# ufcg-lsd/custom-k8s-scheduler

Hardware: AMD Instinct MI355X
Metric: pods scheduled/sec (exact sequential stream, 5,000 nodes x 100,000 pods) (higher is better)
Workload: dtype int32+f64; 1 GPU; config2: 5,000 nodes x 100,000 pods, exact sequential, Fit+Balanced+QoS weights, percentageOfNodesToScore=100; engine=lookahead, launch=resident, table_layout=compact, lookahead=32, parallelism=single

## Files before the change

### custom-k8s-scheduler_amd/csrc/qs_ctx.hpp

```cpp
#pragma once
#include <hip/hip_runtime.h>
#include <rccl/rccl.h>

#include <mutex>
#include <string>
#include <vector>

#include "../../include/qsched.h"
#include "qs_device.hpp"
#include "qs_launch.hpp"

namespace qs_host {

constexpr int64_t kLimit = (1LL << 24) - 1;
constexpr int64_t kWideMemLimit = (1LL << 46) - 1;
constexpr int64_t kGrowLimit32 = (1LL << 31) - 1;
constexpr int64_t kGrowLimitF64 = (1LL << 53) - 1;
constexpr uint32_t kSoaMinNodes = 1u << 16;
constexpr uint32_t kAaMaxNodes = 1u << 20;

struct QsError {
    qs_status st;
    std::string msg;
};

#define HIPCHK(x)                                                                          \
    do {                                                                                   \
        hipError_t e_ = (x);                                                               \
        if (e_ != hipSuccess)                                                              \
            throw QsError{QS_EDEVICE, std::string(#x) + ": " + hipGetErrorString(e_)};     \
    } while (0)

[[noreturn]] inline void fail(qs_status st, const std::string &m) { throw QsError{st, m}; }

inline thread_local std::string g_open_err;
inline qs_status open_failed(qs_status st, const std::string &m) {
    g_open_err = m;
    return st;
}

struct DevBuf {
    void *p = nullptr;
    size_t bytes = 0;
    void ensure(size_t b) {
        if (b <= bytes) return;
        if (p) (void)hipFree(p);
        p = nullptr;
        bytes = 0;
        HIPCHK(hipMalloc(&p, b));
        bytes = b;
    }
    ~DevBuf() {
        if (p) (void)hipFree(p);
    }
    template <class T>
    T *as() const { return (T *)p; }
};

struct Mirror {
    uint32_t n = 0;
    std::vector<int64_t> ac, am, mp, rc, rm, zc, zm, np;
    std::vector<int64_t> ae, re;
    std::vector<uint64_t> th, ts, lb;
    std::vector<int32_t> zone;
    std::vector<uint64_t> gen;
    void resize(uint32_t nn) {
        n = nn;
        zone.assign(nn, 0);
        for (auto *v : {&ac, &am, &mp, &rc, &rm, &zc, &zm, &np}) v->assign(nn, 0);
        ae.assign((size_t)nn * QS_MAX_EXT, 0);
        re.assign((size_t)nn * QS_MAX_EXT, 0);
        th.assign(nn, 0);
        ts.assign(nn, 0);
        lb.assign((size_t)nn * 2, 0);
        gen.assign(nn, 0);
    }
};

inline int ctz64(int64_t v) { return v == 0 ? 64 : __builtin_ctzll((uint64_t)v); }

}

struct qs_stream {
    uint32_t p = 0;
    uint32_t feat = 0;
    std::vector<qs_pod> pods;
    std::vector<uint32_t> order;
    qs_host::DevBuf d_pods, d_podx, d_node, d_key, d_stamp;
    bool ran = false;
    int mode_ran = -1;
    uint64_t epoch_after = 0;
    int shift = 0;
    bool wide = false;
    qs_ctx *owner = nullptr;
    hipGraphExec_t gexec = nullptr;
    std::vector<uint8_t> gkey;
    ~qs_stream() {
        if (gexec) (void)hipGraphExecDestroy(gexec);
    }
};

struct qs_ctx {
    std::mutex mu;
    uint64_t table_epoch = 0;
    qs_config cfg{};
    int device = 0;
    hipStream_t stream = nullptr;
    hipStream_t stream2 = nullptr;
    std::string err;
    qs_host::Mirror m;
    int shift = 20;
    bool wide = false;
    bool dev_valid = false;
    uint32_t zero_alloc = 0;
    qs::DevTable dt{};
    qs::DevCfg dc{};
    qs_scoring_strategy strat[3] = {};
    qs_host::DevBuf strat_tab;
    std::vector<qs_stream *> streams;
    qs_host::DevBuf tbl;
    qs_host::DevBuf soa;
    bool soa_valid = false;
    qs_host::DevBuf tbl_saved;
    qs_host::Mirror m_saved;
    bool saved = false;
    bool saved_wide = false;
    int saved_shift = 20;
    bool mirror_stale = false;
    uint64_t device_faults = 0;
    qs_host::DevBuf diag;
    qs_host::DevBuf scratch, lists, clists, dio, npart, normi, nstat, nfall, nrec, bctrl, one_pod, one_podx;
    qs_host::DevBuf vshard;
    void *pin = nullptr;
    size_t pin_bytes = 0;
    uint64_t score_seq = 0;
    qs_host::DevBuf score_gs;
    uint32_t pend = 0xFFFFFFFFu;
    qs_host::DevBuf hand;
    bool handoff_off = false;
    qs_host::DevBuf resctl;
    int res_timeouts = 0;
    bool res_cooldown = false;
    uint32_t inject_used = 0;
    bool last_resident = false;
    int32_t last_res_path = 0;
    int cus = 0;
    uint64_t run_seq = 0;
    bool last_waits = false;
    uint32_t cap = 0;
    int rank = 0, world = 1;
    ncclComm_t comm = nullptr;
    qs_host::DevBuf mbox, mbox_peers;
    std::vector<void *> mbox_opened;
    bool mbox_on = false;
    bool mbox_fine = false;
    bool mbox_broken = false;
    bool mbox_host = false;
    void *mbox_hptr = nullptr;
    std::string mbox_shm;
    std::vector<void *> mbox_hmaps;
};
namespace qs_host {
void mbox_host_release(qs_ctx *c);
}

namespace qs_host {
struct ShardPlan {
    uint32_t W, v0, nv;
};
inline ShardPlan shard_plan(const qs_ctx *c) {
    if (c->world > 1) return {(uint32_t)c->world, (uint32_t)c->rank, 1u};
    if (c->cfg.virtual_shards > 1) return {(uint32_t)c->cfg.virtual_shards, 0u, (uint32_t)c->cfg.virtual_shards};
    return {1u, 0u, 1u};
}
void exchange_lists(qs_ctx *c, uint64_t *lists, size_t per_rank_entries, hipStream_t stream);
void exchange_u32(qs_ctx *c, uint32_t *buf, size_t per_rank_words, hipStream_t stream);
void allreduce_max_u64(qs_ctx *c, uint64_t *buf, size_t count, hipStream_t stream);
void allreduce_max_u32(qs_ctx *c, uint32_t *buf, size_t count, hipStream_t stream);
constexpr size_t kDioWords = 68;
constexpr size_t kMbRanks = 16, kMbSlots = 3, kMbPartPerRank = 4096;
constexpr size_t kMbFlags = 2 * kMbRanks * 8;
constexpr size_t kMbListSlot = kMbRanks * 64 * 64 * 8;
constexpr size_t kMbPartSlot = kMbRanks * kMbPartPerRank * 16;
constexpr size_t kMbResSlots = 4, kMbResPods = 32;
constexpr size_t kMbResHello = kMbFlags + kMbSlots * (kMbListSlot + kMbPartSlot);
constexpr size_t kMbResFlags = kMbResHello + 256;
constexpr size_t kMbResLists = kMbResFlags + kMbResSlots * kMbResPods * kMbRanks * 8;
constexpr size_t kMbResNFlags = kMbResLists + kMbResSlots * kMbResPods * kMbRanks * 64 * 8;
constexpr size_t kMbResNorm = kMbResNFlags + kMbResSlots * kMbResPods * kMbRanks * 8;
constexpr size_t kMbBytes = kMbResNorm + kMbResSlots * kMbResPods * kMbRanks * 16;
inline uint64_t *mbox_lists(qs_ctx *c, uint32_t slot) {
    return reinterpret_cast<uint64_t *>(static_cast<char *>(c->mbox.p) + kMbFlags + slot * kMbListSlot);
}
inline uint4 *mbox_npart(qs_ctx *c, uint32_t slot) {
    return reinterpret_cast<uint4 *>(static_cast<char *>(c->mbox.p) + kMbFlags + kMbSlots * kMbListSlot +
                                     slot * kMbPartSlot);
}
void mbox_exchange(qs_ctx *c, int phase, uint32_t slot, size_t block_bytes, uint32_t pods, uint32_t L,
                   uint64_t seq, uint32_t *werr, hipStream_t stream);
}
```

### custom-k8s-scheduler_amd/csrc/qs_host.cpp

```cpp
#include "../../include/qsched.h"

#include <hip/hip_runtime.h>

#include <algorithm>
#include <atomic>
#include <chrono>
#include <cmath>
#include <cstddef>
#include <cstdio>
#include <cstdlib>
#include <cstring>
#include <exception>
#include <mutex>
#include <new>
#include <string>
#include <vector>
#include <functional>
#include <condition_variable>
#include <thread>

#include "qs_ctx.hpp"

using namespace qs;

using namespace qs_host;

namespace {

uint32_t feat_of(const qs_config &c) {
    uint32_t f = 0;
    if (c.enable_taint) f |= kFeatTaint;
    if (c.enable_affinity) f |= kFeatAffinity;
    return f;
}

void check_cfg(const qs_config &c) {
    if (c.abi_version != QS_ABI_VERSION) fail(QS_EINVAL, "qs_config.abi_version mismatch");
    if (c.fit_weight_cpu < 0 || c.fit_weight_mem < 0 || c.fit_weight_cpu > 65535 ||
        c.fit_weight_mem > 65535)
        fail(QS_EINVAL, "fit weights out of range");
    int64_t wmax = 0;
    for (int q = 0; q < 3; q++) {
        if (c.w_fit[q] < 0 || c.w_bal[q] < 0 || c.w_fit[q] > 65535 || c.w_bal[q] > 65535)
            fail(QS_EINVAL, "plugin weights must be in [0, 65535]");
        wmax = std::max<int64_t>(wmax, (int64_t)c.w_fit[q] + c.w_bal[q]);
    }
    if (c.w_taint < 0 || c.w_affinity < 0 || c.w_taint > 65535 || c.w_affinity > 65535)
        fail(QS_EINVAL, "plugin weights must be in [0, 65535]");
    if (c.n_fit_resources < 0 || c.n_fit_resources > QS_MAX_SCORE_RES)
        fail(QS_EINVAL, "n_fit_resources must be in [0, 4]");
    if (c.n_balanced_resources < 0 || c.n_balanced_resources > QS_MAX_SCORE_RES)
        fail(QS_EINVAL, "n_balanced_resources must be in [0, 4]");
    uint32_t seen = 0;
    for (int i = 0; i < c.n_fit_resources; i++) {
        const int32_t r = c.fit_resources[i].resource;
        if (r < QS_RES_CPU || r > QS_RES_EXT1) fail(QS_EINVAL, "fit_resources: unknown resource");
        if (seen & (1u << r)) fail(QS_EINVAL, "fit_resources: duplicate resource");
        seen |= 1u << r;
        if (c.fit_resources[i].weight < 1 || c.fit_resources[i].weight > 100)
            fail(QS_EINVAL, "fit_resources: weight must be in [1, 100]");
    }
    seen = 0;
    for (int i = 0; i < c.n_balanced_resources; i++) {
        const int32_t r = c.balanced_resources[i];
        if (r < QS_RES_CPU || r > QS_RES_EXT1) fail(QS_EINVAL, "balanced_resources: unknown resource");
        if (seen & (1u << r)) fail(QS_EINVAL, "balanced_resources: duplicate resource");
        seen |= 1u << r;
    }
    const int64_t tmax = 100 * (wmax + (c.enable_taint ? c.w_taint : 0) +
                                (c.enable_affinity ? c.w_affinity : 0));
    if (tmax >= 0x7FFFFFFF) fail(QS_EINVAL, "weighted total would overflow the packed key");
}

void fit_weights(const qs_config &c, int64_t w[5]) {
    for (int r = 0; r < 5; r++) w[r] = 0;
    if (c.n_fit_resources == 0) {
        w[QS_RES_CPU] = c.fit_weight_cpu;
        w[QS_RES_MEMORY] = c.fit_weight_mem;
        return;
    }
    for (int i = 0; i < c.n_fit_resources; i++) w[c.fit_resources[i].resource] = c.fit_resources[i].weight;
}

uint32_t balanced_ids(const qs_config &c) {
    if (c.n_balanced_resources == 0) return QS_RES_CPU | (QS_RES_MEMORY << 4);
    uint32_t b = 0;
    for (int i = 0; i < c.n_balanced_resources; i++) b |= (uint32_t)c.balanced_resources[i] << (4 * i);
    return b;
}

uint32_t res_feat(const qs_config &c, bool has_ext) {
    static const bool force = getenv("QS_FORCE_RES") && getenv("QS_FORCE_RES")[0] == '1';
    if (force) return kFeatRes | kFeatExt;
    int64_t w[5];
    fit_weights(c, w);
    bool generic = has_ext && (w[QS_RES_EXT0] != 0 || w[QS_RES_EXT1] != 0);
    uint32_t set = 0;
    const uint32_t b = balanced_ids(c);
    for (int i = 0; i < QS_MAX_SCORE_RES; i++) {
        const uint32_t id = (b >> (4 * i)) & 15u;
        if (id == QS_RES_CPU || id == QS_RES_MEMORY || (has_ext && id >= QS_RES_EXT0)) set |= 1u << id;
    }
    generic |= set != ((1u << QS_RES_CPU) | (1u << QS_RES_MEMORY));
    return generic ? (kFeatRes | kFeatExt) : 0u;
}
uint32_t strat_feat(const qs_ctx *c, const qs_pod *pods, uint32_t p) {
    if (c->strat[0].type == QS_STRATEGY_LEAST_ALLOCATED && c->strat[1].type == QS_STRATEGY_LEAST_ALLOCATED &&
        c->strat[2].type == QS_STRATEGY_LEAST_ALLOCATED)
        return 0u;
    for (uint32_t j = 0; j < p; j++)
        if (c->strat[pods[j].qos].type != QS_STRATEGY_LEAST_ALLOCATED) return kFeatStrat | kFeatRes | kFeatExt;
    return 0u;
}

DevCfg make_devcfg(const qs_config &c) {
    DevCfg d{};
    int64_t w[5];
    fit_weights(c, w);
    d.wc = (int32_t)w[QS_RES_CPU];
    d.wm = (int32_t)w[QS_RES_MEMORY];
    d.we0 = (int32_t)w[QS_RES_EXT0];
    d.we1 = (int32_t)w[QS_RES_EXT1];
    d.bal = balanced_ids(c);
    auto rcp = [](int64_t v) { return v > 0 ? 1.0 / (double)v : 0.0; };
    d.yd_both = rcp(w[QS_RES_CPU] + w[QS_RES_MEMORY]);
    d.yd_c = rcp(w[QS_RES_CPU]);
    d.yd_m = rcp(w[QS_RES_MEMORY]);
    d.wtt = c.enable_taint ? c.w_taint : 0;
    d.wna = c.enable_affinity ? c.w_affinity : 0;
    d.feat = feat_of(c);
    d.ba_skip_be = c.balanced_skip_besteffort ? 1u : 0u;
    return d;
}

int table_shift(const Mirror &m) {
    int s = 20;
    for (uint32_t i = 0; i < m.n; i++) {
        s = std::min(s, ctz64(m.am[i]));
        s = std::min(s, ctz64(m.rm[i]));
        s = std::min(s, ctz64(m.zm[i]));
    }
    return s;
}

bool zero_alloc_row(const Mirror &m, uint32_t i) { return m.ac[i] <= 0 || m.am[i] <= 0; }
uint32_t count_zero_alloc(const Mirror &m) {
    uint32_t z = 0;
    for (uint32_t i = 0; i < m.n; i++) z += zero_alloc_row(m, i) ? 1u : 0u;
    return z;
}

void check_range(int64_t v, const char *what, uint32_t i, int64_t limit = kLimit) {
    if (v < 0 || v > limit)
        fail(QS_EINVAL, std::string("node ") + std::to_string(i) + ": " + what + " = " + std::to_string(v) +
                            " outside the device range [0, " + std::to_string(limit) + "]");
}

void check_row_values(const Mirror &m, uint32_t i) {
    check_range(m.ac[i], "alloc_cpu", i);
    check_range(m.rc[i], "req_cpu", i);
    check_range(m.zc[i], "nz_cpu", i);
    check_range(m.np[i], "pods", i);
    check_range(m.mp[i], "max_pods", i);
    check_range(m.am[i], "alloc_mem", i, kWideMemLimit);
    check_range(m.rm[i], "req_mem", i, kWideMemLimit);
    check_range(m.zm[i], "nz_mem", i, kWideMemLimit);
    for (int k = 0; k < QS_MAX_EXT; k++) {
        check_range(m.ae[(size_t)i * QS_MAX_EXT + k], "alloc_ext", i);
        check_range(m.re[(size_t)i * QS_MAX_EXT + k], "req_ext", i);
    }
    if (m.zone[i] < 0 || m.zone[i] >= (int32_t)kMaxZones)
        fail(QS_EINVAL, "node " + std::to_string(i) + ": zone outside [0, 64)");
}

bool row_compact_ok(const Mirror &m, uint32_t i, int shift) {
    return (m.am[i] >> shift) <= kLimit && (m.rm[i] >> shift) <= kLimit && (m.zm[i] >> shift) <= kLimit;
}

HostRow compact_row(const Mirror &m, uint32_t i, int shift, bool wide) {
    HostRow r{};
    check_row_values(m, i);
    if (!wide && !row_compact_ok(m, i, shift))
        fail(QS_EINVAL, "node " + std::to_string(i) + ": memory outside the compact layout");
    r.zone = m.zone[i];
    r.ac = (int32_t)m.ac[i];
    r.rc = (int32_t)m.rc[i];
    r.zc = (int32_t)m.zc[i];
    r.np = (int32_t)m.np[i];
    r.mp = (int32_t)m.mp[i];
    r.yc = r.ac ? 1.0 / (double)r.ac : 0.0;
    if (wide) {
        r.wam = (double)m.am[i];
        r.wrm = (double)m.rm[i];
        r.wzm = (double)m.zm[i];
        r.ym = m.am[i] ? 1.0 / r.wam : 0.0;
    } else {
        r.am = (int32_t)(m.am[i] >> shift);
        r.rm = (int32_t)(m.rm[i] >> shift);
        r.zm = (int32_t)(m.zm[i] >> shift);
        r.ym = r.am ? 1.0 / (double)r.am : 0.0;
    }
    r.ae0 = (int32_t)m.ae[(size_t)i * QS_MAX_EXT + 0];
    r.ae1 = (int32_t)m.ae[(size_t)i * QS_MAX_EXT + 1];
    r.re0 = (int32_t)m.re[(size_t)i * QS_MAX_EXT + 0];
    r.re1 = (int32_t)m.re[(size_t)i * QS_MAX_EXT + 1];
    r.th = m.th[i];
    r.ts = m.ts[i];
    r.lb0 = m.lb[(size_t)i * 2];
    r.lb1 = m.lb[(size_t)i * 2 + 1];
    return r;
}

size_t carve(DevTable &t, uint32_t cap, bool wide, char *base) {
    size_t off = 0;
    auto take = [&](size_t bytes) {
        char *p = base ? base + off : nullptr;
        off += (bytes + 255) & ~(size_t)255;
        return p;
    };
    if (wide) {
        t.rows = nullptr;
        t.wrows = (DRowW *)take((size_t)cap * sizeof(DRowW));
    } else {
        t.wrows = nullptr;
        t.rows = (DRow *)take((size_t)cap * sizeof(DRow));
    }
    t.masks = (DMask *)take((size_t)cap * sizeof(DMask));
    t.zone = (int32_t *)take((size_t)cap * 4);
    t.cap = cap;
    if (cap <= kAaMaxNodes) {
        t.apps = (uint32_t *)take((size_t)kAppWords * cap * 4);
        t.zcount = (int32_t *)take((size_t)kMaxApps * kMaxZones * 4);
    } else {
        t.apps = nullptr;
        t.zcount = nullptr;
    }
    return off;
}

DRow to_drow(const HostRow &r) {
    DRow d;
    d.ac = r.ac; d.am = r.am; d.rc = r.rc; d.rm = r.rm; d.zc = r.zc; d.zm = r.zm;
    d.np = r.np; d.mp = r.mp; d.yc = r.yc; d.ym = r.ym;
    d.ae0 = r.ae0; d.re0 = r.re0; d.ae1 = r.ae1; d.re1 = r.re1;
    return d;
}

uint32_t soa_min_nodes(const qs_ctx *c) {
    const int32_t v = c->cfg.scan_soa_min_nodes;
    return v == 0 ? kSoaMinNodes : (v < 0 ? 0xFFFFFFFFu : (uint32_t)v);
}

DRowW to_drow_wide(const HostRow &r) {
    DRowW d;
    d.ac = r.ac; d.rc = r.rc; d.zc = r.zc; d.np = r.np;
    d.am = r.wam; d.rm = r.wrm; d.zm = r.wzm; d.ym = r.ym;
    d.yc = r.yc; d.mp = r.mp; d.pad = 0;
    d.ae0 = r.ae0; d.re0 = r.re0; d.ae1 = r.ae1; d.re1 = r.re1;
    return d;
}

void upload_table(qs_ctx *c) {
    const uint32_t n = c->m.n;
    const uint32_t cap = std::max<uint32_t>(64, (n + 63) & ~63u);
    const bool wide = c->wide;
    const size_t need = carve(c->dt, cap, wide, nullptr);
    if (cap > c->cap || !c->tbl.p || need > c->tbl.bytes) {
        c->tbl.ensure(need);
        c->cap = std::max(cap, c->cap);
    }
    carve(c->dt, c->cap, wide, c->tbl.as<char>());
    c->dt.n = n;
    const bool soa = !wide && n > 0 && n >= soa_min_nodes(c);
    std::memset(&c->dt.soa, 0, sizeof c->dt.soa);
    std::vector<DRow> rows(wide ? 0 : n);
    std::vector<DRowW> wrows(wide ? n : 0);
    std::vector<DMask> masks(n);
    std::vector<int32_t> cols(soa ? (size_t)kSCols * c->cap : 0, 0);
    for (uint32_t i = 0; i < n; i++) {
        const HostRow r = compact_row(c->m, i, c->shift, wide);
        if (wide) wrows[i] = to_drow_wide(r);
        else rows[i] = to_drow(r);
        masks[i] = DMask{r.th, r.ts, r.lb0, r.lb1};
        if (soa) {
            const int32_t f[kSCols] = {r.ac, r.am, r.rc, r.rm, r.zc, r.zm, r.np, r.mp, r.ae0, r.re0, r.ae1, r.re1};
            for (int k = 0; k < kSCols; k++) cols[(size_t)k * c->cap + i] = f[k];
        }
    }
    if (n) {
        if (wide) HIPCHK(hipMemcpyAsync(c->dt.wrows, wrows.data(), n * sizeof(DRowW), hipMemcpyHostToDevice, c->stream));
        else HIPCHK(hipMemcpyAsync(c->dt.rows, rows.data(), n * sizeof(DRow), hipMemcpyHostToDevice, c->stream));
        HIPCHK(hipMemcpyAsync(c->dt.masks, masks.data(), n * sizeof(DMask), hipMemcpyHostToDevice, c->stream));
        HIPCHK(hipMemcpyAsync(c->dt.zone, c->m.zone.data(), n * 4, hipMemcpyHostToDevice, c->stream));
    }
    if (c->dt.apps) {
        HIPCHK(hipMemsetAsync(c->dt.apps, 0, (size_t)kAppWords * c->cap * 4, c->stream));
        HIPCHK(hipMemsetAsync(c->dt.zcount, 0, (size_t)kMaxApps * kMaxZones * 4, c->stream));
    }
    if (soa) {
        c->soa.ensure(cols.size() * 4);
        for (int k = 0; k < kSCols; k++) c->dt.soa.c[k] = c->soa.as<int32_t>() + (size_t)k * c->cap;
        HIPCHK(hipMemcpyAsync(c->soa.p, cols.data(), cols.size() * 4, hipMemcpyHostToDevice, c->stream));
    }
    HIPCHK(hipStreamSynchronize(c->stream));
    c->dev_valid = true;
    c->soa_valid = soa;
    c->mirror_stale = false;
}

void ensure_soa(qs_ctx *c) {
    if (!c->dt.soa.c[0] || c->soa_valid) return;
    HIPCHK(launch_rows_to_soa(c->dt, c->stream));
    c->soa_valid = true;
}

void push_row(qs_ctx *c, uint32_t i, bool sync = true) {
    if (!c->dev_valid) return;
    const HostRow r = compact_row(c->m, i, c->shift, c->wide);
    hipLaunchKernelGGL(k_set_row, dim3(1), dim3(1), 0, c->stream, c->dt, i, r,
                       kFeatExt | kFeatTaint | kFeatAffinity);
    HIPCHK(hipGetLastError());
    if (sync) HIPCHK(hipStreamSynchronize(c->stream));
}

void flush_pending(qs_ctx *c) {
    if (c->pend == 0xFFFFFFFFu) return;
    const uint32_t i = c->pend;
    c->pend = 0xFFFFFFFFu;
    if (c->dev_valid && i < c->m.n) push_row(c, i, false);
}

void sync_mirror(qs_ctx *c) {
    if (!c->mirror_stale || !c->dev_valid) return;
    const uint32_t n = c->m.n;
    Mirror &m = c->m;
    if (c->wide) {
        std::vector<DRowW> rows(n);
        if (n) HIPCHK(hipMemcpyAsync(rows.data(), c->dt.wrows, n * sizeof(DRowW), hipMemcpyDeviceToHost, c->stream));
        HIPCHK(hipStreamSynchronize(c->stream));
        for (uint32_t i = 0; i < n; i++) {
            m.rc[i] = rows[i].rc;
            m.rm[i] = (int64_t)rows[i].rm;
            m.zc[i] = rows[i].zc;
            m.zm[i] = (int64_t)rows[i].zm;
            m.np[i] = rows[i].np;
            m.re[(size_t)i * QS_MAX_EXT] = rows[i].re0;
            m.re[(size_t)i * QS_MAX_EXT + 1] = rows[i].re1;
        }
    } else {
        std::vector<DRow> rows(n);
        if (n) HIPCHK(hipMemcpyAsync(rows.data(), c->dt.rows, n * sizeof(DRow), hipMemcpyDeviceToHost, c->stream));
        HIPCHK(hipStreamSynchronize(c->stream));
        for (uint32_t i = 0; i < n; i++) {
            m.rc[i] = rows[i].rc;
            m.rm[i] = (int64_t)rows[i].rm << c->shift;
            m.zc[i] = rows[i].zc;
            m.zm[i] = (int64_t)rows[i].zm << c->shift;
            m.np[i] = rows[i].np;
            m.re[(size_t)i * QS_MAX_EXT] = rows[i].re0;
            m.re[(size_t)i * QS_MAX_EXT + 1] = rows[i].re1;
        }
    }
    c->mirror_stale = false;
}

int pod_min_shift(const qs_pod &p) { return std::min(ctz64(p.req_mem), ctz64(p.nz_mem)); }

void check_pod(const qs_pod &p, uint32_t j) {
    auto bad = [&](const char *w) {
        fail(QS_EINVAL, std::string("pod ") + std::to_string(j) + ": " + w);
    };
    if (p.qos < 0 || p.qos > 2) bad("qos must be 0..2");
    if (p.req_cpu < 0 || p.req_mem < 0 || p.nz_cpu < 0 || p.nz_mem < 0) bad("negative request");
    for (int k = 0; k < QS_MAX_EXT; k++)
        if (p.req_ext[k] < 0 || p.req_ext[k] > kLimit) bad("req_ext out of range");
    if (p.req_cpu > kLimit || p.nz_cpu > kLimit) bad("cpu request out of range");
    if (p.req_mem > kWideMemLimit || p.nz_mem > kWideMemLimit) bad("memory request above 2^46 bytes");
    if (p.n_req_terms < 0 || p.n_req_terms > QS_MAX_TERMS || p.n_pref_terms < 0 ||
        p.n_pref_terms > QS_MAX_TERMS)
        bad("term count out of range");
    for (int t = 0; t < p.n_pref_terms; t++)
        if (p.pref_weight[t] < 0 || p.pref_weight[t] > 100) bad("preferred term weight must be 0..100");
    if (p.app < 0 || p.app >= QS_MAX_APPS) bad("app outside [0, QS_MAX_APPS)");
    if (p.anti_affinity < QS_AA_NONE || p.anti_affinity > QS_AA_ZONE) bad("anti_affinity must be 0..2");
}

uint32_t pod_flags(const qs_ctx *c, const qs_pod &p) {
    const uint32_t aff = c->cfg.enable_affinity ? 1u : 0u;
    return (uint32_t)p.qos | ((uint32_t)c->strat[p.qos].type << 2) | (aff * (uint32_t)p.n_req_terms << 4) |
           (aff * (uint32_t)p.n_pref_terms << 8) | ((uint32_t)p.anti_affinity << 12) | ((uint32_t)p.app << 16);
}

size_t pod_record_bytes(bool wide) { return wide ? sizeof(DPodW) : sizeof(DPod); }

void compact_pod(const qs_ctx *c, const qs_pod &p, uint32_t j, int shift, bool wide, void *dst) {
    check_pod(p, j);
    if (wide) {
        DPodW d{};
        d.rc = (int32_t)p.req_cpu;
        d.zc = (int32_t)p.nz_cpu;
        d.rm = (double)p.req_mem;
        d.zm = (double)p.nz_mem;
        d.re0 = (int32_t)p.req_ext[0];
        d.re1 = (int32_t)p.req_ext[1];
        d.wfit = (uint16_t)c->cfg.w_fit[p.qos];
        d.wbal = (uint16_t)c->cfg.w_bal[p.qos];
        d.flags = pod_flags(c, p);
        std::memcpy(dst, &d, sizeof d);
        return;
    }
    if ((p.req_mem >> shift) > kLimit || (p.nz_mem >> shift) > kLimit)
        fail(QS_EINVAL, "pod " + std::to_string(j) + ": memory request out of the compact range");
    DPod d{};
    d.rc = (int32_t)p.req_cpu;
    d.rm = (int32_t)(p.req_mem >> shift);
    d.zc = (int32_t)p.nz_cpu;
    d.zm = (int32_t)(p.nz_mem >> shift);
    d.re0 = (int32_t)p.req_ext[0];
    d.re1 = (int32_t)p.req_ext[1];
    d.wfit = (uint16_t)c->cfg.w_fit[p.qos];
    d.wbal = (uint16_t)c->cfg.w_bal[p.qos];
    d.flags = pod_flags(c, p);
    std::memcpy(dst, &d, sizeof d);
}

DPodX compact_podx(const qs_ctx *c, const qs_pod &p) {
    DPodX x{};
    const bool taint = c->cfg.enable_taint != 0, aff = c->cfg.enable_affinity != 0;
    x.tol_hard = taint ? p.tol_hard : ~0ull;
    x.tol_soft = taint ? p.tol_soft : ~0ull;
    x.sel0 = aff ? p.sel[0] : 0ull;
    x.sel1 = aff ? p.sel[1] : 0ull;
    for (int t = 0; t < QS_MAX_TERMS; t++) {
        x.req[t][0] = p.req_terms[t][0];
        x.req[t][1] = p.req_terms[t][1];
        x.pref[t][0] = p.pref_terms[t][0];
        x.pref[t][1] = p.pref_terms[t][1];
        x.pw[t] = p.pref_weight[t];
    }
    return x;
}

std::vector<uint32_t> qos_order(const qs_pod *pods, uint32_t p, bool sort) {
    std::vector<uint32_t> o(p);
    for (uint32_t j = 0; j < p; j++) o[j] = j;
    if (sort)
        std::stable_sort(o.begin(), o.end(), [&](uint32_t a, uint32_t b) {
            if (pods[a].qos != pods[b].qos) return pods[a].qos > pods[b].qos;
            return pods[a].priority > pods[b].priority;
        });
    return o;
}

void mirror_reserve(Mirror &m, uint32_t i, const qs_pod &p, int sign) {
    m.rc[i] += sign * p.req_cpu;
    m.rm[i] += sign * p.req_mem;
    for (int k = 0; k < QS_MAX_EXT; k++) m.re[(size_t)i * QS_MAX_EXT + k] += sign * p.req_ext[k];
    m.zc[i] += sign * p.nz_cpu;
    m.zm[i] += sign * p.nz_mem;
    m.np[i] += sign;
}

void ensure_layout(qs_ctx *c, const qs_pod *pods, uint32_t p, int extra_shift = 64) {
    const Mirror &m = c->m;
    int want = std::min(c->shift, extra_shift);
    int64_t mem_max = 0, nzm = 0, nzc = 0;
    for (uint32_t j = 0; j < p; j++) {
        want = std::min(want, pod_min_shift(pods[j]));
        mem_max = std::max({mem_max, pods[j].req_mem, pods[j].nz_mem});
        nzm = std::max(nzm, pods[j].nz_mem);
        nzc = std::max(nzc, pods[j].nz_cpu);
    }
    want = std::max(0, want);
    bool wide = c->wide;
    for (uint32_t i = 0; i < m.n; i++) {
        const __int128 more = (__int128)std::max<int64_t>(0, m.mp[i] - m.np[i]) + 1;
        if ((__int128)m.zc[i] + more * nzc > kGrowLimit32)
            fail(QS_EINVAL, "node " + std::to_string(i) + ": NonZeroRequested cpu could pass 2^31 m during the stream");
        if (!wide && (!row_compact_ok(m, i, want) ||
                      (__int128)(m.zm[i] >> want) + more * (nzm >> want) > kGrowLimit32))
            wide = true;
        if (wide && (__int128)m.zm[i] + more * nzm > kGrowLimitF64)
            fail(QS_EINVAL, "node " + std::to_string(i) + ": NonZeroRequested memory could pass 2^53 B during the stream");
    }
    if (!wide && (mem_max >> want) > kLimit) wide = true;
    if (wide != c->wide || (!wide && want < c->shift)) {
        sync_mirror(c);
        c->wide = wide;
        if (!wide) c->shift = want;
        c->dev_valid = false;
        c->saved = false;
    }
    if (!c->dev_valid) upload_table(c);
}

bool pod_fits_layout(const qs_ctx *c, const qs_pod &p) {
    if (!c->dev_valid) return false;
    if (c->wide) return true;
    return pod_min_shift(p) >= c->shift && (p.req_mem >> c->shift) <= kLimit && (p.nz_mem >> c->shift) <= kLimit;
}

struct RowSnap {
    int64_t ac, am, mp, rc, rm, zc, zm, np, ae[QS_MAX_EXT], re[QS_MAX_EXT];
    uint64_t th, ts, lb0, lb1, gen;
    int32_t zone;
};
RowSnap snap_row(const Mirror &m, uint32_t i) {
    RowSnap r{m.ac[i], m.am[i], m.mp[i], m.rc[i], m.rm[i], m.zc[i], m.zm[i], m.np[i], {}, {},
              m.th[i], m.ts[i], m.lb[2 * (size_t)i], m.lb[2 * (size_t)i + 1], m.gen[i], m.zone[i]};
    for (int k = 0; k < QS_MAX_EXT; k++) {
        r.ae[k] = m.ae[(size_t)i * QS_MAX_EXT + k];
        r.re[k] = m.re[(size_t)i * QS_MAX_EXT + k];
    }
    return r;
}
void put_row(Mirror &m, uint32_t i, const RowSnap &r) {
    m.ac[i] = r.ac; m.am[i] = r.am; m.mp[i] = r.mp; m.rc[i] = r.rc; m.rm[i] = r.rm;
    m.zc[i] = r.zc; m.zm[i] = r.zm; m.np[i] = r.np;
    for (int k = 0; k < QS_MAX_EXT; k++) {
        m.ae[(size_t)i * QS_MAX_EXT + k] = r.ae[k];
        m.re[(size_t)i * QS_MAX_EXT + k] = r.re[k];
    }
    m.th[i] = r.th; m.ts[i] = r.ts; m.lb[2 * (size_t)i] = r.lb0; m.lb[2 * (size_t)i + 1] = r.lb1;
    m.gen[i] = r.gen; m.zone[i] = r.zone;
}

enum InjectHook : uint32_t { kInjStreamRun = 1u, kInjHandoff = 2u, kInjResidentStall = 4u };
bool inject_once(qs_ctx *c, const char *name, uint32_t bit) {
    const char *e = getenv("QS_INJECT_FAULT");
    if (!e || std::strcmp(e, name) != 0 || (c->inject_used & bit)) return false;
    c->inject_used |= bit;
    return true;
}
void maybe_inject_fault(qs_ctx *c, const char *entry) {
    if (inject_once(c, entry, kInjStreamRun))
        fail(QS_EDEVICE, std::string("injected device fault in ") + entry);
}

void flush_pending(qs_ctx *c);

template <class F>
qs_status guarded(qs_ctx *c, F &&f, bool keep_pending = false) {
    if (!c) return QS_EINVAL;
    std::lock_guard<std::mutex> lk(c->mu);
    try {
        if (!keep_pending) flush_pending(c);
        f();
        c->err.clear();
        return QS_OK;
    } catch (const QsError &e) {
        c->err = e.msg;
        if (e.st == QS_EDEVICE || e.st == QS_ETIMEOUT) {
            c->dev_valid = false;
            c->mirror_stale = false;
            c->saved = false;
            c->device_faults++;
        }
        return e.st;
    } catch (const std::bad_alloc &) {
        c->err = "out of host memory";
        return QS_ENOMEM;
    } catch (const std::exception &e) {
        c->err = e.what();
        return QS_EINVAL;
    } catch (...) {
        c->err = "unknown error";
        return QS_EINVAL;
    }
}

struct KernelTimer {
    bool on;
    hipStream_t stream, stream2;
    std::vector<std::pair<hipEvent_t, hipEvent_t>> ev[4];
    double secs[4] = {0, 0, 0, 0};
    uint64_t count[4] = {0, 0, 0, 0};
    KernelTimer(bool o, hipStream_t s, hipStream_t s2) : on(o), stream(s), stream2(s2) {}
    void begin(int k, hipStream_t s) {
        if (!on) return;
        hipEvent_t a, b;
        HIPCHK(hipEventCreate(&a));
        HIPCHK(hipEventCreate(&b));
        HIPCHK(hipEventRecord(a, s));
        ev[k].push_back({a, b});
    }
    void end(int k, hipStream_t s) {
        if (!on) return;
        HIPCHK(hipEventRecord(ev[k].back().second, s));
    }
    void finish() {
        if (!on) return;
        HIPCHK(hipStreamSynchronize(stream));
        HIPCHK(hipStreamSynchronize(stream2));
        for (int k = 0; k < 4; k++) {
            for (auto &e : ev[k]) {
                float ms = 0.f;
                HIPCHK(hipEventElapsedTime(&ms, e.first, e.second));
                secs[k] += ms * 1e-3;
                count[k]++;
                (void)hipEventDestroy(e.first);
                (void)hipEventDestroy(e.second);
            }
            ev[k].clear();
        }
    }
};

uint32_t la_window(const qs_ctx *c);
bool la_overlap(const qs_ctx *c);

int pick_engine(const qs_ctx *c, uint32_t n) {
    int e = c->cfg.engine;
    const uint32_t feat = c->dc.feat;
    if (e == QS_ENGINE_AUTO) {
        if (n > 0 && la_geometry(n, la_window(c), shard_plan(c).W, 2 * la_window(c)).G > 0)
            e = QS_ENGINE_LOOKAHEAD;
        else if (n <= persistent_max_nodes(feat)) e = QS_ENGINE_PERSISTENT;
        else e = QS_ENGINE_SCAN;
    }
    if (e == QS_ENGINE_BATCHED) fail(QS_EINVAL, "the batched engine runs through QS_MODE_BATCHED");
    if (e == QS_ENGINE_PERSISTENT && n > persistent_max_nodes(feat))
        fail(QS_EINVAL, "PERSISTENT engine supports at most " +
                            std::to_string(persistent_max_nodes(feat)) + " nodes for this profile");
    return e;
}

bool la_overlap(const qs_ctx *c) {
    static const char *env = getenv("QS_LA_OVERLAP");
    if (env && env[0] == '0') return false;
    return !c->cfg.lookahead_serial && la_window(c) <= 32;
}

LaGeom lookahead_geometry(const qs_ctx *c, uint32_t n, bool overlap) {
    const ShardPlan sp = shard_plan(c);
    const uint32_t K = la_window(c);
    LaGeom geo = la_geometry(n, K, sp.W, overlap ? 2 * K : K);
    geo.v0 = sp.v0;
    geo.nv = sp.nv;
    return geo;
}

uint32_t la_window(const qs_ctx *c) {
    int K = c->cfg.lookahead > 0 ? c->cfg.lookahead : 32;
    return (uint32_t)std::min(64, std::max(1, K));
}

void percentile_stats(const std::vector<uint64_t> &st, qs_stats *s) {
    if (st.size() < 2) return;
    std::vector<double> d(st.size() - 1);
    for (size_t i = 1; i < st.size(); i++) d[i - 1] = (double)(st[i] - st[i - 1]) * 0.01;
    std::sort(d.begin(), d.end());
    auto pct = [&](double q) { return d[std::min(d.size() - 1, (size_t)(q * (double)(d.size() - 1) + 0.5))]; };
    s->p50_cycle_us = pct(0.50);
    s->p99_cycle_us = pct(0.99);
    s->max_cycle_us = d.back();
}

}

uint64_t run_batched(qs_ctx *c, qs_stream *s, const void *dp, const DPodX *dx, int32_t *on, uint64_t *ok,
                     KernelTimer &kt) {
    const uint32_t n = c->m.n, P = s->p;
    for (int q = 0; q < 3; q++)
        if (c->strat[q].type != QS_STRATEGY_LEAST_ALLOCATED)
            fail(QS_EINVAL, "QS_MODE_BATCHED scores LeastAllocated only (qs_set_scoring_strategy[_qos]: class " +
                                std::to_string(q) + " has another strategy)");
    if (c->dc.feat & (kFeatTaint | kFeatAffinity))
        fail(QS_EINVAL, "QS_MODE_BATCHED supports the Fit + Balanced (+ extended resources) profile");
    if (!c->dt.apps) fail(QS_EINVAL, "QS_MODE_BATCHED keeps anti-affinity state for tables up to 2^20 nodes");
    if (c->world > 1 || c->cfg.virtual_shards > 1) fail(QS_EINVAL, "QS_MODE_BATCHED runs unsharded");
    if (batch_claim_lds(n) > 160 * 1024)
        fail(QS_EINVAL, "QS_MODE_BATCHED claims batches in LDS: tables up to 712,672 nodes");
    HIPCHK(batch_claim_prepare());
    const uint32_t B = c->cfg.batch_pods > 0 ? (uint32_t)std::min(64, c->cfg.batch_pods) : 64u;
    LaGeom geo = la_geometry(n, B, 1, 64);
    if (geo.G == 0) fail(QS_EINVAL, "no batched geometry for this table size");
    geo.waves = 4;
    geo.k32 = 0;
    const size_t lwords = (size_t)geo.K * 64 * geo.eplr;
    const size_t cwords = std::max<size_t>(1, (size_t)geo.K * geo.G * geo.L);
    c->lists.ensure(8 * lwords);
    c->clists.ensure(8 * cwords);
    c->bctrl.ensure(4 * 192);
    uint32_t *ctrl = c->bctrl.as<uint32_t>(), *bidx = ctrl + 64, *tickets = ctrl + 128;
    LaBufs bf{c->lists.as<uint64_t>(), c->clists.as<uint64_t>(), nullptr, nullptr, nullptr, nullptr,
              nullptr, bidx, ctrl};
    const char *fm = getenv("QS_BATCH_FUSED_MERGE");
    if (!(fm && fm[0] == '0')) bf.tickets = tickets;
    auto batch = [&]() {
        kt.begin(2, c->stream);
        HIPCHK(launch_la_window(c->dt, dp, dx, 0, P, c->dc, geo, bf, on, ok, nullptr, nullptr, c->stream, 1));
        kt.end(2, c->stream);
        kt.begin(3, c->stream);
        HIPCHK(launch_batch_claim(c->dt, dp, bf.lists, ctrl, bidx, P, B, on, ok, c->stream));
        kt.end(3, c->stream);
    };
    const uint32_t nb0 = (P + B - 1) / B;
    auto enqueue = [&]() {
        HIPCHK(hipMemsetAsync(bf.lists, 0, 8 * lwords, c->stream));
        HIPCHK(hipMemsetAsync(tickets, 0, 4 * 64, c->stream));
        HIPCHK(launch_batch_init(ctrl, bidx, P, B, c->stream));
        static const char *se = getenv("QS_SYNC_EVERY");
        const uint32_t every = se ? (uint32_t)atoi(se) : 0u;
        for (uint32_t b = 0; b < nb0; ++b) {
            batch();
            if (every && (b + 1) % every == 0 && !kt.on) HIPCHK(hipStreamSynchronize(c->stream));
        }
    };
    static const char *genv = getenv("QS_GRAPH");
    if (!kt.on && !(genv && genv[0] == '0')) {
        std::vector<uint8_t> key;
        auto put = [&](const void *p, size_t nb) { key.insert(key.end(), (const uint8_t *)p, (const uint8_t *)p + nb); };
        const void *ptrs[] = {c->dt.rows, c->dt.wrows, c->dt.apps, bf.lists, bf.clists, ctrl, dp, on, ok};
        put(ptrs, sizeof ptrs);
        put(&c->dt.n, sizeof c->dt.n);
        put(&c->dc, sizeof c->dc);
        put(&geo, sizeof geo);
        const int tag = 2;
        put(&tag, sizeof tag);
        put(&bf.tickets, sizeof bf.tickets);
        if (!s->gexec || s->gkey != key) {
            if (s->gexec) (void)hipGraphExecDestroy(s->gexec);
            s->gexec = nullptr;
            HIPCHK(hipStreamBeginCapture(c->stream, hipStreamCaptureModeThreadLocal));
            try {
                enqueue();
            } catch (...) {
                hipGraph_t g = nullptr;
                (void)hipStreamEndCapture(c->stream, &g);
                if (g) (void)hipGraphDestroy(g);
                throw;
            }
            hipGraph_t g = nullptr;
            HIPCHK(hipStreamEndCapture(c->stream, &g));
            const hipError_t ie = hipGraphInstantiate(&s->gexec, g, nullptr, nullptr, 0);
            (void)hipGraphDestroy(g);
            HIPCHK(ie);
            s->gkey = key;
        }
        HIPCHK(hipGraphLaunch(s->gexec, c->stream));
    } else {
        enqueue();
    }
    uint64_t batches = nb0;
    for (;;) {
        uint32_t h[2] = {0, 0};
        HIPCHK(hipMemcpyAsync(h, ctrl, 8, hipMemcpyDeviceToHost, c->stream));
        HIPCHK(hipStreamSynchronize(c->stream));
        if (h[0] == 0) break;
        if (batches > 2ull * P + 64) fail(QS_EDEVICE, "batched mode made no progress");
        batch();
        ++batches;
    }
    c->soa_valid = false;
    return batches;
}

extern "C" {

const char *qs_version(void) { return "qsched 0.1 (gfx950)"; }

void qs_config_default(qs_config *cfg) {
    if (!cfg) return;
    std::memset(cfg, 0, sizeof(*cfg));
    cfg->abi_version = QS_ABI_VERSION;
    cfg->engine = QS_ENGINE_AUTO;
    cfg->fit_weight_cpu = 1;
    cfg->fit_weight_mem = 1;
    const int32_t wf[3] = {1, 2, 3}, wb[3] = {1, 1, 1};
    for (int q = 0; q < 3; q++) { cfg->w_fit[q] = wf[q]; cfg->w_bal[q] = wb[q]; }
    cfg->w_taint = 3;
    cfg->w_affinity = 2;
    cfg->qos_sort = 1;
}

qs_status qs_open(const qs_config *cfg, int device, qs_ctx **out) {
    g_open_err.clear();
    if (!cfg || !out) return open_failed(QS_EINVAL, "qs_open: null config or output pointer");
    *out = nullptr;
    qs_ctx *c = new (std::nothrow) qs_ctx();
    if (!c) return QS_ENOMEM;
    try {
        check_cfg(*cfg);
        c->cfg = *cfg;
        c->device = device;
        int ndev = 0;
        HIPCHK(hipGetDeviceCount(&ndev));
        if (device < 0 || device >= ndev) fail(QS_EINVAL, "no such device");
        HIPCHK(hipSetDevice(device));
        HIPCHK(hipStreamCreateWithFlags(&c->stream, hipStreamNonBlocking));
        HIPCHK(hipStreamCreateWithFlags(&c->stream2, hipStreamNonBlocking));
        c->dc = make_devcfg(c->cfg);
        c->scratch.ensure(scan_scratch_bytes());
        HIPCHK(hipMemset(c->scratch.p, 0, scan_scratch_bytes()));
    } catch (const QsError &e) {
        delete c;
        return open_failed(e.st, e.msg);
    } catch (...) {
        delete c;
        return open_failed(QS_EDEVICE, "qs_open: unexpected failure");
    }
    *out = c;
    return QS_OK;
}

qs_status qs_close(qs_ctx *c) {
    if (!c) return QS_EINVAL;
    {
        std::lock_guard<std::mutex> lk(c->mu);
        (void)hipSetDevice(c->device);
        if (c->stream) (void)hipStreamSynchronize(c->stream);
        if (c->comm) (void)ncclCommDestroy(c->comm);
        c->comm = nullptr;
        for (void *p : c->mbox_opened) (void)hipIpcCloseMemHandle(p);
        c->mbox_opened.clear();
        mbox_host_release(c);
        for (qs_stream *ps : c->streams) ps->owner = nullptr;
        c->streams.clear();
    }
    hipStream_t s = c->stream, s2 = c->stream2;
    if (s2) (void)hipStreamSynchronize(s2);
    if (c->pin) (void)hipHostFree(c->pin);
    delete c;
    if (s) (void)hipStreamDestroy(s);
    if (s2) (void)hipStreamDestroy(s2);
    return QS_OK;
}

static void shape_table(const qs_shape_point *sh, uint32_t n, uint8_t table[101]) {
    if (!sh || !table) fail(QS_EINVAL, "shape: null pointer");
    if (n < 1 || n > QS_MAX_SHAPE) fail(QS_EINVAL, "shape: 1 to 16 points");
    for (uint32_t i = 0; i < n; i++) {
        if (sh[i].utilization < 0 || sh[i].utilization > 100) fail(QS_EINVAL, "shape: utilization must be in [0, 100]");
        if (sh[i].score < 0 || sh[i].score > 10) fail(QS_EINVAL, "shape: score must be in [0, 10]");
        if (i && sh[i].utilization <= sh[i - 1].utilization)
            fail(QS_EINVAL, "shape: utilization must be strictly increasing");
    }
    for (int64_t p = 0; p <= 100; p++) {
        int64_t v = (int64_t)sh[n - 1].score * 10;
        for (uint32_t i = 0; i < n; i++) {
            if (p > sh[i].utilization) continue;
            const int64_t s1 = (int64_t)sh[i].score * 10;
            if (i == 0) { v = s1; break; }
            const int64_t s0 = (int64_t)sh[i - 1].score * 10, u0 = sh[i - 1].utilization, u1 = sh[i].utilization;
            v = s0 + (s1 - s0) * (p - u0) / (u1 - u0);
            break;
        }
        table[p] = (uint8_t)v;
    }
}

qs_status qs_shape_table(const qs_shape_point *shape, uint32_t n, uint8_t table[101]) {
    try {
        shape_table(shape, n, table);
    } catch (const QsError &) {
        return QS_EINVAL;
    }
    return QS_OK;
}

static void strategy_table(const qs_scoring_strategy *s, uint8_t tab[128]) {
    if (!s) fail(QS_EINVAL, "null scoring strategy");
    if (s->type != QS_STRATEGY_LEAST_ALLOCATED && s->type != QS_STRATEGY_MOST_ALLOCATED &&
        s->type != QS_STRATEGY_REQUESTED_TO_CAPACITY_RATIO)
        fail(QS_EINVAL, "unknown scoring strategy type");
    if (s->type != QS_STRATEGY_REQUESTED_TO_CAPACITY_RATIO && s->n_shape != 0)
        fail(QS_EINVAL, "a shape is given for a scoring strategy that takes none");
    std::memset(tab, 0, 128);
    if (s->type == QS_STRATEGY_REQUESTED_TO_CAPACITY_RATIO) {
        if (s->n_shape < 1 || s->n_shape > QS_MAX_SHAPE) fail(QS_EINVAL, "shape: 1 to 16 points");
        shape_table(s->shape, (uint32_t)s->n_shape, tab);
    }
}

static void set_strategy(qs_ctx *c, int q0, int q1, const qs_scoring_strategy *s, const uint8_t tab[128]) {
    if (!c->streams.empty()) fail(QS_ESTATE, "the scoring strategy cannot change while prepared streams exist");
    HIPCHK(hipSetDevice(c->device));
    HIPCHK(hipStreamSynchronize(c->stream));
    alignas(16) uint8_t all[3 * 128];
    qs_scoring_strategy next[3] = {c->strat[0], c->strat[1], c->strat[2]};
    for (int q = 0; q < 3; q++) {
        if (q >= q0 && q <= q1) {
            next[q] = qs_scoring_strategy{};
            next[q].type = s->type;
            next[q].n_shape = s->n_shape;
            for (int i = 0; i < s->n_shape; i++) next[q].shape[i] = s->shape[i];
            std::memcpy(all + 128 * q, tab, 128);
        } else {
            uint8_t t[128];
            strategy_table(&c->strat[q], t);
            std::memcpy(all + 128 * q, t, 128);
        }
    }
    c->strat_tab.ensure(sizeof all);
    HIPCHK(hipMemcpy(c->strat_tab.p, all, sizeof all, hipMemcpyHostToDevice));
    bool rtcr = false;
    for (int q = 0; q < 3; q++) {
        c->strat[q] = next[q];
        rtcr |= next[q].type == QS_STRATEGY_REQUESTED_TO_CAPACITY_RATIO;
    }
    const uint64_t tp = rtcr ? (uint64_t)(uintptr_t)c->strat_tab.p : 0;
    c->dc.strat_tab_lo = (uint32_t)tp;
    c->dc.strat_tab_hi = (uint32_t)(tp >> 32);
}

qs_status qs_set_scoring_strategy(qs_ctx *c, const qs_scoring_strategy *s) {
    return guarded(c, [&] {
        uint8_t tab[128];
        strategy_table(s, tab);
        set_strategy(c, 0, 2, s, tab);
    });
}

qs_status qs_set_scoring_strategy_qos(qs_ctx *c, int32_t qos, const qs_scoring_strategy *s) {
    return guarded(c, [&] {
        if (qos < 0 || qos > 2) fail(QS_EINVAL, "qos must be 0 (BestEffort), 1 (Burstable) or 2 (Guaranteed)");
        uint8_t tab[128];
        strategy_table(s, tab);
        set_strategy(c, qos, qos, s, tab);
    });
}

qs_status qs_get_scoring_strategy_qos(qs_ctx *c, int32_t qos, qs_scoring_strategy *out) {
    return guarded(c, [&] {
        if (qos < 0 || qos > 2) fail(QS_EINVAL, "qos must be 0 (BestEffort), 1 (Burstable) or 2 (Guaranteed)");
        if (!out) fail(QS_EINVAL, "null scoring strategy");
        *out = c->strat[qos];
    });
}

const char *qs_last_error(const qs_ctx *c) {
    if (c) return c->err.c_str();
    return g_open_err.empty() ? "null context" : g_open_err.c_str();
}

qs_status qs_nodes_load(qs_ctx *c, const qs_node_soa *nd, uint32_t n) {
    return guarded(c, [&] {
        if (!nd || !nd->alloc_cpu || !nd->alloc_mem) fail(QS_EINVAL, "alloc_cpu/alloc_mem required");
        HIPCHK(hipSetDevice(c->device));
        Mirror &m = c->m;
        m.resize(n);
        auto get = [](const int64_t *a, size_t i, int64_t d) { return a ? a[i] : d; };
        for (uint32_t i = 0; i < n; i++) {
            m.ac[i] = nd->alloc_cpu[i];
            m.am[i] = nd->alloc_mem[i];
            m.mp[i] = get(nd->max_pods, i, 110);
            m.rc[i] = get(nd->req_cpu, i, 0);
            m.rm[i] = get(nd->req_mem, i, 0);
            m.zc[i] = get(nd->nz_cpu, i, 0);
            m.zm[i] = get(nd->nz_mem, i, 0);
            m.np[i] = get(nd->pods, i, 0);
            for (int k = 0; k < QS_MAX_EXT; k++) {
                m.ae[(size_t)i * QS_MAX_EXT + k] = get(nd->alloc_ext, (size_t)i * QS_MAX_EXT + k, 0);
                m.re[(size_t)i * QS_MAX_EXT + k] = get(nd->req_ext, (size_t)i * QS_MAX_EXT + k, 0);
            }
            m.zone[i] = nd->zone ? nd->zone[i] : 0;
            m.th[i] = nd->taint_hard ? nd->taint_hard[i] : 0;
            m.ts[i] = nd->taint_soft ? nd->taint_soft[i] : 0;
            m.lb[2 * (size_t)i] = nd->label_bits ? nd->label_bits[2 * (size_t)i] : 0;
            m.lb[2 * (size_t)i + 1] = nd->label_bits ? nd->label_bits[2 * (size_t)i + 1] : 0;
        }
        for (uint32_t i = 0; i < n; i++) check_row_values(m, i);
        c->shift = table_shift(m);
        c->zero_alloc = count_zero_alloc(m);
        c->wide = false;
        for (uint32_t i = 0; i < n && !c->wide; i++) c->wide = !row_compact_ok(m, i, c->shift);
        c->dev_valid = false;
        c->saved = false;
        c->mirror_stale = false;
        ++c->table_epoch;
        upload_table(c);
    });
}

qs_status qs_nodes_read(qs_ctx *c, const qs_node_soa_out *o, uint32_t n) {
    return guarded(c, [&] {
        if (!o) fail(QS_EINVAL, "null output");
        if (n != c->m.n) fail(QS_EINVAL, "n does not match the loaded table");
        sync_mirror(c);
        const Mirror &m = c->m;
        auto put = [](int64_t *d, const std::vector<int64_t> &s) {
            if (d) std::memcpy(d, s.data(), s.size() * 8);
        };
        put(o->alloc_cpu, m.ac); put(o->alloc_mem, m.am); put(o->max_pods, m.mp);
        put(o->req_cpu, m.rc); put(o->req_mem, m.rm); put(o->nz_cpu, m.zc); put(o->nz_mem, m.zm);
        put(o->pods, m.np); put(o->alloc_ext, m.ae); put(o->req_ext, m.re);
        if (o->taint_hard) std::memcpy(o->taint_hard, m.th.data(), 8 * (size_t)n);
        if (o->taint_soft) std::memcpy(o->taint_soft, m.ts.data(), 8 * (size_t)n);
        if (o->label_bits) std::memcpy(o->label_bits, m.lb.data(), 16 * (size_t)n);
        if (o->zone) std::memcpy(o->zone, m.zone.data(), 4 * (size_t)n);
    });
}

qs_status qs_node_upsert(qs_ctx *c, uint32_t idx, const qs_node_row *r, uint64_t generation) {
    return guarded(c, [&] {
        if (!r) fail(QS_EINVAL, "null row");
        HIPCHK(hipSetDevice(c->device));
        sync_mirror(c);
        Mirror &m = c->m;
        if (idx > m.n) fail(QS_EINVAL, "idx beyond table end (append only at idx == n)");
        if (idx < m.n && generation != 0 && generation <= m.gen[idx]) return;
        Mirror one;
        one.resize(1);
        one.ac[0] = r->alloc_cpu; one.am[0] = r->alloc_mem; one.mp[0] = r->max_pods;
        one.rc[0] = r->req_cpu; one.rm[0] = r->req_mem; one.zc[0] = r->nz_cpu; one.zm[0] = r->nz_mem;
        one.np[0] = r->pods;
        for (int k = 0; k < QS_MAX_EXT; k++) { one.ae[k] = r->alloc_ext[k]; one.re[k] = r->req_ext[k]; }
        one.th[0] = r->taint_hard; one.ts[0] = r->taint_soft;
        one.lb[0] = r->label_bits[0]; one.lb[1] = r->label_bits[1];
        one.zone[0] = r->zone;
        one.gen[0] = generation;
        check_row_values(one, 0);
        const bool was_zero = idx < m.n && zero_alloc_row(m, idx);
        if (idx == m.n) {
            Mirror old = m;
            m.resize(old.n + 1);
            auto cp = [&](std::vector<int64_t> &d, const std::vector<int64_t> &s) { std::copy(s.begin(), s.end(), d.begin()); };
            cp(m.ac, old.ac); cp(m.am, old.am); cp(m.mp, old.mp); cp(m.rc, old.rc); cp(m.rm, old.rm);
            cp(m.zc, old.zc); cp(m.zm, old.zm); cp(m.np, old.np); cp(m.ae, old.ae); cp(m.re, old.re);
            std::copy(old.th.begin(), old.th.end(), m.th.begin());
            std::copy(old.ts.begin(), old.ts.end(), m.ts.begin());
            std::copy(old.lb.begin(), old.lb.end(), m.lb.begin());
            std::copy(old.gen.begin(), old.gen.end(), m.gen.begin());
            std::copy(old.zone.begin(), old.zone.end(), m.zone.begin());
            c->dev_valid = false;
            c->saved = false;
        }
        put_row(m, idx, snap_row(one, 0));
        c->zero_alloc += (zero_alloc_row(m, idx) ? 1u : 0u) - (was_zero ? 1u : 0u);
        ++c->table_epoch;
        const int want = std::min({ctz64(r->alloc_mem), ctz64(r->req_mem), ctz64(r->nz_mem)});
        const bool was_valid = c->dev_valid;
        const int old_shift = c->shift;
        const bool old_wide = c->wide;
        ensure_layout(c, nullptr, 0, want);
        if (was_valid && c->dev_valid && c->shift == old_shift && c->wide == old_wide) push_row(c, idx);
    });
}

static qs_status reserve_impl(qs_ctx *c, uint32_t node, const qs_pod *p, int sign) {
    return guarded(c, [&] {
        if (!p) fail(QS_EINVAL, "null pod");
        if (node >= c->m.n) fail(QS_EINVAL, "node index out of range");
        check_pod(*p, 0);
        HIPCHK(hipSetDevice(c->device));
        sync_mirror(c);
        const RowSnap before = snap_row(c->m, node);
        mirror_reserve(c->m, node, *p, sign);
        ++c->table_epoch;
        try {
            check_row_values(c->m, node);
            if (pod_fits_layout(c, *p) && (c->wide || row_compact_ok(c->m, node, c->shift))) {
                if (c->pend != 0xFFFFFFFFu && c->pend != node) flush_pending(c);
                c->pend = node;
                return;
            }
            flush_pending(c);
            const bool was_valid = c->dev_valid;
            const int old_shift = c->shift;
            const bool old_wide = c->wide;
            ensure_layout(c, p, 1);
            if (was_valid && c->shift == old_shift && c->wide == old_wide) push_row(c, node);
        } catch (...) {
            put_row(c->m, node, before);
            throw;
        }
    }, true);
}
qs_status qs_reserve(qs_ctx *c, uint32_t node, const qs_pod *p) { return reserve_impl(c, node, p, +1); }
qs_status qs_unreserve(qs_ctx *c, uint32_t node, const qs_pod *p) { return reserve_impl(c, node, p, -1); }

__attribute__((always_inline)) static inline void unpack_body(const uint32_t *pk, uint32_t n, const uint32_t w[4],
                                                              uint8_t *feas, int32_t *score, int32_t *total) {
    typedef uint32_t u32x16 __attribute__((ext_vector_type(16)));
    typedef int32_t i32x16 __attribute__((ext_vector_type(16)));
    typedef uint8_t u8x16 __attribute__((ext_vector_type(16)));
    typedef uint8_t u8x64 __attribute__((ext_vector_type(64)));
    typedef int32_t i32x64 __attribute__((ext_vector_type(64)));
    uint32_t i = 0;
    for (; i + 16 <= n; i += 16) {
        u32x16 v;
        std::memcpy(&v, pk + i, sizeof v);
        const i32x16 ok = v != kScoreInfeasible;
        const u32x16 z = v & (u32x16)ok;
        if (feas) {
            const u8x16 f = __builtin_convertvector(ok, u8x16) & (uint8_t)1;
            std::memcpy(feas + i, &f, sizeof f);
        }
        if (total) {
            const u32x16 t = (z & 255u) * w[0] + ((z >> 8) & 255u) * w[1] + ((z >> 16) & 255u) * w[2] + (z >> 24) * w[3];
            const i32x16 r = ((i32x16)t & ok) | ~ok;
            std::memcpy(total + i, &r, sizeof r);
        }
        if (score) {
            u8x64 b;
            std::memcpy(&b, &z, sizeof b);
            const i32x64 wd = __builtin_convertvector(b, i32x64);
            std::memcpy(score + 4 * (size_t)i, &wd, sizeof wd);
        }
    }
    for (; i < n; ++i) {
        const bool f = pk[i] != kScoreInfeasible;
        const uint32_t z = f ? pk[i] : 0u;
        if (feas) feas[i] = f;
        if (score)
            for (uint32_t k = 0; k < 4; ++k) score[4 * (size_t)i + k] = (int32_t)((z >> (8 * k)) & 255u);
        if (total)
            total[i] = f ? (int32_t)((z & 255u) * w[0] + ((z >> 8) & 255u) * w[1] + ((z >> 16) & 255u) * w[2] +
                                     (z >> 24) * w[3])
                         : -1;
    }
}
__attribute__((target("avx512f,avx512bw,avx512vl"))) static void unpack_avx512(const uint32_t *pk, uint32_t n,
                                                                               const uint32_t w[4], uint8_t *feas,
                                                                               int32_t *score, int32_t *total) {
    unpack_body(pk, n, w, feas, score, total);
}
__attribute__((target("avx2"))) static void unpack_avx2(const uint32_t *pk, uint32_t n, const uint32_t w[4],
                                                        uint8_t *feas, int32_t *score, int32_t *total) {
    unpack_body(pk, n, w, feas, score, total);
}
static void unpack_base(const uint32_t *pk, uint32_t n, const uint32_t w[4], uint8_t *feas, int32_t *score,
                        int32_t *total) {
    unpack_body(pk, n, w, feas, score, total);
}
class UnpackPool {
   public:
    static UnpackPool &get() {
        static UnpackPool *p = new UnpackPool;
        return *p;
    }
    int parts() const { return (int)th_.size() + 1; }
    void run(const std::function<void(int)> &fn) {
        std::lock_guard<std::mutex> one(run_mu_);
        {
            std::lock_guard<std::mutex> g(mu_);
            fn_ = &fn;
            left_.store((int)th_.size(), std::memory_order_relaxed);
            gen_.fetch_add(1, std::memory_order_release);
        }
        cv_.notify_all();
        fn(0);
        while (left_.load(std::memory_order_acquire) != 0) std::this_thread::yield();
    }

   private:
    UnpackPool() {
        const unsigned hw = std::max(1u, std::thread::hardware_concurrency());
        const char *e = getenv("QS_UNPACK_THREADS");
        const unsigned want = e ? (unsigned)std::max(0, atoi(e)) : 7u;
        const int helpers = (int)std::min(want, hw > 1 ? hw - 1 : 0u);
        for (int k = 0; k < helpers; ++k) th_.emplace_back([this, k] { loop(k + 1); });
        for (auto &t : th_) t.detach();
    }
    void loop(int part) {
        uint64_t seen = 0;
        for (;;) {
            const auto t0 = std::chrono::steady_clock::now();
            while (gen_.load(std::memory_order_acquire) == seen &&
                   std::chrono::steady_clock::now() - t0 < std::chrono::microseconds(50))
                std::this_thread::yield();
            if (gen_.load(std::memory_order_acquire) == seen) {
                std::unique_lock<std::mutex> lk(mu_);
                cv_.wait(lk, [&] { return gen_.load(std::memory_order_acquire) != seen; });
            }
            seen = gen_.load(std::memory_order_acquire);
            (*fn_)(part);
            left_.fetch_sub(1, std::memory_order_acq_rel);
        }
    }
    std::vector<std::thread> th_;
    std::mutex mu_, run_mu_;
    std::condition_variable cv_;
    std::atomic<uint64_t> gen_{0};
    std::atomic<int> left_{0};
    const std::function<void(int)> *fn_ = nullptr;
};

static void unpack_scores(const uint32_t *pk, uint32_t n, const uint32_t w[4], uint8_t *feas, int32_t *score,
                          int32_t *total) {
    using Fn = void (*)(const uint32_t *, uint32_t, const uint32_t *, uint8_t *, int32_t *, int32_t *);
    static const Fn fn = [] {
#if !defined(__HIP_DEVICE_COMPILE__)
        __builtin_cpu_init();
        if (getenv("QS_UNPACK_BASE")) return (Fn)unpack_base;
        if (__builtin_cpu_supports("avx512bw") && __builtin_cpu_supports("avx512vl")) return (Fn)unpack_avx512;
        if (__builtin_cpu_supports("avx2")) return (Fn)unpack_avx2;
#endif
        return (Fn)unpack_base;
    }();
    static const uint32_t par_min = [] {
        const char *e = getenv("QS_UNPACK_PAR_MIN");
        return e ? (uint32_t)std::max(0, atoi(e)) : 16384u;
    }();
    if (n < par_min || (!score && !total) || UnpackPool::get().parts() < 2) {
        fn(pk, n, w, feas, score, total);
        return;
    }
    UnpackPool &pool = UnpackPool::get();
    const uint32_t parts = (uint32_t)pool.parts();
    const uint32_t per = ((n + parts - 1) / parts + 15) & ~15u;
    pool.run([&](int part) {
        const uint32_t b = std::min(n, (uint32_t)part * per), e = std::min(n, b + per);
        if (b < e)
            fn(pk + b, e - b, w, feas ? feas + b : nullptr, score ? score + 4 * (size_t)b : nullptr,
               total ? total + b : nullptr);
    });
}

static const bool g_sdiag = getenv("QS_SCORE_DIAG") && getenv("QS_SCORE_DIAG")[0] == '1';
struct ScoreSplit { std::chrono::steady_clock::time_point ts, tl, t0, te; };
static thread_local ScoreSplit g_split;
static void score_diag_report(uint64_t seq, std::chrono::steady_clock::time_point tu) {
    auto us = [](auto a, auto b) { return std::chrono::duration<double, std::micro>(b - a).count(); };
    const ScoreSplit &s = g_split;
    if (us(s.ts, tu) > 500.0)
        std::fprintf(stderr, "QS_SCORE_DIAG call %llu: prep %.1f us, launch %.1f us, wait %.1f us, unpack %.1f us\n",
                     (unsigned long long)seq, us(s.ts, s.tl), us(s.tl, s.t0), us(s.t0, s.te), us(s.te, tu));
}

static const uint32_t *score_pod_launch(qs_ctx *c, const qs_pod *pod, uint32_t wts[4], int32_t *best) {
    if (g_sdiag) g_split.ts = std::chrono::steady_clock::now();
    if (!pod) fail(QS_EINVAL, "null pod");
    HIPCHK(hipSetDevice(c->device));
    check_pod(*pod, 0);
    if (!pod_fits_layout(c, *pod)) {
        flush_pending(c);
        ensure_layout(c, pod, 1);
    }
    const uint32_t n = c->m.n;
    alignas(16) uint8_t dp[sizeof(DPodW)];
    compact_pod(c, *pod, 0, c->shift, c->wide, dp);
    if (c->wide) {
        const DPodW *q = reinterpret_cast<const DPodW *>(dp);
        wts[0] = q->wfit; wts[1] = q->wbal;
    } else {
        const DPod *q = reinterpret_cast<const DPod *>(dp);
        wts[0] = q->wfit; wts[1] = q->wbal;
    }
    DevCfg dc = c->dc;
    const bool pod_ext = pod->req_ext[0] || pod->req_ext[1];
    dc.feat = feat_of(c->cfg) | (pod_ext ? kFeatExt : 0u) | (c->wide ? kFeatWide | kFeatExt : 0u) |
              res_feat(c->cfg, pod_ext) | strat_feat(c, pod, 1);
    wts[2] = (dc.feat & kFeatTaint) ? (uint32_t)dc.wtt : 0u;
    wts[3] = (dc.feat & kFeatAffinity) ? (uint32_t)dc.wna : 0u;
    if (n == 0 || !c->dev_valid) {
        if (best) *best = -1;
        return nullptr;
    }
    const DPodX dx = compact_podx(c, *pod);
    const size_t pb = score_pod1_pack_bytes(n);
    if (c->pin_bytes < pb) {
        if (c->pin) (void)hipHostFree(c->pin);
        c->pin = nullptr;
        c->pin_bytes = 0;
        HIPCHK(hipHostMalloc(&c->pin, pb, hipHostMallocDefault));
        c->pin_bytes = pb;
        std::memset(c->pin, 0, pb);
    }
    if (!c->score_gs.p) {
        c->score_gs.ensure(32);
        HIPCHK(hipMemsetAsync(c->score_gs.p, 0, 32, c->stream));
    }
    const uint32_t pidx = c->pend < n ? c->pend : 0xFFFFFFFFu;
    const HostRow prow = pidx < n ? compact_row(c->m, pidx, c->shift, c->wide) : HostRow{};
    const uint64_t seq = ++c->score_seq;
    const auto tl = std::chrono::steady_clock::now();
    HIPCHK(launch_score_pod1(c->dt, dp, &dx, dc, static_cast<uint8_t *>(c->pin), c->score_gs.as<uint64_t>(), seq,
                             pidx, prow, c->stream));
    c->pend = 0xFFFFFFFFu;
    volatile uint64_t *done = reinterpret_cast<volatile uint64_t *>(static_cast<uint8_t *>(c->pin) + 8);
    const auto t0 = std::chrono::steady_clock::now();
    while (*done != seq) {
        if (std::chrono::steady_clock::now() - t0 > std::chrono::milliseconds(200)) {
            HIPCHK(hipStreamSynchronize(c->stream));
            if (*done != seq) fail(QS_EDEVICE, "qs_score_pod: the scoring kernel did not complete");
            break;
        }
    }
    if (g_sdiag) {
        g_split.tl = tl;
        g_split.t0 = t0;
        g_split.te = std::chrono::steady_clock::now();
    }
    std::atomic_thread_fence(std::memory_order_acquire);
    const uint8_t *h = static_cast<const uint8_t *>(c->pin);
    uint64_t kbest = 0;
    std::memcpy(&kbest, h, 8);
    if (best) *best = kbest ? (int32_t)(0xFFFFFFFFu - (uint32_t)kbest) : -1;
    return reinterpret_cast<const uint32_t *>(h + 16);
}

qs_status qs_score_pod(qs_ctx *c, const qs_pod *pod, uint8_t *feas, int32_t *score, int32_t *total,
                       int32_t *best) {
    return guarded(c, [&] {
        uint32_t w[4];
        const uint32_t *pk = score_pod_launch(c, pod, w, best);
        if (pk) unpack_scores(pk, c->m.n, w, feas, score, total);
        if (g_sdiag && pk) score_diag_report(c->score_seq, std::chrono::steady_clock::now());
    }, true);
}

qs_status qs_score_pod_packed(qs_ctx *c, const qs_pod *pod, const uint32_t **packed, int32_t *best) {
    return guarded(c, [&] {
        uint32_t w[4];
        const uint32_t *pk = score_pod_launch(c, pod, w, best);
        if (packed) *packed = pk;
        if (g_sdiag && pk) score_diag_report(c->score_seq, std::chrono::steady_clock::now());
    }, true);
}

qs_status qs_stream_prepare(qs_ctx *c, const qs_pod *pods, uint32_t p, qs_stream **out) {
    if (!out) return QS_EINVAL;
    *out = nullptr;
    qs_stream *s = nullptr;
    qs_status st = guarded(c, [&] {
        if (p && !pods) fail(QS_EINVAL, "null pods");
        HIPCHK(hipSetDevice(c->device));
        s = new qs_stream();
        s->p = p;
        s->pods.assign(pods, pods + p);
        for (uint32_t j = 0; j < p; j++) check_pod(pods[j], j);
        ensure_layout(c, pods, p);
        s->shift = c->shift;
        s->wide = c->wide;
        s->feat = feat_of(c->cfg) | (c->wide ? kFeatWide | kFeatExt : 0u);
        bool has_ext = false;
        for (uint32_t j = 0; j < p && !has_ext; j++) has_ext = pods[j].req_ext[0] || pods[j].req_ext[1];
        if (has_ext) s->feat |= kFeatExt;
        s->feat |= res_feat(c->cfg, has_ext) | strat_feat(c, pods, p);
        s->order = qos_order(pods, p, c->cfg.qos_sort != 0);
        const size_t rb = pod_record_bytes(c->wide);
        std::vector<uint8_t> dp(rb * std::max<uint32_t>(p, 1));
        const bool needx = feat_of(c->cfg) & (kFeatTaint | kFeatAffinity);
        std::vector<DPodX> dx(needx ? std::max<uint32_t>(p, 1) : 1);
        for (uint32_t k = 0; k < p; k++) {
            const uint32_t j = s->order[k];
            compact_pod(c, pods[j], j, c->shift, c->wide, dp.data() + rb * k);
            if (needx) dx[k] = compact_podx(c, pods[j]);
        }
        const size_t P1 = std::max<uint32_t>(p, 1);
        s->d_pods.ensure(rb * P1);
        s->d_podx.ensure(sizeof(DPodX) * dx.size());
        s->d_node.ensure(4 * P1);
        s->d_key.ensure(8 * P1);
        if (c->cfg.record_timestamps) s->d_stamp.ensure(8 * P1);
        HIPCHK(hipMemcpyAsync(s->d_pods.p, dp.data(), rb * p, hipMemcpyHostToDevice, c->stream));
        HIPCHK(hipMemcpyAsync(s->d_podx.p, dx.data(), sizeof(DPodX) * dx.size(), hipMemcpyHostToDevice, c->stream));
        HIPCHK(hipStreamSynchronize(c->stream));
        c->streams.push_back(s);
        s->owner = c;
    });
    if (st != QS_OK) {
        delete s;
        return st;
    }
    *out = s;
    return QS_OK;
}

qs_status qs_stream_run(qs_ctx *c, qs_stream *s, qs_mode mode, qs_stats *stats) {
    return guarded(c, [&] {
        if (!s) fail(QS_EINVAL, "null stream");
        if (mode != QS_MODE_EXACT && mode != QS_MODE_BATCHED) fail(QS_EINVAL, "unknown qs_mode");
        if (s->shift != c->shift || s->wide != c->wide) fail(QS_ESTATE, "node table re-laid out after prepare");
        HIPCHK(hipSetDevice(c->device));
        s->ran = false;
        s->mode_ran = -1;
        ++c->table_epoch;
        if (!c->dev_valid) upload_table(c);
        const uint32_t n = c->m.n, P = s->p;
        c->dc.feat = s->feat;
        const int eng = mode == QS_MODE_BATCHED ? QS_ENGINE_BATCHED : pick_engine(c, n);
        int32_t *on = s->d_node.as<int32_t>();
        uint64_t *ok = s->d_key.as<uint64_t>();
        uint64_t *st = c->cfg.record_timestamps ? s->d_stamp.as<uint64_t>() : nullptr;
        uint64_t batches = 0;
        hipEvent_t e0, e1;
        HIPCHK(hipEventCreate(&e0));
        HIPCHK(hipEventCreate(&e1));
        KernelTimer kt(c->cfg.profile_kernels != 0, c->stream, c->stream2);
        HIPCHK(hipEventRecord(e0, c->stream));
        if (P > 0 && n == 0) {
            HIPCHK(hipMemsetAsync(on, 0xFF, 4 * (size_t)P, c->stream));
            HIPCHK(hipMemsetAsync(ok, 0, 8 * (size_t)P, c->stream));
        } else if (P > 0) {
            const void *dp = s->d_pods.p;
            const DPodX *dx = s->d_podx.as<DPodX>();
            if (eng == QS_ENGINE_BATCHED) {
                batches = run_batched(c, s, dp, dx, on, ok, kt);
            } else if (eng == QS_ENGINE_PERSISTENT) {
                kt.begin(0, c->stream);
                HIPCHK(launch_persistent(c->dt, dp, dx, P, c->dc, on, ok, st, c->stream));
                kt.end(0, c->stream);
                batches = 1;
            } else if (eng == QS_ENGINE_SCAN) {
                HIPCHK(hipMemsetAsync(c->scratch.p, 0, scan_scratch_bytes(), c->stream));
                ensure_soa(c);
                for (uint32_t k = 0; k < P; k++) {
                    kt.begin(1, c->stream);
                    HIPCHK(launch_scan_pod(c->dt, dp, dx, k, c->dc, c->scratch.p, on, ok, st,
                                           nullptr, nullptr, nullptr, 1, c->stream));
                    kt.end(1, c->stream);
                    HIPCHK(launch_scan_pod(c->dt, dp, dx, k, c->dc, c->scratch.p, on, ok, st,
                                           nullptr, nullptr, nullptr, 2, c->stream));
                }
                batches = P;
            } else if (eng == QS_ENGINE_ALLREDUCE) {
                if (!c->comm)
                    fail(QS_ESTATE, "the all-reduce engine needs an RCCL communicator (qs_open_shard with an id)");
                const uint32_t V = c->world == 1 && c->cfg.virtual_shards > 1 ? (uint32_t)c->cfg.virtual_shards : 1u;
                const uint32_t R = V > 1 ? V : (uint32_t)c->world;
                DevTable dt = c->dt;
                std::memset(&dt.soa, 0, sizeof dt.soa);
                std::vector<uint32_t> sh(2 * (size_t)R);
                for (uint32_t r = 0; r < R; ++r) {
                    sh[2 * r] = (uint32_t)((uint64_t)n * r / R);
                    sh[2 * r + 1] = (uint32_t)((uint64_t)n * (r + 1) / R);
                }
                const uint32_t r0 = V > 1 ? 0u : (uint32_t)c->rank;
                c->vshard.ensure(8 * (size_t)R);
                HIPCHK(hipMemcpy(c->vshard.p, sh.data(), 8 * (size_t)R, hipMemcpyHostToDevice));
                HIPCHK(hipMemsetAsync(c->scratch.p, 0, scan_scratch_bytes(), c->stream));
                char *lohi = static_cast<char *>(c->scratch.p) + offsetof(ScanHead, lo);
                auto range = [&](uint32_t r) {
                    return hipMemcpyAsync(lohi, c->vshard.as<uint32_t>() + 2 * r, 8, hipMemcpyDeviceToDevice, c->stream);
                };
                if (V == 1) HIPCHK(range(r0));
                ScanHead *sc = c->scratch.as<ScanHead>();
                const bool norm = (c->dc.feat & (kFeatTaint | kFeatAffinity)) != 0;
                for (uint32_t k = 0; k < P; k++) {
                    kt.begin(1, c->stream);
                    if (norm) {
                        for (uint32_t v = 0; v < V; ++v) {
                            if (V > 1) HIPCHK(range(v));
                            HIPCHK(launch_scan_pod(dt, dp, dx, k, c->dc, c->scratch.p, on, ok, st, nullptr, nullptr,
                                                   nullptr, 8, c->stream));
                        }
                        allreduce_max_u32(c, &sc->mt, 2, c->stream);
                    }
                    for (uint32_t v = 0; v < V; ++v) {
                        if (V > 1) HIPCHK(range(v));
                        HIPCHK(launch_scan_pod(dt, dp, dx, k, c->dc, c->scratch.p, on, ok, st, nullptr, nullptr,
                                               nullptr, 16 | 32, c->stream));
                    }
                    allreduce_max_u64(c, reinterpret_cast<uint64_t *>(&sc->best), 1, c->stream);
                    HIPCHK(launch_scan_pod(dt, dp, dx, k, c->dc, c->scratch.p, on, ok, st, nullptr, nullptr,
                                           nullptr, 64, c->stream));
                    kt.end(1, c->stream);
                }
                batches = P;
            } else {
                const bool overlap = la_overlap(c);
                LaGeom geo = lookahead_geometry(c, n, overlap);
                static const char *rw = getenv("QS_RESOLVER_WAVES");
                const bool norm = (c->dc.feat & (kFeatTaint | kFeatAffinity)) != 0;
                const bool mbox = c->mbox_on && !c->comm;
                if (c->world > 1 && !c->comm && !mbox)
                    fail(QS_ESTATE, "sharded context without a transport: pass an RCCL id to qs_open_shard "
                                    "or connect the mailbox (qs_dist_mailbox_connect)");
                if (mbox && c->mbox_broken)
                    fail(QS_ESTATE, "mailbox ranks out of step after a timeout: every rank must call "
                                    "qs_dist_mailbox_connect again (between two barriers) before the next run");
                geo.waves = norm || (rw && rw[0] == '1' && !overlap) ? 1u : 4u;
                const char *nw = getenv("QS_NORM_WAVES");
                if (norm && overlap && geo.epl == 1 && !(nw && nw[0] == '1')) geo.waves = 4;
                int64_t wmax = 0;
                for (int q = 0; q < 3; q++) wmax = std::max<int64_t>(wmax, (int64_t)c->cfg.w_fit[q] + c->cfg.w_bal[q]);
                if (c->dc.feat & kFeatTaint) wmax += c->cfg.w_taint;
                if (c->dc.feat & kFeatAffinity) wmax += c->cfg.w_affinity;
                geo.k32 = (100 * wmax + 1 < 1024 && n <= (1u << 22)) ? 1u : 0u;
                if (geo.G == 0) fail(QS_EINVAL, "no lookahead geometry for this table size");
                const size_t rank_entries = (size_t)geo.K * 64 * geo.eplr;
                const size_t lwords = geo.W * rank_entries;
                const size_t cwords = std::max<size_t>(1, (size_t)geo.nv * geo.K * geo.G * geo.L);
                const int nbuf = overlap ? 2 : 1;
                c->lists.ensure(8 * lwords * nbuf);
                c->clists.ensure(8 * cwords * nbuf);
                c->dio.ensure(2 * kDioWords * 4);
                const size_t nparts = norm ? (size_t)geo.W * geo.K * geo.G : 1;
                c->npart.ensure(16 * nparts * nbuf);
                c->normi.ensure(16 * (size_t)geo.K * nbuf);
                c->nfall.ensure(16);
                c->nrec.ensure(4 * kDioWords);
                static const bool diag_on = getenv("QS_DIAG") && getenv("QS_DIAG")[0] == '1';
                uint64_t *diag = nullptr;
                if (diag_on) {
                    c->diag.ensure(128);
                    HIPCHK(hipMemsetAsync(c->diag.p, 0, 128, c->stream));
                    diag = c->diag.as<uint64_t>();
                }
                static const char *ho = getenv("QS_HANDOFF");
                static const char *genv0 = getenv("QS_GRAPH");
                const bool handoff_ok = overlap && !c->comm && !c->handoff_off && !kt.on && !(ho && ho[0] == '0');
                const bool graph_forced = genv0 && genv0[0] == '1';
                const bool handoff = handoff_ok && !graph_forced;
                if (!c->hand.p) {
                    c->hand.ensure(32);
                    HIPCHK(hipMemset(c->hand.p, 0, 32));
                }
                uint64_t *hw = c->hand.as<uint64_t>();
                c->dc.ready = handoff ? hw + 1 : nullptr;
                const uint64_t seq_run = (handoff || mbox) ? ++c->run_seq : 0;
                c->dc.epoch = handoff ? seq_run : 0;
                c->last_waits = handoff || mbox;
                if (mbox && (uint64_t)geo.K * geo.G > kMbPartPerRank)
                    fail(QS_EINVAL, "mailbox transport: K*G exceeds the mailbox partials capacity");
                c->dc.werr = handoff ? reinterpret_cast<uint32_t *>(hw + 2) : nullptr;
                uint64_t *L0 = c->lists.as<uint64_t>(), *C0 = c->clists.as<uint64_t>();
                uint32_t *dio = c->dio.as<uint32_t>();
                const uint32_t nwin = (P + geo.K - 1) / geo.K;
                const auto th0 = std::chrono::steady_clock::now();
                static const char *se = getenv("QS_SYNC_EVERY");
                const uint32_t sync_every = se ? (uint32_t)std::max(0, atoi(se)) : 0u;
                bool capturing = false;
                auto enqueue = [&]() {
                if (handoff || mbox) HIPCHK(hipMemsetAsync(hw + 2, 0, 8, c->stream));
                HIPCHK(hipMemsetAsync(c->lists.p, 0, 8 * lwords * nbuf, c->stream));
                HIPCHK(hipMemsetAsync(c->dio.p, 0, 2 * kDioWords * 4, c->stream));
                HIPCHK(hipMemsetAsync(c->nfall.p, 0, 16, c->stream));
                auto bufs = [&](uint32_t w) {
                    const int b = overlap ? (int)(w & 1) : 0;
                    LaBufs bf{L0 + b * lwords, C0 + b * cwords, c->npart.as<uint4>() + b * nparts,
                              c->normi.as<NormInfo>() + (size_t)b * geo.K, nullptr, nullptr,
                              c->nfall.as<unsigned long long>()};
                    bf.rec = c->nrec.as<uint32_t>();
                    if (mbox) {
                        bf.lists = mbox_lists(c, w % 3);
                        bf.npart = mbox_npart(c, w % 3);
                    }
                    if (overlap) {
                        bf.dprev = dio + ((w + 1) & 1) * kDioWords;
                        bf.dcur = dio + (w & 1) * kDioWords;
                    }
                    return bf;
                };
                auto select = [&](uint32_t w, hipStream_t ss) {
                    const LaBufs bf = bufs(w);
                    kt.begin(2, ss);
                    uint32_t *werr = reinterpret_cast<uint32_t *>(hw + 2);
                    if (norm) {
                        HIPCHK(launch_la_window(c->dt, dp, dx, w * geo.K, P, c->dc, geo, bf, on, ok, st, diag, ss, 4));
                        if (c->comm) exchange_u32(c, (uint32_t *)bf.npart, 4 * (size_t)geo.K * geo.G, ss);
                        else if (mbox) mbox_exchange(c, 0, w % 3, 16 * (size_t)geo.K * geo.G, 0, 0, (seq_run << 32) | (w + 1), werr, ss);
                    }
                    HIPCHK(launch_la_window(c->dt, dp, dx, w * geo.K, P, c->dc, geo, bf, on, ok, st, diag, ss, 1));
                    kt.end(2, ss);
                    if (c->comm) exchange_lists(c, bf.lists, rank_entries, ss);
                    else if (mbox) mbox_exchange(c, 1, w % 3, 8 * rank_entries, geo.K, geo.L, (seq_run << 32) | (w + 1), werr, ss);
                    if (handoff) HIPCHK(launch_ready_set(hw + 1, (c->dc.epoch << 32) | (w + 1), ss));
                };
                auto resolve = [&](uint32_t w) {
                    kt.begin(3, c->stream);
                    HIPCHK(launch_la_window(c->dt, dp, dx, w * geo.K, P, c->dc, geo, bufs(w), on, ok, st,
                                            diag, c->stream, 2));
                    kt.end(3, c->stream);
                };
                if (!overlap) {
                    for (uint32_t w = 0; w < nwin; ++w) {
                        select(w, c->stream);
                        resolve(w);
                        if (sync_every && !capturing && (w + 1) % sync_every == 0)
                            HIPCHK(hipStreamSynchronize(c->stream));
                    }
                } else {
                    constexpr int R = 4;
                    hipEvent_t esel[R], eres[R], est;
                    for (int r = 0; r < R; ++r) {
                        HIPCHK(hipEventCreateWithFlags(&esel[r], hipEventDisableTiming));
                        HIPCHK(hipEventCreateWithFlags(&eres[r], hipEventDisableTiming));
                    }
                    HIPCHK(hipEventCreateWithFlags(&est, hipEventDisableTiming));
                    HIPCHK(hipEventRecord(est, c->stream));
                    HIPCHK(hipStreamWaitEvent(c->stream2, est, 0));
                    select(0, c->stream2);
                    HIPCHK(hipEventRecord(esel[0], c->stream2));
                    for (uint32_t w = 0; w < nwin; ++w) {
                        if (w + 1 < nwin) {
                            if (w >= 1) HIPCHK(hipStreamWaitEvent(c->stream2, eres[(w - 1) % R], 0));
                            select(w + 1, c->stream2);
                            HIPCHK(hipEventRecord(esel[(w + 1) % R], c->stream2));
                        }
                        if (!handoff) HIPCHK(hipStreamWaitEvent(c->stream, esel[w % R], 0));
                        resolve(w);
                        HIPCHK(hipEventRecord(eres[w % R], c->stream));
                        if (sync_every && !capturing && (w + 1) % sync_every == 0) {
                            HIPCHK(hipStreamSynchronize(c->stream2));
                            HIPCHK(hipStreamSynchronize(c->stream));
                        }
                    }
                    hipEvent_t eend = nullptr;
                    if (handoff) {
                        HIPCHK(hipEventCreateWithFlags(&eend, hipEventDisableTiming));
                        HIPCHK(hipEventRecord(eend, c->stream2));
                        HIPCHK(hipStreamWaitEvent(c->stream, eend, 0));
                    }
                    for (int r = 0; r < R; ++r) {
                        (void)hipEventDestroy(esel[r]);
                        (void)hipEventDestroy(eres[r]);
                    }
                    (void)hipEventDestroy(est);
                    if (eend) (void)hipEventDestroy(eend);
                }
                };
                static const char *genv = getenv("QS_GRAPH");
                const bool graph_ok = !c->comm || (genv && genv[0] == '1');
                const bool use_graph = graph_ok && !handoff && !mbox && !kt.on && !diag_on && !(genv && genv[0] == '0');
                const char *renv = getenv("QS_RESIDENT");
                if (!c->cus) {
                    int cu = 0;
                    HIPCHK(hipDeviceGetAttribute(&cu, hipDeviceAttributeMultiprocessorCount, c->device));
                    c->cus = cu;
                }
                LaGeom pgeo = geo;
                if (norm && overlap && !(nw && nw[0] == '1')) pgeo.waves = 4;
                const char *rk = getenv("QS_RES_K32");
                if (rk && rk[0] == '0') pgeo.k32 = 0;
                LaGeom rgeo = la_stream_res_plan(pgeo, c->dc.feat, n, (uint32_t)c->cus, 2);
                if (rgeo.G > 0 && rgeo.K * rgeo.G + 1 > la_stream_res_max_blocks(rgeo, c->dc.feat, n, (uint32_t)c->cus))
                    rgeo = la_stream_res_plan(pgeo, c->dc.feat, n, (uint32_t)c->cus, 1);
                static const char *senv = getenv("QS_RES_SEL");
                uint32_t sel = rgeo.K * rgeo.G;
                if (senv && atoi(senv) > 0) sel = (uint32_t)atoi(senv);
                if (norm) sel = std::max(sel, rgeo.K * rgeo.G);
                const bool coresident =
                    rgeo.G > 0 && 1 + sel <= la_stream_res_max_blocks(rgeo, c->dc.feat, n, (uint32_t)c->cus);
                const bool res_transport = c->world == 1 ? !mbox && !c->comm : mbox;
                const bool res_allowed = c->res_timeouts < 2 && !c->res_cooldown;
                const bool resident = overlap && res_transport && res_allowed && !diag_on &&
                                      !(renv && renv[0] == '0') && rgeo.G > 0 && coresident;
                c->last_resident = resident;
                if (!resident) c->res_cooldown = false;
                if (resident) {
                    c->resctl.ensure(la_stream_res_ctl_bytes());
                    c->dc.ready = nullptr;
                    c->dc.epoch = 0;
                    c->dc.werr = reinterpret_cast<uint32_t *>(hw + 2);
                    c->last_waits = true;
                    HIPCHK(hipMemsetAsync(c->lists.p, 0, 8 * lwords * nbuf, c->stream));
                    HIPCHK(hipMemsetAsync(c->dio.p, 0, 2 * kDioWords * 4, c->stream));
                    HIPCHK(hipMemsetAsync(c->resctl.p, 0, la_stream_res_ctl_bytes(), c->stream));
                    HIPCHK(hipMemsetAsync(hw + 2, 0, 8, c->stream));
                    c->npart.ensure(16 * 2 * (size_t)rgeo.K * rgeo.G);
                    c->normi.ensure(16 * 2 * 64);
                    c->nstat.ensure(4 * 2 * 128 * (size_t)rgeo.K);
                    HIPCHK(hipMemsetAsync(c->nfall.p, 0, 16, c->stream));
                    const size_t rcw = std::max<size_t>(1, (size_t)rgeo.K * rgeo.G * rgeo.L);
                    c->clists.ensure(8 * rcw * 2);
                    ResShard rsh{1u, 0u, 0ull, nullptr, 0ull, 0ull, 0ull, 0ull, 0ull};
                    if (c->world > 1)
                        rsh = ResShard{(uint32_t)c->world, (uint32_t)c->rank, seq_run, c->mbox_peers.as<char *>(),
                                       kMbResHello, kMbResFlags, kMbResLists, kMbResNFlags, kMbResNorm};
                    DevCfg dcr = c->dc;
                    const char *inj = getenv("QS_INJECT_FAULT");
                    dcr.inject = (inject_once(c, "resident_stall", kInjResidentStall) ||
                                  (inj && std::strcmp(inj, "resident_stall_always") == 0)) ? 1u : 0u;
                    if (inj && std::strcmp(inj, "resident_skew") == 0) dcr.inject = 2u;
                    dcr.first_ticks = c->world > 1 ? 500000000ull : 0ull;
                    const char *fa = getenv("QS_FAST_ALLOC");
                    dcr.all_alloc = c->zero_alloc == 0 && !(fa && fa[0] == '0') ? 1u : 0u;
                    c->last_res_path = (!norm && rgeo.k32 ? 1 : 0) |
                                       (!norm && !(c->dc.feat & kFeatRes) && dcr.all_alloc ? 2 : 0);
                    static const bool rdiag_on = getenv("QS_RES_DIAG") && (getenv("QS_RES_DIAG")[0] == '1' ||
                                                                             getenv("QS_RES_DIAG")[0] == '2');
                    dcr.sel_diag = getenv("QS_RES_DIAG") && getenv("QS_RES_DIAG")[0] == '1' ? 1u : 0u;
                    uint64_t *rdiag = nullptr;
                    if (rdiag_on) {
                        c->diag.ensure(1024);
                        rdiag = c->diag.as<uint64_t>();
                        HIPCHK(hipMemsetAsync(rdiag, 0, 1024, c->stream));
                    }
                    kt.begin(3, c->stream);
                    HIPCHK(launch_la_stream_res(c->dt, dp, dx, dcr, P, rgeo, L0, c->clists.as<uint64_t>(),
                                                (uint32_t)lwords, (uint32_t)rcw, c->npart.as<uint4>(),
                                                c->normi.as<NormInfo>(), c->nstat.as<uint32_t>(),
                                                c->nfall.as<unsigned long long>(), on, ok,
                                                st, c->resctl.p, sel, rdiag, rsh, c->stream));
                    kt.end(3, c->stream);
                    if (rdiag) {
                        uint64_t h[128] = {0};
                        HIPCHK(hipMemcpyAsync(h, rdiag, 1024, hipMemcpyDeviceToHost, c->stream));
                        HIPCHK(hipStreamSynchronize(c->stream));
                        const double nw = h[3] ? (double)h[3] : 1.0;
                        fprintf(stderr, "QS_RES_DIAG resolver %.3f us per window; windows whose lists were not prefetched %llu of %llu (selectors %u)\n",
                                h[1] * 0.01 / nw, (unsigned long long)h[4], (unsigned long long)h[3], sel);
                        if (h[2])
                            fprintf(stderr, "QS_RES_DIAG selector 0: done seen %.2f us, its task finished %.2f us after "
                                            "the resolver's start of the window it overlaps (%llu windows)\n",
                                    h[13] * 0.01 / (double)h[2], h[14] * 0.01 / (double)h[2], (unsigned long long)h[2]);
                        {
                            std::vector<double> fin;
                            for (uint32_t k = 0; k < std::min(sel, 64u); ++k)
                                if (h[64 + k]) fin.push_back(h[64 + k] * 0.01);
                            std::sort(fin.begin(), fin.end());
                            if (!fin.empty()) {
                                fprintf(stderr, "QS_RES_DIAG selectors' mean finish (us after window start), sorted:");
                                for (double v : fin) fprintf(stderr, " %.1f", v);
                                fprintf(stderr, "\n");
                            }
                        }
                        if (h[36] + h[37] + h[38])
                            fprintf(stderr, "QS_RES_DIAG B3 -> B1 busy (ns per window, without the B1 wait): D %.0f, A %.0f, "
                                            "C %.0f\n", h[38] * 10.0 / nw, h[37] * 10.0 / nw, h[36] * 10.0 / nw);
                        if (h[33])
                            fprintf(stderr, "QS_RES_DIAG last list of a window published %.2f us after the start of "
                                            "the window before it (%llu windows; after 13 us %llu, after 15 us %llu)\n",
                                    h[32] * 0.01 / (double)h[33], (unsigned long long)h[33],
                                    (unsigned long long)h[34], (unsigned long long)h[35]);
                        if (h[6])
                            fprintf(stderr, "QS_RES_DIAG prefetch check: %llu windows short of lists, %.2f lists missing "
                                            "on average\n", (unsigned long long)h[6], (double)h[5] / (double)h[6]);
                        if (h[27] + h[28] + h[29] + h[30] + h[31])
                            fprintf(stderr, "QS_RES_DIAG window boundary (ns per window, wave D): bookkeeping %.0f "
                                            "-> B2 %.0f -> B3 %.0f -> B1 %.0f -> pod 0 decided %.0f\n",
                                    h[27] * 10.0 / nw, h[28] * 10.0 / nw, h[29] * 10.0 / nw, h[30] * 10.0 / nw,
                                    h[31] * 10.0 / nw);
                        if (h[19])
                            fprintf(stderr, "QS_RES_DIAG selector task (us): scoring %.2f chunk top-L %.2f publish/merge %.2f (tasks %llu, merges %llu)\n",
                                    h[16] * 0.01 / (double)h[19], h[17] * 0.01 / (double)h[19], h[18] * 0.01 / (double)h[19],
                                    (unsigned long long)h[19], (unsigned long long)h[20]);
                        if (h[12])
                            fprintf(stderr, "QS_RES_DIAG busy cycles/step: D %.0f A %.0f B %.0f C %.0f (steps %llu)\n",
                                    h[8] / (double)h[12], h[9] / (double)h[12], h[10] / (double)h[12],
                                    h[11] / (double)h[12], (unsigned long long)h[12]);
                        if (h[12])
                            fprintf(stderr, "QS_RES_DIAG step marks: D argmax %.0f | A pub+reads %.0f applied %.0f | C reads %.0f keyC %.0f loads %.0f\n",
                                    h[26] / (double)h[12], h[21] / (double)h[12], h[22] / (double)h[12],
                                    h[23] / (double)h[12], h[24] / (double)h[12], h[25] / (double)h[12]);
                    }
                } else if (use_graph) {
                    std::vector<uint8_t> key;
                    auto put = [&](const void *p, size_t nb) {
                        key.insert(key.end(), (const uint8_t *)p, (const uint8_t *)p + nb);
                    };
                    const void *ptrs[] = {c->dt.rows, c->dt.wrows, c->dt.masks, L0, C0, dio, st, (void *)c->comm, dp, dx,
                                          c->npart.p, c->normi.p, c->nfall.p};
                    put(ptrs, sizeof ptrs);
                    put(&c->dt.n, sizeof c->dt.n);
                    put(&c->dc, sizeof c->dc);
                    put(&geo, sizeof geo);
                    put(&overlap, sizeof overlap);
                    if (!s->gexec || s->gkey != key) {
                        if (s->gexec) (void)hipGraphExecDestroy(s->gexec);
                        s->gexec = nullptr;
                        HIPCHK(hipStreamBeginCapture(c->stream, hipStreamCaptureModeThreadLocal));
                        capturing = true;
                        try {
                            enqueue();
                        } catch (...) {
                            hipGraph_t g = nullptr;
                            (void)hipStreamEndCapture(c->stream, &g);
                            if (g) (void)hipGraphDestroy(g);
                            throw;
                        }
                        hipGraph_t g = nullptr;
                        HIPCHK(hipStreamEndCapture(c->stream, &g));
                        const hipError_t ie = hipGraphInstantiate(&s->gexec, g, nullptr, nullptr, 0);
                        (void)hipGraphDestroy(g);
                        HIPCHK(ie);
                        s->gkey = key;
                    }
                    HIPCHK(hipGraphLaunch(s->gexec, c->stream));
                } else {
                    enqueue();
                }
                batches = nwin;
                if (getenv("QS_HOSTTIME"))
                    fprintf(stderr, "QS_HOSTTIME enqueue %.3f ms for %u windows (overlap %d)\n",
                            std::chrono::duration<double>(std::chrono::steady_clock::now() - th0).count() * 1e3,
                            nwin, (int)overlap);
                if (diag_on) {
                    uint64_t h[16] = {0};
                    HIPCHK(hipMemcpyAsync(h, diag, 128, hipMemcpyDeviceToHost, c->stream));
                    HIPCHK(hipStreamSynchronize(c->stream));
                    const double np = h[5] ? (double)h[5] : 1.0;
                    fprintf(stderr, geo.waves == 1 ? "QS_DIAG resolve cycles/pod: cand %.0f issue %.0f fresh %.0f wmax %.0f commit %.0f (pods %llu, G=%u E=%u epl=%u)\n"
                                                   : "QS_DIAG resolve4 busy cycles/pod: D %.0f A %.0f B %.0f C %.0f (C row wait %.0f) (pods %llu, G=%u E=%u epl=%u)\n",
                            h[0] / np, h[1] / np, h[2] / np, h[3] / np, h[4] / np,
                            (unsigned long long)h[5], geo.G, geo.E, geo.epl);
                    if (geo.waves == 4)
                        fprintf(stderr, "QS_DIAG resolve4 pre-score cycles/pod: A %.0f C %.0f; per window: prologue %.0f epilogue %.0f\n",
                                h[6] / np, h[7] / np, h[8] / (double)nwin, h[9] / (double)nwin);
                }
            }
        }
        HIPCHK(hipEventRecord(e1, c->stream));
        HIPCHK(hipEventSynchronize(e1));
        float ms = 0.f;
        HIPCHK(hipEventElapsedTime(&ms, e0, e1));
        (void)hipEventDestroy(e0);
        (void)hipEventDestroy(e1);
        uint64_t rescans = 0, resumed = 0;
        if (eng == QS_ENGINE_LOOKAHEAD && c->last_waits) {
            uint64_t w = 0;
            HIPCHK(hipMemcpy(&w, c->hand.as<uint64_t>() + 2, 8, hipMemcpyDeviceToHost));
            if (inject_once(c, "handoff", kInjHandoff)) w = 1;
            if (w) {
                if (c->last_resident) {
                    ++c->res_timeouts;
                    c->res_cooldown = true;
                } else if (!c->mbox_on) {
                    c->handoff_off = true;
                }
                if (c->mbox_on && !c->comm) c->mbox_broken = true;
                fail(QS_ETIMEOUT, c->mbox_on ? "mailbox exchange timed out (a peer never posted its window)"
                                             : c->last_resident
                                                   ? "resident lookahead stream timed out (a hand-off never arrived); "
                                                     "the next run uses per-window launches"
                                                   : "lookahead window hand-off timed out (lists never published); "
                                                     "the context falls back to stream events");
            }
        }
        if (eng == QS_ENGINE_LOOKAHEAD && c->last_resident) c->res_timeouts = 0;
        if (eng == QS_ENGINE_LOOKAHEAD && c->nfall.p) {
            uint64_t h[2] = {0, 0};
            HIPCHK(hipMemcpy(h, c->nfall.p, 16, hipMemcpyDeviceToHost));
            rescans = h[0];
            resumed = h[1];
            if (getenv("QS_NORM_DIAG"))
                fprintf(stderr, "QS_NORM_DIAG rescans %llu resumed windows %llu\n", (unsigned long long)h[0],
                        (unsigned long long)h[1]);
        }
        c->mirror_stale = true;
        if (eng != QS_ENGINE_SCAN) c->soa_valid = false;
        kt.finish();
        maybe_inject_fault(c, "stream_run");
        sync_mirror(c);
        s->ran = true;
        s->mode_ran = (int)mode;
        s->epoch_after = ++c->table_epoch;
        if (stats) {
            std::memset(stats, 0, sizeof(*stats));
            for (int k = 0; k < 4; k++) {
                stats->kernel_s[k] = kt.secs[k];
                stats->kernel_launches[k] = kt.count[k];
            }
            stats->pods = P;
            stats->evals = (uint64_t)P * n;
            stats->wall_s = ms * 1e-3;
            stats->batches = batches;
            stats->truncations = rescans;
            stats->engine_used = eng;
            stats->table_layout = c->wide ? 1 : 0;
            stats->resumed_windows = resumed;
            stats->resident = (eng == QS_ENGINE_LOOKAHEAD && c->last_resident) ? 1 : 0;
            stats->resident_path = stats->resident ? c->last_res_path : 0;
            stats->device_faults = c->device_faults;
        }
    });
}

qs_status qs_stream_results(qs_ctx *c, qs_stream *s, int32_t *placement, uint64_t *best_key) {
    return guarded(c, [&] {
        if (!s || !s->ran) fail(QS_ESTATE, "stream has not run");
        HIPCHK(hipSetDevice(c->device));
        const uint32_t P = s->p;
        std::vector<int32_t> node(P);
        std::vector<uint64_t> key(P);
        if (P) {
            HIPCHK(hipMemcpyAsync(node.data(), s->d_node.p, 4 * (size_t)P, hipMemcpyDeviceToHost, c->stream));
            HIPCHK(hipMemcpyAsync(key.data(), s->d_key.p, 8 * (size_t)P, hipMemcpyDeviceToHost, c->stream));
            HIPCHK(hipStreamSynchronize(c->stream));
        }
        for (uint32_t k = 0; k < P; k++) {
            const uint32_t j = s->order[k];
            if (placement) placement[j] = node[k];
            if (best_key) best_key[j] = key[k];
        }
    });
}

qs_status qs_stream_free(qs_ctx *c, qs_stream *s) {
    (void)c;
    if (s && s->owner) {
        std::lock_guard<std::mutex> lk(s->owner->mu);
        auto &v = s->owner->streams;
        v.erase(std::remove(v.begin(), v.end(), s), v.end());
    }
    delete s;
    return QS_OK;
}

qs_status qs_table_save(qs_ctx *c) {
    return guarded(c, [&] {
        if (!c->dev_valid) fail(QS_ESTATE, "no node table loaded");
        HIPCHK(hipSetDevice(c->device));
        sync_mirror(c);
        c->tbl_saved.ensure(c->tbl.bytes);
        HIPCHK(hipMemcpyAsync(c->tbl_saved.p, c->tbl.p, c->tbl.bytes, hipMemcpyDeviceToDevice, c->stream));
        HIPCHK(hipStreamSynchronize(c->stream));
        c->m_saved = c->m;
        c->saved_wide = c->wide;
        c->saved_shift = c->shift;
        c->saved = true;
    });
}

qs_status qs_table_restore(qs_ctx *c) {
    return guarded(c, [&] {
        if (!c->saved || !c->dev_valid || c->tbl_saved.bytes != c->tbl.bytes || c->saved_wide != c->wide ||
            c->saved_shift != c->shift)
            fail(QS_ESTATE, "no matching qs_table_save snapshot");
        HIPCHK(hipSetDevice(c->device));
        HIPCHK(hipMemcpyAsync(c->tbl.p, c->tbl_saved.p, c->tbl.bytes, hipMemcpyDeviceToDevice, c->stream));
        c->m = c->m_saved;
        c->zero_alloc = count_zero_alloc(c->m);
        c->mirror_stale = false;
        ++c->table_epoch;
        c->soa_valid = false;
    });
}

qs_status qs_schedule_stream(qs_ctx *c, const qs_pod *pods, uint32_t p, qs_mode mode,
                             int32_t *placement, qs_stats *stats) {
    using clk = std::chrono::steady_clock;
    auto t0 = clk::now();
    qs_stream *s = nullptr;
    qs_status st = qs_stream_prepare(c, pods, p, &s);
    if (st != QS_OK) return st;
    auto t1 = clk::now();
    qs_stats local{};
    st = qs_stream_run(c, s, mode, &local);
    if (st != QS_OK) { qs_stream_free(nullptr, s); return st; }
    auto t2 = clk::now();
    st = qs_stream_results(c, s, placement, nullptr);
    if (st == QS_OK && c->cfg.record_timestamps && p > 1) {
        std::vector<uint64_t> stamps(p);
        if (hipMemcpy(stamps.data(), s->d_stamp.p, 8 * (size_t)p, hipMemcpyDeviceToHost) == hipSuccess)
            percentile_stats(stamps, &local);
    }
    auto t3 = clk::now();
    for (uint32_t j = 0; j < p && st == QS_OK; j++) {
        if (placement[j] >= 0) local.placed++;
        else local.unschedulable++;
    }
    qs_status st2 = qs_stream_free(c, s);
    if (st == QS_OK) st = st2;
    local.h2d_s = std::chrono::duration<double>(t1 - t0).count();
    local.d2h_s = std::chrono::duration<double>(t3 - t2).count();
    if (stats) *stats = local;
    return st;
}

size_t qs_struct_size(int which) {
    switch (which) {
        case 0: return sizeof(qs_config);
        case 1: return sizeof(qs_node_soa);
        case 2: return sizeof(qs_node_row);
        case 3: return sizeof(qs_pod);
        case 4: return sizeof(qs_container);
        case 5: return sizeof(qs_stats);
        case 6: return sizeof(qs_scoring_strategy);
        default: return 0;
    }
}

static qs_status fit_errors(qs_ctx *c, qs_stream *s, const uint32_t *pods, uint32_t mreq, uint32_t *counts,
                            uint32_t *tcounts) {
    return guarded(c, [&] {
        if (!s || !s->ran) fail(QS_ESTATE, "stream has not run");
        if (s->mode_ran != QS_MODE_EXACT) fail(QS_EINVAL, "FitError diagnosis covers exact streams");
        if (s->epoch_after != c->table_epoch) fail(QS_ESTATE, "the node table changed after the stream's run");
        if (mreq && (!pods || !counts)) fail(QS_EINVAL, "null pods / counts");
        const uint32_t P = s->p;
        for (uint32_t q = 0; q < mreq; q++)
            if (pods[q] >= P) fail(QS_EINVAL, "pod index out of range");
        std::memset(counts, 0, sizeof(uint32_t) * QS_FIT_REASONS * (size_t)mreq);
        if (tcounts) std::memset(tcounts, 0, sizeof(uint32_t) * 64 * (size_t)mreq);
        if (!mreq) return;
        HIPCHK(hipSetDevice(c->device));
        sync_mirror(c);
        std::vector<int32_t> node(P);
        if (P) HIPCHK(hipMemcpy(node.data(), s->d_node.p, 4 * (size_t)P, hipMemcpyDeviceToHost));
        std::vector<std::vector<uint32_t>> want(P);
        std::vector<uint32_t> pos_of(P);
        for (uint32_t k = 0; k < P; k++) pos_of[s->order[k]] = k;
        for (uint32_t q = 0; q < mreq; q++) want[pos_of[pods[q]]].push_back(q);
        Mirror m = c->m;
        for (uint32_t k = 0; k < P; k++)
            if (node[k] >= 0) mirror_reserve(m, (uint32_t)node[k], s->pods[s->order[k]], -1);
        const bool taint = c->cfg.enable_taint != 0, aff = c->cfg.enable_affinity != 0;
        auto subset = [](const uint64_t *mask, const uint64_t *bits) {
            return (mask[0] & ~bits[0]) == 0 && (mask[1] & ~bits[1]) == 0;
        };
        for (uint32_t k = 0; k < P; k++) {
            const qs_pod &p = s->pods[s->order[k]];
            if (node[k] < 0 && !want[k].empty()) {
                uint32_t cnt[QS_FIT_REASONS] = {0};
                uint32_t tcnt[64] = {0};
                const bool any_req = p.req_cpu || p.req_mem || p.req_ext[0] || p.req_ext[1];
                for (uint32_t i = 0; i < m.n; i++) {
                    if (taint && (m.th[i] & ~p.tol_hard) != 0) {
                        ++cnt[QS_FIT_TAINT];
                        ++tcnt[__builtin_ctzll(m.th[i] & ~p.tol_hard)];
                        continue;
                    }
                    if (aff) {
                        const uint64_t *lb = &m.lb[2 * (size_t)i];
                        bool ok = subset(p.sel, lb);
                        if (ok && p.n_req_terms > 0) {
                            bool one = false;
                            for (int t = 0; t < p.n_req_terms; t++) one = one || subset(p.req_terms[t], lb);
                            ok = one;
                        }
                        if (!ok) { ++cnt[QS_FIT_AFFINITY]; continue; }
                    }
                    if (m.np[i] + 1 > m.mp[i]) ++cnt[QS_FIT_TOO_MANY_PODS];
                    if (!any_req) continue;
                    if (p.req_cpu > 0 && p.req_cpu > m.ac[i] - m.rc[i]) ++cnt[QS_FIT_CPU];
                    if (p.req_mem > 0 && p.req_mem > m.am[i] - m.rm[i]) ++cnt[QS_FIT_MEMORY];
                    for (int e = 0; e < QS_MAX_EXT; e++) {
                        const int64_t q = p.req_ext[e];
                        if (q != 0 && q > m.ae[(size_t)i * QS_MAX_EXT + e] - m.re[(size_t)i * QS_MAX_EXT + e])
                            ++cnt[QS_FIT_EXT0 + e];
                    }
                }
                for (uint32_t q : want[k]) {
                    std::memcpy(counts + (size_t)q * QS_FIT_REASONS, cnt, sizeof cnt);
                    if (tcounts) std::memcpy(tcounts + (size_t)q * 64, tcnt, sizeof tcnt);
                }
            }
            if (node[k] >= 0) mirror_reserve(m, (uint32_t)node[k], p, +1);
        }
    });
}

qs_status qs_stream_fit_errors(qs_ctx *c, qs_stream *s, const uint32_t *pods, uint32_t mreq, uint32_t *counts) {
    return fit_errors(c, s, pods, mreq, counts, nullptr);
}

qs_status qs_stream_fit_taints(qs_ctx *c, qs_stream *s, const uint32_t *pods, uint32_t mreq, uint32_t *counts,
                               uint32_t *taint_counts) {
    if (!taint_counts && mreq) return QS_EINVAL;
    return fit_errors(c, s, pods, mreq, counts, taint_counts);
}

qs_status qs_stream_stamps(qs_ctx *c, qs_stream *s, uint64_t *stamps) {
    return guarded(c, [&] {
        if (!s || !s->ran || !s->d_stamp.p) fail(QS_ESTATE, "no timestamps recorded");
        HIPCHK(hipMemcpy(stamps, s->d_stamp.p, 8 * (size_t)s->p, hipMemcpyDeviceToHost));
    });
}

}
```

### custom-k8s-scheduler_amd/csrc/qs_kernels.hip

```cpp
#include "qs_kernels.hpp"

namespace qs {

__global__ __launch_bounds__(256) void k_rows_to_soa(DevTable t) {
    const uint32_t i = blockIdx.x * 256 + threadIdx.x;
    if (i >= t.n) return;
    const DRow r = t.rows[i];
    t.soa.c[kSAc][i] = r.ac; t.soa.c[kSAm][i] = r.am; t.soa.c[kSRc][i] = r.rc; t.soa.c[kSRm][i] = r.rm;
    t.soa.c[kSZc][i] = r.zc; t.soa.c[kSZm][i] = r.zm; t.soa.c[kSNp][i] = r.np; t.soa.c[kSMp][i] = r.mp;
    t.soa.c[kSAe0][i] = r.ae0; t.soa.c[kSRe0][i] = r.re0; t.soa.c[kSAe1][i] = r.ae1; t.soa.c[kSRe1][i] = r.re1;
}

__global__ void k_batch_init(uint32_t *ctrl, uint32_t *bidx, uint32_t P, uint32_t B) {
    const uint32_t nb = min(P, B);
    if (threadIdx.x < nb) bidx[threadIdx.x] = threadIdx.x;
    if (threadIdx.x == 0) { ctrl[0] = nb; ctrl[1] = nb; }
}

hipError_t launch_batch_init(uint32_t *ctrl, uint32_t *bidx, uint32_t P, uint32_t B, hipStream_t stream) {
    hipLaunchKernelGGL(k_batch_init, dim3(1), dim3(64), 0, stream, ctrl, bidx, P, B);
    return hipGetLastError();
}

hipError_t batch_claim_prepare() {
    QS_RET(batch_claim_prepare_f<kFeatExt>());
    return wide_batch_claim_prepare();
}

size_t batch_claim_lds(uint32_t n) {
    return batch_claim_lds_bytes(n);
}

hipError_t launch_batch_claim(const DevTable &t, const void *pods, const uint64_t *lists, uint32_t *ctrl,
                              uint32_t *bidx, uint32_t P, uint32_t B, int32_t *on, uint64_t *ok,
                              hipStream_t stream) {
    const size_t lds = batch_claim_lds(t.n);
    if (lds > 160 * 1024) return hipErrorInvalidValue;
    if (t.wrows) return wide_batch_claim(t, pods, lists, ctrl, bidx, P, B, on, ok, lds, stream);
    return batch_claim_f<kFeatExt>(t, pods, lists, ctrl, bidx, P, B, on, ok, lds, stream);
}

__global__ void k_set_row(DevTable t, uint32_t i, HostRow v, uint32_t feat) {
    (void)feat;
    set_row(t, i, v);
}

static uint32_t feat_class(uint32_t feat) {
    return feat == 0 ? 0u : (feat == kFeatExt ? kFeatExt : (kFeatExt | kFeatTaint | kFeatAffinity));
}

hipError_t launch_persistent(const DevTable &t, const void *pods, const DPodX *podx, uint32_t P,
                             const DevCfg &c, int32_t *on, uint64_t *ok, uint64_t *st,
                             hipStream_t stream) {
    if (c.feat & kFeatStrat)
        return t.wrows ? strat_wide_persistent(t, pods, podx, P, c, on, ok, st, stream)
                       : strat_compact_persistent(t, pods, podx, P, c, on, ok, st, stream);
    if (c.feat & kFeatRes)
        return t.wrows ? res_wide_persistent(t, pods, podx, P, c, on, ok, st, stream)
                       : res_compact_persistent(t, pods, podx, P, c, on, ok, st, stream);
    if (t.wrows) return wide_persistent(t, pods, podx, P, c, on, ok, st, stream);
    switch (feat_class(c.feat)) {
        case 0: return persistent_f<0>(t, pods, podx, P, c, on, ok, st, stream);
        case kFeatExt: return persistent_f<kFeatExt>(t, pods, podx, P, c, on, ok, st, stream);
        default:
            return persistent_f<kFeatExt | kFeatTaint | kFeatAffinity>(t, pods, podx, P, c, on, ok,
                                                                         st, stream);
    }
}

uint32_t persistent_max_nodes(uint32_t feat) {
    if (feat & kFeatStrat)
        return (feat & kFeatWide) ? strat_wide_persistent_max_nodes(feat) : strat_compact_persistent_max_nodes(feat);
    if (feat & kFeatRes)
        return (feat & kFeatWide) ? res_wide_persistent_max_nodes(feat) : res_compact_persistent_max_nodes(feat);
    if (feat & kFeatWide) return wide_persistent_max_nodes(feat);
    switch (feat_class(feat)) {
        case 0: return persistent_cap<0>();
        case kFeatExt: return persistent_cap<kFeatExt>();
        default: return persistent_cap<kFeatExt | kFeatTaint | kFeatAffinity>();
    }
}

hipError_t launch_rows_to_soa(const DevTable &t, hipStream_t stream) {
    if (!t.soa.c[0] || t.n == 0 || !t.rows) return hipSuccess;
    hipLaunchKernelGGL(k_rows_to_soa, dim3((t.n + 255) / 256), dim3(256), 0, stream, t);
    return hipGetLastError();
}

hipError_t launch_scan_pod(const DevTable &t, const void *pods, const DPodX *podx, uint32_t s,
                           const DevCfg &c, void *scratch, int32_t *on, uint64_t *ok, uint64_t *st,
                           uint8_t *feas, int32_t *score, int32_t *total, int part,
                           hipStream_t stream) {
    if (c.feat & kFeatStrat)
        return t.wrows ? strat_wide_scan_pod(t, pods, podx, s, c, scratch, on, ok, st, feas, score, total, part, stream)
                       : strat_compact_scan_pod(t, pods, podx, s, c, scratch, on, ok, st, feas, score, total, part, stream);
    if (c.feat & kFeatRes)
        return t.wrows ? res_wide_scan_pod(t, pods, podx, s, c, scratch, on, ok, st, feas, score, total, part, stream)
                       : res_compact_scan_pod(t, pods, podx, s, c, scratch, on, ok, st, feas, score, total, part, stream);
    if (t.wrows) return wide_scan_pod(t, pods, podx, s, c, scratch, on, ok, st, feas, score, total, part, stream);
    switch (feat_class(c.feat)) {
        case 0: return scan_pod_f<0>(t, pods, podx, s, c, scratch, on, ok, st, feas, score, total, part, stream);
        case kFeatExt: return scan_pod_f<kFeatExt>(t, pods, podx, s, c, scratch, on, ok, st, feas, score, total, part, stream);
        default:
            return scan_pod_f<kFeatExt | kFeatTaint | kFeatAffinity>(t, pods, podx, s, c, scratch, on, ok, st, feas, score, total, part, stream);
    }
}

size_t scan_scratch_bytes() { return sizeof(ScanScratch); }

uint32_t score_pod1_max_nodes() { return kScorePod1Max; }
size_t score_pod1_pack_bytes(uint32_t n) { return score_pack_bytes(n); }
hipError_t launch_score_pod1(const DevTable &t, const void *pod, const DPodX *podx, const DevCfg &c, uint8_t *hout,
                             uint64_t *gs, uint64_t seq, uint32_t pidx, const HostRow &prow, hipStream_t stream) {
    if (c.feat & kFeatStrat)
        return t.wrows ? strat_wide_score_pod1(t, pod, podx, c, hout, gs, seq, pidx, prow, stream)
                       : strat_compact_score_pod1(t, pod, podx, c, hout, gs, seq, pidx, prow, stream);
    if (c.feat & kFeatRes)
        return t.wrows ? res_wide_score_pod1(t, pod, podx, c, hout, gs, seq, pidx, prow, stream)
                       : res_compact_score_pod1(t, pod, podx, c, hout, gs, seq, pidx, prow, stream);
    if (t.wrows) return wide_score_pod1(t, pod, podx, c, hout, gs, seq, pidx, prow, stream);
    switch (feat_class(c.feat)) {
        case 0: return score_pod1_f<0>(t, pod, podx, c, hout, gs, seq, pidx, prow, stream);
        case kFeatExt: return score_pod1_f<kFeatExt>(t, pod, podx, c, hout, gs, seq, pidx, prow, stream);
        default:
            return score_pod1_f<kFeatExt | kFeatTaint | kFeatAffinity>(t, pod, podx, c, hout, gs, seq, pidx, prow, stream);
    }
}

__global__ void k_ready_set(uint64_t *ready, uint64_t value) {
    if (threadIdx.x == 0) __hip_atomic_store(ready, value, __ATOMIC_RELEASE, __HIP_MEMORY_SCOPE_AGENT);
}
hipError_t launch_ready_set(uint64_t *ready, uint64_t value, hipStream_t stream) {
    hipLaunchKernelGGL(k_ready_set, dim3(1), dim3(64), 0, stream, ready, value);
    return hipGetLastError();
}

hipError_t launch_la_window(const DevTable &t, const void *pods, const DPodX *podx, uint32_t s0,
                            uint32_t P, const DevCfg &c, const LaGeom &geo, const LaBufs &bf,
                            int32_t *on, uint64_t *ok, uint64_t *st, uint64_t *diag,
                            hipStream_t stream, int part) {
    if (bf.dprev && geo.waves == 1 && !(c.feat & kFeatNorm)) return hipErrorInvalidValue;
    if ((c.feat & kFeatNorm) && diag && geo.waves != 4) return hipErrorInvalidValue;
    if (c.feat & kFeatStrat)
        return t.wrows ? strat_wide_la_window(t, pods, podx, s0, P, c, geo, bf, on, ok, st, diag, stream, part)
                       : strat_compact_la_window(t, pods, podx, s0, P, c, geo, bf, on, ok, st, diag, stream, part);
    if (c.feat & kFeatRes)
        return t.wrows ? res_wide_la_window(t, pods, podx, s0, P, c, geo, bf, on, ok, st, diag, stream, part)
                       : res_compact_la_window(t, pods, podx, s0, P, c, geo, bf, on, ok, st, diag, stream, part);
    if (t.wrows) return wide_la_window(t, pods, podx, s0, P, c, geo, bf, on, ok, st, diag, stream, part);
    if (c.feat & kFeatNorm)
        return la_window_f<kFeatExt | kFeatTaint | kFeatAffinity>(t, pods, podx, s0, P, c, geo, bf, on, ok, st, diag, stream, part);
    if (c.feat & kFeatExt) return la_window_f<kFeatExt>(t, pods, podx, s0, P, c, geo, bf, on, ok, st, diag, stream, part);
    return la_window_f<0>(t, pods, podx, s0, P, c, geo, bf, on, ok, st, diag, stream, part);
}

LaGeom la_stream_res_plan(const LaGeom &geo, uint32_t feat, uint32_t n, uint32_t cus, uint32_t per_cu) {
    LaGeom r = geo;
    r.G = 0;
    const uint32_t fl = feat & ~(kFeatWide | kFeatRes | kFeatStrat);
    const bool fit = fl == 0 || fl == kFeatExt;
    const bool norm = (feat & kFeatNorm) != 0 && geo.K <= kResNormK;
    const bool shard_ok = geo.W == 1 ? geo.nv == 1 && geo.epl == 1
                                     : geo.nv == 1 && geo.K <= 32 && geo.W * geo.L <= (uint32_t)kResBS;
    if (!((fit || norm) && shard_ok && geo.waves == 4 && geo.L <= 64 && n > 0 && cus > geo.K)) return r;
    n = (n + geo.W - 1) / geo.W;
    const bool two = per_cu >= 2 && fit;
    const uint32_t gmax = std::min(two ? 16u : 8u, ((two ? 2u : 1u) * cus - 1) / geo.K);
    if (gmax == 0) return r;
    constexpr uint32_t bs = kResBS;
    static const uint32_t gwant = getenv("QS_RES_G") ? (uint32_t)std::max(0, atoi(getenv("QS_RES_G"))) : 0u;
    const uint32_t gsmall = std::min((cus - 1) / geo.K, (n + 3 * bs - 1) / (3 * bs));
    const uint32_t G0 = std::min(gmax, std::max({gwant, gsmall, (n + 5 * bs - 1) / (5 * bs)}));
    const uint32_t e_need = ((n + G0 - 1) / G0 + bs - 1) / bs;
    uint32_t E = 0;
    for (uint32_t e : {3u, 5u, 7u, 8u, 16u})
        if (e >= e_need) { E = e; break; }
    if (E == 0) return r;
    const uint32_t G = (n + E * bs - 1) / (E * bs);
    const uint32_t e2 = G * geo.L <= bs ? 1u : 2u;
    if (G * geo.L > e2 * bs || (e2 == 2 && (!two || E == 3))) return r;
    r.e2 = e2;
    r.E = E;
    r.chunk = E * bs;
    r.G = G;
    return r;
}
size_t la_stream_res_ctl_bytes() { return kResCtlBytes; }

uint32_t la_stream_res_max_blocks(const LaGeom &geo, uint32_t feat, uint32_t n, uint32_t cus) {
    const int per = (feat & kFeatStrat) ? ((feat & kFeatWide) ? strat_wide_la_stream_res_per_cu(geo, feat, n)
                                                              : strat_compact_la_stream_res_per_cu(geo, feat, n))
                    : (feat & kFeatRes)   ? ((feat & kFeatWide) ? res_wide_la_stream_res_per_cu(geo, feat, n)
                                                              : res_compact_la_stream_res_per_cu(geo, feat, n))
                    : (feat & kFeatWide)  ? wide_la_stream_res_per_cu(geo, feat, n)
                    : (feat & kFeatNorm)  ? la_stream_res_per_cu<kFeatExt | kFeatTaint | kFeatAffinity>(geo, n)
                    : (feat & kFeatExt) ? la_stream_res_per_cu<kFeatExt>(geo, n)
                                        : la_stream_res_per_cu<0>(geo, n);
    const int sgpr_waves = 800 / (((int)kResSgprMax + 15) / 16 * 16 + 16);
    const int safe = std::min(per, sgpr_waves / (kResBS / 64 / 4));
    return (uint32_t)std::max(0, safe) * cus;
}

hipError_t launch_la_stream_res(const DevTable &t, const void *pods, const DPodX *podx, const DevCfg &c, uint32_t P,
                                const LaGeom &geo, uint64_t *lists0, uint64_t *clists0, uint32_t lwords,
                                uint32_t cwords, uint4 *npart, NormInfo *norm, uint32_t *stat, unsigned long long *nfall,
                                int32_t *on, uint64_t *ok, uint64_t *st, void *ctl, uint32_t sel_blocks, uint64_t *rdiag,
                                const ResShard &rsh, hipStream_t stream) {
    if (geo.G == 0 || (uint64_t)t.n * (t.wrows ? sizeof(DRowW) : sizeof(DRow)) >= (1ull << 31))
        return hipErrorInvalidValue;
    if (c.feat & kFeatStrat)
        return (t.wrows ? strat_wide_la_stream_res : strat_compact_la_stream_res)(
            t, pods, podx, c, P, geo, lists0, clists0, lwords, cwords, npart, norm, stat, nfall, on, ok, st, ctl,
            sel_blocks, rdiag, rsh, stream);
    if (c.feat & kFeatRes)
        return (t.wrows ? res_wide_la_stream_res : res_compact_la_stream_res)(
            t, pods, podx, c, P, geo, lists0, clists0, lwords, cwords, npart, norm, stat, nfall, on, ok, st, ctl,
            sel_blocks, rdiag, rsh, stream);
    if (t.wrows)
        return wide_la_stream_res(t, pods, podx, c, P, geo, lists0, clists0, lwords, cwords, npart, norm, stat, nfall, on,
                                  ok, st, ctl, sel_blocks, rdiag, rsh, stream);
    if (c.feat & kFeatNorm)
        return la_stream_res_f<kFeatExt | kFeatTaint | kFeatAffinity>(t, pods, podx, c, P, geo, lists0, clists0, lwords,
                                                                      cwords, npart, norm, stat, nfall, on, ok, st, ctl,
                                                                      sel_blocks, rdiag, rsh, stream);
    if (c.feat & kFeatExt)
        return la_stream_res_f<kFeatExt>(t, pods, podx, c, P, geo, lists0, clists0, lwords, cwords, npart, norm, stat,
                                         nfall, on, ok, st, ctl, sel_blocks, rdiag, rsh, stream);
    return la_stream_res_f<0>(t, pods, podx, c, P, geo, lists0, clists0, lwords, cwords, npart, norm, stat, nfall, on,
                              ok, st, ctl, sel_blocks, rdiag, rsh, stream);
}

LaGeom la_geometry(uint32_t n, uint32_t K, uint32_t W, uint32_t L) {
    static const uint32_t Es[] = {1, 2, 3, 4, 5, 6, 8, 10, 12, 16};
    static const char *env_e = getenv("QS_LA_E");
    const uint32_t e_target = env_e ? (uint32_t)std::max(1, atoi(env_e)) : 5u;
    LaGeom g{};
    g.K = K;
    g.L = std::max(K, L);
    g.W = std::max(1u, W);
    g.v0 = 0;
    g.nv = g.W;
    if (g.W > 16 || g.L > 64) return g;
    const uint32_t ns = (n + g.W - 1) / g.W;
    const uint32_t gmax = 2048u / g.L;
    const uint32_t target = e_target * 256u;
    uint32_t G = std::max(1u, std::min(gmax, (ns + target - 1) / target));
    const uint32_t per = (ns + G - 1) / G;
    const uint32_t e_need = std::max(1u, (per + 255) / 256);
    uint32_t E = 0;
    for (uint32_t e : Es)
        if (e >= e_need) { E = e; break; }
    if (E == 0) return g;
    g.E = E;
    g.chunk = E * 256;
    G = std::max(1u, (ns + g.chunk - 1) / g.chunk);
    g.eplr = 1;
    g.lr = 0;
    g.epl = 1;
    while (g.epl < g.W) g.epl *= 2;
    g.G = G;
    return g;
}

}
```

### custom-k8s-scheduler_amd/csrc/qs_kernels.hpp

```cpp
#pragma once
#include <algorithm>
#include <cstring>

#include "qs_device.hpp"
#include "qs_launch.hpp"

#ifndef QS_EXP_HOOKS
#define QS_EXP_NORM_AB(norm) (norm)
#define QS_EXP_SLOT_KEY(act, r, q)
#define QS_EXP_CAND_KEY(f, tot, cr, p)
#define QS_EXP_PARK_RETURN()
#endif

#include "qs_key32.hpp"

namespace qs {

constexpr uint32_t kFeatNorm = kFeatTaint | kFeatAffinity;

template <int NPT, int BS, uint32_t F>
__global__ __launch_bounds__(BS) void k_persistent(DevTable t, const PodT<F> *__restrict__ pods,
                                                   const DPodX *__restrict__ podx, uint32_t P,
                                                   DevCfg c, int32_t *__restrict__ out_node,
                                                   uint64_t *__restrict__ out_key,
                                                   uint64_t *__restrict__ stamps) {
    constexpr int NW = BS / kWave;
    __shared__ uint64_t red[2][NW];
    __shared__ uint32_t redn[2][2][NW];
    const int tid = threadIdx.x, lane = tid & 63, w = tid >> 6;
    const uint32_t n = t.n;
    RowT<F> r[NPT];
    RowX x[NPT];
#pragma unroll
    for (int k = 0; k < NPT; ++k) {
        const uint32_t idx = tid + k * BS;
        if (idx < n) { r[k] = load_row<F>(t, idx); x[k] = load_rowx<F>(t, idx); }
        else { r[k] = empty_row<F>(); x[k] = RowX{0, 0, 0, 0, 0, 0, 0, 0}; }
    }
    PodT<F> pn = pods[0];
    for (uint32_t s = 0; s < P; ++s) {
        const PodT<F> p = pn;
        pn = pods[s + 1 < P ? s + 1 : s];
        DPodX px;
        if (F & kFeatNorm) px = podx[s];
        uint32_t mt = 0, ma = 0;
        double ymt = 0.0, yma = 0.0;
        if (F & kFeatNorm) {
            uint32_t lt = 0, la = 0;
#pragma unroll
            for (int k = 0; k < NPT; ++k) {
                const bool f = feasible<F>(r[k], x[k], p, px);
                const uint32_t a = f ? taint_raw(x[k], px) : 0u;
                const uint32_t b = f ? affinity_raw(x[k], p, px) : 0u;
                lt = a > lt ? a : lt;
                la = b > la ? b : la;
            }
            lt = wave_max_u32(lt);
            la = wave_max_u32(la);
            if (lane == 0) { redn[s & 1][0][w] = lt; redn[s & 1][1][w] = la; }
            __syncthreads();
#pragma unroll
            for (int i = 0; i < NW; ++i) {
                const uint32_t a = redn[s & 1][0][i], b = redn[s & 1][1][i];
                mt = a > mt ? a : mt;
                ma = b > ma ? b : ma;
            }
            ymt = rcp_exact(mt);
            yma = rcp_exact(ma);
        }
        uint64_t best = 0;
#pragma unroll
        for (int k = 0; k < NPT; ++k) {
            const bool f = feasible<F>(r[k], x[k], p, px);
            const uint32_t tot = node_total<F>(r[k], x[k], p, px, c, mt, ymt, ma, yma, nullptr);
            const uint64_t key = f ? pack_key(tot + 1, tid + k * BS) : 0ull;
            best = key > best ? key : best;
        }
        best = wave_max_u64(best);
        if (lane == 0) red[s & 1][w] = best;
        __syncthreads();
        uint64_t ks = 0;
#pragma unroll
        for (int i = 0; i < NW; ++i) {
            const uint64_t v = red[s & 1][i];
            ks = v > ks ? v : ks;
        }
        const uint32_t win = key_node(ks);
        if (ks != 0) {
#pragma unroll
            for (int k = 0; k < NPT; ++k)
                if (tid + k * BS == win) reserve(r[k], x[k], p, +1);
        }
        if (tid == 0) {
            out_node[s] = ks ? (int32_t)win : -1;
            if (out_key) out_key[s] = ks;
            if (stamps) stamps[s] = __builtin_amdgcn_s_memrealtime();
        }
    }
#pragma unroll
    for (int k = 0; k < NPT; ++k) {
        const uint32_t idx = tid + k * BS;
        if (idx < n) { store_dyn<F>(t, idx, r[k]); store_dynx<F>(t, idx, x[k]); }
    }
}

constexpr uint32_t kScanBlocksMax = 2048;
struct ScanScratch {
    unsigned long long best;
    uint32_t mt, ma;
    uint32_t lo, hi;
    uint64_t partial[kScanBlocksMax];
};
static_assert(offsetof(ScanScratch, lo) == offsetof(ScanHead, lo) && offsetof(ScanScratch, mt) == offsetof(ScanHead, mt),
              "ScanHead mirrors ScanScratch");

template <int BS>
__device__ __forceinline__ uint64_t block_max_u64(uint64_t v) {
    __shared__ uint64_t red[BS / kWave];
    v = wave_max_u64(v);
    if ((threadIdx.x & 63) == 0) red[threadIdx.x >> 6] = v;
    __syncthreads();
    uint64_t m = 0;
#pragma unroll
    for (int i = 0; i < BS / kWave; ++i) m = red[i] > m ? red[i] : m;
    return m;
}

template <uint32_t F>
__global__ __launch_bounds__(256) void k_scan_norm(DevTable t, const PodT<F> *__restrict__ pods,
                                                   const DPodX *__restrict__ podx, uint32_t s,
                                                   ScanScratch *sc) {
    const PodT<F> p = pods[s];
    const DPodX px = podx[s];
    uint32_t lt = 0, la = 0;
    const uint32_t lo = sc->lo, hi = sc->hi ? sc->hi : t.n;
    for (uint32_t i = lo + blockIdx.x * 256 + threadIdx.x; i < hi; i += gridDim.x * 256) {
        const RowT<F> r = load_row<F>(t, i);
        const RowX x = load_rowx<F>(t, i);
        if (feasible<F>(r, x, p, px)) {
            const uint32_t a = taint_raw(x, px), b = affinity_raw(x, p, px);
            lt = a > lt ? a : lt;
            la = b > la ? b : la;
        }
    }
    lt = wave_max_u32(lt);
    la = wave_max_u32(la);
    if ((threadIdx.x & 63) == 0) {
        if (lt) atomicMax(&sc->mt, lt);
        if (la) atomicMax(&sc->ma, la);
    }
}

template <uint32_t F>
__global__ __launch_bounds__(256) void k_scan_key(DevTable t, const PodT<F> *__restrict__ pods,
                                                  const DPodX *__restrict__ podx, uint32_t s,
                                                  DevCfg c, ScanScratch *sc, uint8_t *feas_out,
                                                  int32_t *score_out, int32_t *total_out) {
    const PodT<F> p = pods[s];
    DPodX px;
    uint32_t mt = 0, ma = 0;
    if (F & kFeatNorm) { px = podx[s]; mt = sc->mt; ma = sc->ma; }
    const double ymt = rcp_exact(mt), yma = rcp_exact(ma);
    uint64_t best = 0;
    const uint32_t lo = sc->lo, hi = sc->hi ? sc->hi : t.n;
    for (uint32_t i = lo + blockIdx.x * 256 + threadIdx.x; i < hi; i += gridDim.x * 256) {
        const RowT<F> r = load_row<F>(t, i);
        const RowX x = load_rowx<F>(t, i);
        const bool f = feasible<F>(r, x, p, px);
        uint32_t sco[4];
        const uint32_t tot = node_total<F>(r, x, p, px, c, mt, ymt, ma, yma, score_out ? sco : nullptr);
        const uint64_t key = f ? pack_key(tot + 1, i) : 0ull;
        best = key > best ? key : best;
        if (feas_out) feas_out[i] = f;
        if (total_out) total_out[i] = f ? (int32_t)tot : -1;
        if (score_out) {
#pragma unroll
            for (int q = 0; q < 4; ++q) score_out[4 * (size_t)i + q] = f ? (int32_t)sco[q] : 0;
        }
    }
    best = block_max_u64<256>(best);
    if (threadIdx.x == 0) sc->partial[blockIdx.x] = best;
}

__device__ __forceinline__ int4 soa_quad(const int32_t *col, uint32_t q) {
    return __builtin_bit_cast(int4, __builtin_nontemporal_load(reinterpret_cast<const u32x4 *>(col) + q));
}

template <uint32_t F>
__global__ __launch_bounds__(256) void k_scan_soa(DevTable t, const PodT<F> *__restrict__ pods,
                                                  uint32_t s, DevCfg c, ScanScratch *sc,
                                                  uint8_t *feas_out, int32_t *score_out,
                                                  int32_t *total_out) {
    const PodT<F> p = pods[s];
    const DPodX px{};
    const uint32_t nq = (t.n + 3) / 4;
    uint64_t best = 0;
    const uint32_t stride = gridDim.x * 256;
    for (uint32_t q0 = blockIdx.x * 256 + threadIdx.x; q0 < nq; q0 += 2 * stride) {
        int4 cols[2][kSCols];
#pragma unroll
        for (int h = 0; h < 2; ++h) {
            const uint32_t qh = min(q0 + h * stride, nq - 1);
#pragma unroll
            for (int k = 0; k < 8; ++k) cols[h][k] = soa_quad(t.soa.c[k], qh);
            if (F & kFeatExt) {
#pragma unroll
                for (int k = 8; k < kSCols; ++k) cols[h][k] = soa_quad(t.soa.c[k], qh);
            }
        }
#pragma unroll
        for (int h = 0; h < 2; ++h) {
        const uint32_t q = q0 + h * stride;
        if (q >= nq) break;
        const int4 *col = cols[h];
#pragma unroll
        for (int e = 0; e < 4; ++e) {
            auto el = [&](int k) { return e == 0 ? col[k].x : e == 1 ? col[k].y : e == 2 ? col[k].z : col[k].w; };
            RowT<F> r;
            r.ac = el(kSAc); r.am = el(kSAm); r.rc = el(kSRc); r.rm = el(kSRm);
            r.zc = el(kSZc); r.zm = el(kSZm); r.np = el(kSNp); r.mp = el(kSMp);
            r.yc = r.ac ? rcp_int(r.ac) : 0.0;
            r.ym = r.am ? rcp_int(r.am) : 0.0;
            RowX x{};
            if (F & kFeatExt) { x.ae0 = el(kSAe0); x.re0 = el(kSRe0); x.ae1 = el(kSAe1); x.re1 = el(kSRe1); }
            const uint32_t idx = 4 * q + e;
            const bool f = feasible<F>(r, x, p, px);
            uint32_t sco[4];
            const uint32_t tot = node_total<F>(r, x, p, px, c, 0, 0.0, 0, 0.0, score_out ? sco : nullptr);
            const uint64_t key = f ? pack_key(tot + 1, idx) : 0ull;
            best = key > best ? key : best;
            if (idx < t.n) {
                if (feas_out) feas_out[idx] = f;
                if (total_out) total_out[idx] = f ? (int32_t)tot : -1;
                if (score_out) {
#pragma unroll
                    for (int k = 0; k < 4; ++k) score_out[4 * (size_t)idx + k] = f ? (int32_t)sco[k] : 0;
                }
            }
        }
        }
    }
    best = block_max_u64<256>(best);
    if (threadIdx.x == 0) sc->partial[blockIdx.x] = best;
}

template <uint32_t F>
__global__ __launch_bounds__(256) void k_scan_commit(DevTable t, const PodT<F> *__restrict__ pods,
                                                     uint32_t s, uint32_t nblk, ScanScratch *sc,
                                                     int32_t *out_node, uint64_t *out_key,
                                                     uint64_t *stamps) {
    uint64_t v = 0;
    for (uint32_t i = threadIdx.x; i < nblk; i += 256) v = sc->partial[i] > v ? sc->partial[i] : v;
    const uint64_t ks = nblk ? block_max_u64<256>(v) : sc->best;
    if (threadIdx.x != 0) return;
    if (nblk && !out_node) {
        sc->best = ks > sc->best ? ks : sc->best;
        return;
    }
    sc->best = nblk ? ks : 0ull;
    sc->mt = 0;
    sc->ma = 0;
    if (!out_node) return;
    const PodT<F> p = pods[s];
    if (ks) {
        const uint32_t w = key_node(ks);
        RowT<F> r = load_row<F>(t, w);
        RowX x = load_rowx<F>(t, w);
        reserve(r, x, p, +1);
        store_dyn<F>(t, w, r);
        store_dynx<F>(t, w, x);
        if (t.soa.c[0]) {
            t.soa.c[kSRc][w] = r.rc; t.soa.c[kSRm][w] = r.rm;
            t.soa.c[kSZc][w] = r.zc; t.soa.c[kSZm][w] = r.zm;
            t.soa.c[kSNp][w] = r.np;
            if (F & kFeatExt) { t.soa.c[kSRe0][w] = x.re0; t.soa.c[kSRe1][w] = x.re1; }
        }
    }
    out_node[s] = ks ? (int32_t)key_node(ks) : -1;
    if (out_key) out_key[s] = ks;
    if (stamps) stamps[s] = __builtin_amdgcn_s_memrealtime();
}

__device__ __forceinline__ void set_row(const DevTable &t, uint32_t i, const HostRow &v) {
    t.masks[i] = DMask{v.th, v.ts, v.lb0, v.lb1};
    if (t.zone) t.zone[i] = v.zone;
    if (t.wrows) {
        DRowW w;
        w.ac = v.ac; w.rc = v.rc; w.zc = v.zc; w.np = v.np;
        w.am = v.wam; w.rm = v.wrm; w.zm = v.wzm; w.ym = v.ym;
        w.yc = v.yc; w.mp = v.mp; w.pad = 0;
        w.ae0 = v.ae0; w.re0 = v.re0; w.ae1 = v.ae1; w.re1 = v.re1;
        t.wrows[i] = w;
        return;
    }
    DRow r;
    r.ac = v.ac; r.am = v.am; r.rc = v.rc; r.rm = v.rm; r.zc = v.zc; r.zm = v.zm;
    r.np = v.np; r.mp = v.mp; r.yc = v.yc; r.ym = v.ym;
    r.ae0 = v.ae0; r.re0 = v.re0; r.ae1 = v.ae1; r.re1 = v.re1;
    t.rows[i] = r;
    if (t.soa.c[0]) {
        const int32_t f[kSCols] = {v.ac, v.am, v.rc, v.rm, v.zc, v.zm, v.np, v.mp, v.ae0, v.re0, v.ae1, v.re1};
#pragma unroll
        for (int k = 0; k < kSCols; ++k) t.soa.c[k][i] = f[k];
    }
}
// ... 2705 lines not shown
            const uint32_t nidx = e ? knode(e) : 0u;
            return (dirty[nidx >> 5] >> (nidx & 31)) & 1u;
        };
        for (uint32_t w = 0; w < nwin; ++w) {
            const uint32_t s0 = w * K, kend = min(K, P - s0);
            const PodT<F> *wp = wpods2[w & 1];
            if (*late) {
                ++nfallback;
                const uint64_t *lists = lists0 + (size_t)(w & 1) * lwords;
                if (lane == 0) (void)res_wait_ge(&ctl->rdy[w & 1][0], (w >> 1) * K + kend, c.werr, res_bound(c, w));
                __builtin_amdgcn_fence(__ATOMIC_ACQUIRE, "wavefront");
                uint64_t e[3];
#pragma unroll
                for (uint32_t j = 0; j < 3; ++j)
                    e[j] = j < kend ? load_coh_u64(lists + (size_t)j * 64 + lane) : 0ull;
#pragma unroll
                for (uint32_t j = 0; j < 3; ++j) ringE[(s0 + j) % kResRing][lane] = kconv(e[j]);
                const uint32_t n0 = e[0] ? key_node(e[0]) : 0u;
                ringR[s0 % kResRing][lane] = load_row<F>(t, n0);
                if (F & kFeatExt) {
                    const RowX x = load_rowx<F>(t, n0);
                    ringX[s0 % kResRing][lane] = make_int4(x.ae0, x.re0, x.ae1, x.re1);
                }
            }
            const KT e0 = ringE[s0 % kResRing][lane];
            c1 = (e0 != 0 && !dirty_bit(e0)) ? e0 : (KT)0;
            C1[1][lane] = c1;
            if (w > 0) bmark(0);
            __syncthreads();
            PodT<F> pcur = wp[0];
            for (uint32_t i = 0; i < kend; ++i) {
                QS_RSTAMP_BEGIN()
                const uint32_t g = s0 + i;
                const int par = i & 1;
                const KT en = ringE[(g + 1) % kResRing][lane];
                const RowT<F> r1 = ringR[g % kResRing][lane];
                RowX x1{};
                if (F & kFeatExt) {
                    const int4 e = ringX[g % kResRing][lane];
                    x1.ae0 = e.x; x1.re0 = e.y; x1.ae1 = e.z; x1.re1 = e.w;
                }
                const PodT<F> pn1 = wp[i + 1];
                const uint32_t en_node = en ? knode(en) : 0u;
                const uint32_t dword = dirty[en_node >> 5];
                QS_RSTAMP_MARK(0)
                RowT<F> cr = r1;
                RowX crx = x1;
                reserve(cr, crx, pcur, +1);
                const bool f = feasible<F>(cr, crx, pn1, px);
                const uint32_t tot = fit_bal_total<F, FA>(cr, crx, pn1, cv);
                QS_EXP_CAND_KEY(f, tot, cr, pn1)
                QS_RSTAMP_MARK(1)
                if (i + 1 < kend) {
                    if constexpr (R32) keyC[par][lane] = (c1 != 0 && f) ? (k32_score(tot + 1) | (c1 & kK32NodeMask)) : 0u;
                    else keyC[par][lane] = (c1 != 0 && f) ? pack_key(tot + 1, key_node(c1)) : 0ull;
                    const bool dirt = ((dword >> (en_node & 31)) & 1u) != 0;
                    c1 = (en != 0 && !dirt) ? en : (KT)0;
                    C1[par][lane] = c1;
                }
                QS_RSTAMP_MARK(2)
                pcur = pn1;
                QS_RSTAMP_END()
                __syncthreads();
            }
            __syncthreads();
            __syncthreads();
            bmark(-1);
        }
        if (rdiag && lane == 0) { rdiag[4] = nfallback; rdiag[5] = 0; rdiag[6] = 0; }
        };
        if constexpr (kFastAllocClass) {
            if (fast_alloc) role_c(std::integral_constant<bool, true>{});
            else role_c(std::integral_constant<bool, false>{});
        } else {
            role_c(std::integral_constant<bool, false>{});
        }
    } else if (!NORM && wv == 4) {
        uint64_t ein = 0;
        bool skip = true;
        for (uint32_t w = 0; w < nwin; ++w) {
            const uint32_t s0 = w * K, kend = min(K, P - s0);
            const bool hasnext = w + 1 < nwin;
            const uint32_t knext = hasnext ? min(K, P - s0 - K) : 0u;
            const uint64_t *lists = lists0 + (size_t)(w & 1) * lwords;
            const uint64_t *listsn = lists0 + (size_t)((w + 1) & 1) * lwords;
            const uint32_t tnext = ((w + 1) >> 1) * K + knext;
            const bool pfw = hasnext && kend >= 6;
            const uint32_t ic = pfw ? kend - 3 : kend - 1;
            bool lt = hasnext;
            uint32_t rdyv = 0;
            __syncthreads();
            for (uint32_t i = 0; i < kend; ++i) {
                const uint32_t g = s0 + i;
                if (!(skip && i == 0)) ringE[(g + 2) % kResRing][lane] = kconv(ein);
                if (i == ic) {
                    if (pfw) lt = !((uint32_t)__builtin_amdgcn_readfirstlane(rdyv) >= tnext);
                    if (lane == 0) *late = lt ? 1u : 0u;
                }
                uint64_t v = 0;
                if (i + 3 < kend) {
                    v = load_coh_u64(lists + (size_t)(i + 3) * 64 + lane);
                } else if (i >= ic && !lt && hasnext) {
                    const uint32_t j = i + 3 - kend;
                    v = load_coh_u64(listsn + (size_t)min(j, knext - 1) * 64 + lane);
                    v = j < knext ? v : 0ull;
                }
                ein = v;
                if (pfw && i + 4 == kend) rdyv = load_coh_u32(&ctl->rdy[(w + 1) & 1][0]);
                __syncthreads();
            }
            skip = lt;
            __syncthreads();
            __syncthreads();
        }
    } else if (!NORM && wv == 5) {
        for (uint32_t w = 0; w < nwin; ++w) {
            const uint32_t s0 = w * K, kend = min(K, P - s0);
            const bool hasnext = w + 1 < nwin;
            const bool pfw = hasnext && kend >= 6;
            __syncthreads();
            for (uint32_t i = 0; i < kend; ++i) {
                const uint32_t g = s0 + i;
                const bool go = i + 1 < kend || (pfw ? *late == 0u : !hasnext);
                if (go) {
                    const KT e = ringE[(g + 1) % kResRing][lane];
                    const uint32_t nd = e ? knode(e) : 0u;
                    const RowT<F> r = load_row<F>(t, nd);
                    ringR[(g + 1) % kResRing][lane] = r;
                    if (F & kFeatExt) {
                        const RowX x = load_rowx<F>(t, nd);
                        ringX[(g + 1) % kResRing][lane] = make_int4(x.ae0, x.re0, x.ae1, x.re1);
                    }
                }
                __syncthreads();
            }
            __syncthreads();
            __syncthreads();
        }
    } else if constexpr (NORM) {
        constexpr uint32_t q = sizeof(DPodX) / 16;
        const uint32_t pw = (uint32_t)(wv - 4);
        uint32_t ndi = 0;
        for (uint32_t w = 0; w < nwin; ++w) {
            const uint32_t s0 = w * K, kend = min(K, P - s0);
            const uint32_t knext = w + 1 < nwin ? min(K, P - s0 - K) : 0u;
            const uint32_t wb = w & 1, nb = (w + 1) & 1;
            const PodT<F> *wp = wpods2[wb];
            const uint32_t id0 = pw * 64 + lane, id1 = id0 + 256;
            const bool h0 = id0 < knext * q, h1 = id1 < knext * q;
            const int4 *src = reinterpret_cast<const int4 *>(podx + (size_t)s0 + K);
            int4 q0 = make_int4(0, 0, 0, 0), q1 = make_int4(0, 0, 0, 0);
            if (h0) q0 = src[id0];
            if (h1) q1 = src[id1];
            uint32_t nfl = 0;
            if (pw == 0 && (uint32_t)lane < knext) nfl = pods[s0 + K + lane].flags;
            const uint32_t qq = (uint32_t)lane & 31u;
            const bool mycur = wv == 4 && lane < 32;
            DPodX myx{};
            uint32_t myf = 0;
            auto load_mine = [&]() {
                myx = mycur ? wpodx2[wb][qq] : wpodx2[nb][qq];
                myf = mycur ? wp[qq].flags : nflag2[nb][qq];
            };
            auto new_slot = [&](uint32_t j, bool cur) {
                QS_EXP_PARK_RETURN()
                const ResPub pv = read_pub(&pub[j & 1]);
                if (pv.ks == 0 || pv.slot >= 0) return;
                const RowX sx = stagexN[j & 1][pv.src];
                const uint32_t l = pv.nd_old;
                if (lane == 0) smask[l] = DMask{sx.th, sx.ts, sx.lb0, sx.lb1};
                const uint32_t st = static_raw(sx.th, sx.ts, sx.lb0, sx.lb1, myf, myx);
                if (lane < 32) {
                    if (cur && qq >= j + 3 && qq < kend) Tcur[qq * kResTStride + l] = st;
                } else if (qq < knext) {
                    Tnext[qq * kResTStride + l] = st;
                }
            };
            auto inherited = [&](uint32_t j) {
                QS_EXP_PARK_RETURN()
                const uint32_t l = 2 * j + (lane < 32 ? 0u : 1u);
                if (l < ndi && qq < knext) {
                    const RowX sx = carryxN[l];
                    Tnext[qq * kResTStride + l] = static_raw(sx.th, sx.ts, sx.lb0, sx.lb1, myf, myx);
                }
            };
            auto rescan_tail = [&](uint32_t j, uint64_t ks) {
                const uint32_t W = ks ? key_node(ks) : 0u;
                const bool slot = __ballot((uint32_t)lane < *snd && sidx[lane] == W) != 0;
                if (!ks || slot) return;
                const int pj = j & 1;
                const RowT<F> rw = load_row<F>(t, W);
                const RowX xw = load_rowx<F>(t, W);
                uint32_t st2 = 0;
                if (j + 2 < kend) st2 = static_raw(xw.th, xw.ts, xw.lb0, xw.lb1, wp[j + 2].flags, wpodx2[wb][j + 2]);
                if (lane == 0) {
                    stage[pj][0] = rw;
                    stagexN[pj][0] = xw;
                    stS[pj][0] = st2;
                }
                if (j + 1 < kend) {
                    RowT<F> cr = rw;
                    RowX crx = xw;
                    reserve(cr, crx, wp[j], +1);
                    const PodT<F> q1 = wp[j + 1];
                    const DPodX qx = wpodx2[wb][j + 1];
                    const NormInfo nf = wnorm2[wb][j + 1];
                    const double2 yr = wrcp2[wb][j + 1];
                    const bool f = feasible<F>(cr, crx, q1, qx);
                    const uint32_t tot = node_total<F>(cr, crx, q1, qx, cv, nf.mt, yr.x, nf.ma, yr.y, nullptr);
                    uint32_t fl = 0;
                    if (!f) {
                        if (F & kFeatTaint) fl |= taint_raw(crx, qx) == nf.mt ? 1u : 0u;
                        if (F & kFeatAffinity) fl |= affinity_raw(crx, q1, qx) == nf.ma ? 2u : 0u;
                    }
                    if (lane == 0) {
                        keyC[pj][0] = f ? pack_key(tot + 1, W) : 0ull;
                        flagC[pj][0] = fl;
                    }
                }
            };
            __syncthreads();
            __syncthreads();
            for (uint32_t i = 0; i < kend; ++i) {
                if (i == 0) {
                    int4 *dst = reinterpret_cast<int4 *>(&wpodx2[nb][0]);
                    if (h0) dst[id0] = q0;
                    if (h1) dst[id1] = q1;
                    if (pw == 0 && (uint32_t)lane < knext) nflag2[nb][lane] = nfl;
                } else if (wv == 4 || wv == 7) {
                    if (i == 1) load_mine();
                    if (wv == 4) new_slot(i - 1, true);
                    else inherited(i - 1);
                }
                __syncthreads();
                if (pub[i & 1].slot == -2) {
                    const uint64_t ks = rescan_pass(i, wb);
                    if (wv == 4) rescan_tail(i, ks);
                    __syncthreads();
                }
            }
            if ((wv == 4 || wv == 7) && kend == 1) load_mine();
            if (wv == 4) new_slot(kend - 1, false);
            if (wv == 7)
                for (uint32_t j = kend - 1; 2 * j < ndi; ++j) inherited(j);
            __syncthreads();
            for (uint32_t idx = id0; idx < knext * 64; idx += 256) {
                const uint32_t qq = idx >> 6, l = idx & 63u, r = xrank[l];
                if (r != 0xFFFFFFFFu) Tcur[qq * kResTStride + r] = Tnext[qq * kResTStride + l];
            }
            ndi = (uint32_t)__popcll(__ballot(xrank[lane] != 0xFFFFFFFFu));
            __syncthreads();
        }
    }
    if (kResDiag && rdiag && lane == 0 && wv < 4) {
        rdiag[8 + wv] = busy_;
        if (wv == 1) { rdiag[21] = sub_[0]; rdiag[22] = sub_[1]; }
        if (wv == 3) { rdiag[23] = sub_[0]; rdiag[24] = sub_[1]; rdiag[25] = sub_[2]; }
        if (wv == 0) rdiag[26] = sub_[0];
        if (wv == 0) rdiag[12] = steps_;
    }
    if (rdiag && lane == 0 && wv == 0)
        for (int k = 0; k < 5; ++k) rdiag[27 + k] = bseg_[k];
    if (rdiag && lane == 0 && wv == 0) rdiag[38] = bseg_[5];
    if (rdiag && lane == 0 && (wv == 1 || wv == 3)) rdiag[wv == 1 ? 37 : 36] = bseg_[0];
}
#undef QS_RSTAMP_BEGIN
#undef QS_RSTAMP_END

template <uint32_t F, int E, int E2, bool K32>
__global__ __launch_bounds__(kResBS) void k_la_stream_res(DevTable t, const PodT<F> *__restrict__ pods, DevCfg c,
                                                       uint32_t P, uint32_t K, uint32_t G, uint32_t L,
                                                       uint32_t chunk, uint32_t nwin, uint64_t *lists0,
                                                       uint64_t *clists0, uint32_t lwords, uint32_t cwords,
                                                       int32_t *__restrict__ out_node,
                                                       uint64_t *__restrict__ out_key,
                                                       uint64_t *__restrict__ stamps, ResCtl *ctl,
                                                       uint64_t *__restrict__ rdiag, const DPodX *__restrict__ podx,
                                                       uint4 *npart0, NormInfo *norm0, uint32_t *stat0,
                                                       unsigned long long *nfall, ResShard rsh) {
    if (blockIdx.x != 0) {
        res_selector<E, E2, F>(t, pods, c, P, K, G, L, chunk, nwin, lists0, clists0, lwords, cwords, ctl,
                               blockIdx.x - 1, gridDim.x - 1, rdiag, podx, npart0, norm0, stat0, rsh);
        return;
    }
    if (rsh.W > 1 && threadIdx.x == 0)
        for (uint32_t r = 0; r < rsh.W; ++r)
            __hip_atomic_store(reinterpret_cast<uint64_t *>(rsh.peers[r] + rsh.hello) + rsh.rank, rsh.seq,
                               __ATOMIC_RELEASE, __HIP_MEMORY_SCOPE_SYSTEM);
    extern __shared__ __attribute__((aligned(16))) uint32_t lds[];
    if ((F & kFeatNorm) == 0 && threadIdx.x >= 384) {
        __syncthreads();
        for (uint32_t w = 0; w < nwin; ++w)
            for (uint32_t j = 0, nb = min(K, P - w * K) + 3; j < nb; ++j) __syncthreads();
        return;
    }
    const uint64_t t0 = rdiag ? __builtin_amdgcn_s_memrealtime() : 0ull;
    la_resolve4_stream<F, K32>(lds, t, pods, c, P, K, nwin, lists0, lwords, out_node, out_key, stamps, ctl, rdiag,
                               podx, norm0, stat0, nfall);
    if (rdiag && threadIdx.x == 0) { rdiag[1] = __builtin_amdgcn_s_memrealtime() - t0; rdiag[3] = nwin; }
}

static hipError_t res_lds_attr(const void *fn, size_t lds4) {
    if (lds4 <= 64 * 1024) return hipSuccess;
    return hipFuncSetAttribute(fn, hipFuncAttributeMaxDynamicSharedMemorySize, (int)lds4);
}
template <uint32_t F>
static hipError_t la_stream_res_f(const DevTable &t, const void *pods, const DPodX *podx, const DevCfg &c, uint32_t P,
                                  const LaGeom &geo, uint64_t *lists0, uint64_t *clists0, uint32_t lwords,
                                  uint32_t cwords, uint4 *npart0, NormInfo *norm0, uint32_t *stat0,
                                  unsigned long long *nfall, int32_t *on, uint64_t *ok, uint64_t *st, void *ctl,
                                  uint32_t sel_blocks, uint64_t *rdiag, const ResShard &rsh, hipStream_t stream) {
    const uint32_t K = geo.K, G = geo.G, L = geo.L, nwin = (P + K - 1) / K;
    if (rsh.W > 1 && (rsh.W * L > (uint32_t)kResBS || K > 32 || rsh.W > 16 || !rsh.peers))
        return hipErrorInvalidValue;
    const uint32_t E2 = geo.e2;
    if (G * L > E2 * (uint32_t)kResBS || (E2 == 2 && (F & kFeatNorm))) return hipErrorInvalidValue;
    const size_t lds4 = res_stream_lds_bytes<F>(t.n, geo.k32 != 0);
    if (lds4 > kResLdsMax) return hipErrorInvalidValue;
    if ((F & kFeatNorm) && (K > kResNormK || sel_blocks < K * G || !podx || !npart0 || !norm0 || !stat0))
        return hipErrorInvalidValue;
    const dim3 grid(1 + sel_blocks);
    const PodT<F> *pp = (const PodT<F> *)pods;
    ResCtl *rc = (ResCtl *)ctl;
#define QS_RESK(EE, EE2, KK)                                                                                          \
    do {                                                                                                              \
    if (hipError_t ea = res_lds_attr((const void *)k_la_stream_res<F, EE, EE2, KK>, lds4); ea != hipSuccess) return ea; \
    hipLaunchKernelGGL((k_la_stream_res<F, EE, EE2, KK>), grid, dim3(kResBS), lds4, stream, t, pp, c, P, K, G, L,       \
                       geo.chunk, nwin, lists0, clists0, lwords, cwords, on, ok, st, rc, rdiag, podx, npart0, norm0,   \
                       stat0, nfall, rsh);                                                                       \
    } while (0)
#define QS_RESE(EE, EE2) \
    else if (geo.E == EE && E2 == EE2) { if (geo.k32) QS_RESK(EE, EE2, true); else QS_RESK(EE, EE2, false); }
#define QS_RESE2(EE) \
    else if (geo.E == EE && E2 == 2 && (F & kFeatNorm) == 0) { \
        if constexpr ((F & kFeatNorm) == 0) { if (geo.k32) QS_RESK(EE, 2, true); else QS_RESK(EE, 2, false); } }
    if (false) {
    }
    QS_RESE(3, 1) QS_RESE(5, 1) QS_RESE(7, 1) QS_RESE(8, 1) QS_RESE(16, 1)
    QS_RESE2(5) QS_RESE2(7) QS_RESE2(8) QS_RESE2(16)
    else return hipErrorInvalidValue;
#undef QS_RESE
#undef QS_RESE2
#undef QS_RESK
    return hipGetLastError();
}
constexpr size_t kResCtlBytes = sizeof(ResCtl);

template <uint32_t F>
static int la_stream_res_per_cu(const LaGeom &geo, uint32_t n) {
    const size_t lds4 = res_stream_lds_bytes<F>(n, geo.k32 != 0);
    const void *fn = nullptr;
#define QS_RESP(EE, KK) \
    if (geo.E == EE && geo.e2 == 1 && (geo.k32 != 0) == KK) fn = (const void *)k_la_stream_res<F, EE, 1, KK>;
    QS_RESP(3, true) QS_RESP(3, false) QS_RESP(5, true) QS_RESP(5, false) QS_RESP(7, true) QS_RESP(7, false)
    QS_RESP(8, true) QS_RESP(8, false) QS_RESP(16, true) QS_RESP(16, false)
#undef QS_RESP
    if constexpr ((F & kFeatNorm) == 0) {
#define QS_RESP2(EE, KK) \
        if (geo.E == EE && geo.e2 == 2 && (geo.k32 != 0) == KK) fn = (const void *)k_la_stream_res<F, EE, 2, KK>;
        QS_RESP2(5, true) QS_RESP2(5, false) QS_RESP2(7, true) QS_RESP2(7, false) QS_RESP2(8, true) QS_RESP2(8, false) QS_RESP2(16, true) QS_RESP2(16, false)
#undef QS_RESP2
    }
    int per = 0;
    if (!fn || res_lds_attr(fn, lds4) != hipSuccess ||
        hipOccupancyMaxActiveBlocksPerMultiprocessor(&per, fn, kResBS, lds4) != hipSuccess) {
        (void)hipGetLastError();
        return 0;
    }
    return per;
}

#ifdef QS_CLAIM_DIAG
static __device__ uint64_t g_claim_diag[5];
#define CLAIM_STAMP0() uint64_t cds[4] = {0, 0, 0, 0}; uint64_t ctp = diag_stamp();
#define CLAIM_STAMP(q) { const uint64_t t_ = diag_stamp(); cds[q] += t_ - ctp; ctp = t_; }
#else
#define CLAIM_STAMP0()
#define CLAIM_STAMP(q)
#endif
constexpr int kClaimWaves = 16;
constexpr uint32_t kClaimNonEmpty = 1u << 31;
constexpr uint32_t kClaimCarried = 64, kClaimNone = 65;
constexpr uint32_t kClLkey = 0, kClLnode = kClLkey + 64 * 64 * 8, kClLazb = kClLnode + 64 * 64 * 4,
                   kClAz = kClLazb + 64 * 64 * 4, kClPend = kClAz + kMaxApps * kMaxZones / 8, kClSrc = kClPend + 256,
                   kClPod = kClSrc + 256, kClNodes = kClPod + 512;
__host__ __device__ constexpr size_t batch_claim_lds_bytes(uint32_t n) {
    return kClNodes + (((size_t)n + 31) / 32 + 1 + 3) / 4 * 16;
}

template <uint32_t F>
__global__ __launch_bounds__(64 * kClaimWaves) void k_batch_claim(
    DevTable t, const PodT<F> *__restrict__ pods, const uint64_t *__restrict__ lists, uint32_t GLp,
    uint32_t *ctrl, uint32_t *bidx, uint32_t P, uint32_t B, int32_t *__restrict__ out_node,
    uint64_t *__restrict__ out_key) {
    extern __shared__ __attribute__((aligned(16))) uint32_t lds[];
    const int tid = threadIdx.x, lane = tid & 63, wv = tid >> 6;
    CLAIM_STAMP0();
    const uint32_t nwords = (t.n + 31) / 32, sent = nwords * 32;
    uint8_t *lb = reinterpret_cast<uint8_t *>(lds);
    uint64_t *lkey = reinterpret_cast<uint64_t *>(lb + kClLkey);
    uint32_t *lnode = reinterpret_cast<uint32_t *>(lb + kClLnode);
    uint32_t *lazb = reinterpret_cast<uint32_t *>(lb + kClLazb);
    uint32_t *claimed_az = reinterpret_cast<uint32_t *>(lb + kClAz);
    uint32_t *pend = reinterpret_cast<uint32_t *>(lb + kClPend);
    uint32_t *rsrc = reinterpret_cast<uint32_t *>(lb + kClSrc);
    uint32_t *lpod = reinterpret_cast<uint32_t *>(lb + kClPod);
    uint32_t *claimed = reinterpret_cast<uint32_t *>(lb + kClNodes);
    const uint32_t nb = ctrl[0], cursor = ctrl[1];
    for (uint32_t i = tid; i < nwords; i += 64 * kClaimWaves) claimed[i] = 0;
    if (tid == 0) claimed[nwords] = 0xFFFFFFFFu;
    for (uint32_t i = tid; i < kMaxApps * kMaxZones / 32; i += 64 * kClaimWaves) claimed_az[i] = 0;
    {
        constexpr int Q = 64 / kClaimWaves;
        uint64_t ev[Q];
        uint32_t fv[Q];
#pragma unroll
        for (int q = 0; q < Q; ++q) {
            const uint32_t i = (uint32_t)wv + kClaimWaves * q;
            ev[q] = i < nb ? lists[(size_t)i * GLp + lane] : 0ull;
            fv[q] = i < nb ? bidx[i] : 0u;
        }
        uint32_t sv[Q];
#pragma unroll
        for (int q = 0; q < Q; ++q) {
            sv[q] = fv[q];
            fv[q] = (uint32_t)wv + kClaimWaves * q < nb ? pods[sv[q]].flags : 0u;
        }
        uint32_t zv[Q];
#pragma unroll
        for (int q = 0; q < Q; ++q)
            zv[q] = (ev[q] && pod_aa(fv[q]) == 2u) ? (uint32_t)t.zone[key_node(ev[q])] : 0u;
#pragma unroll
        for (int q = 0; q < Q; ++q) {
            const uint32_t i = (uint32_t)wv + kClaimWaves * q;
            const bool ok = ev[q] != 0ull;
            lkey[i * 64 + lane] = ev[q];
            lnode[i * 64 + lane] = ok ? key_node(ev[q]) : sent;
            lazb[i * 64 + lane] = pod_app(fv[q]) * kMaxZones + (zv[q] & (kMaxZones - 1));
            const uint32_t ne = __ballot(ok) ? kClaimNonEmpty : 0u;
            if (lane == 0) { lpod[i] = sv[q]; lpod[64 + i] = fv[q] | ne; }
        }
    }
    __syncthreads();
    if (wv != 0) return;
    CLAIM_STAMP(0);
    uint32_t npend = 0;
    const uint32_t my_s = (uint32_t)lane < nb ? lpod[lane] : 0u;
    const uint32_t my_flags = lpod[64 + lane];
    CLAIM_STAMP(1);
    struct Ents {
        uint32_t node, azb;
    };
    auto ents = [&](uint32_t j) -> Ents {
        const uint32_t o = min(j, 63u) * 64 + (uint32_t)lane;
        return Ents{lnode[o], lazb[o]};
    };
    Ents sa = ents(0), sb = ents(1), sc{sent, 0u};
    uint32_t fl = (uint32_t)__builtin_amdgcn_readlane((int)my_flags, 0);
    uint64_t am;
    {
        uint32_t tk = (claimed[sa.node >> 5] >> (sa.node & 31)) & 1u;
        am = __ballot(tk == 0u);
    }
    auto step = [&](uint32_t i, const Ents &cur, const Ents &nxt, Ents &n2) {
        const uint32_t fl1 = (uint32_t)__builtin_amdgcn_readlane((int)my_flags, (int)min(i + 1, 63u));
        const bool aa = pod_aa(fl) == 2u, aa1 = pod_aa(fl1) == 2u;
        const uint32_t cw1 = claimed[nxt.node >> 5];
        const uint32_t aw1 = aa1 ? claimed_az[nxt.azb >> 5] : 0u;
        n2 = ents(i + 2);
        uint32_t w = 0xFFFFFFFFu, bw = 0xFFFFFFFFu;
        if (am) {
            const int src = __builtin_ctzll(am);
            w = (uint32_t)__builtin_amdgcn_readlane((int)cur.node, src);
            if (aa) bw = (uint32_t)__builtin_amdgcn_readlane((int)cur.azb, src);
            if (lane == 0) {
                __hip_atomic_fetch_or(&claimed[w >> 5], 1u << (w & 31), __ATOMIC_RELAXED,
                                      __HIP_MEMORY_SCOPE_WORKGROUP);
                if (aa)
                    __hip_atomic_fetch_or(&claimed_az[bw >> 5], 1u << (bw & 31), __ATOMIC_RELAXED,
                                          __HIP_MEMORY_SCOPE_WORKGROUP);
                rsrc[i] = (uint32_t)src;
            }
        } else if (fl & kClaimNonEmpty) {
            if (lane == 0) {
                pend[npend] = (uint32_t)__builtin_amdgcn_readlane((int)my_s, (int)i);
                rsrc[i] = kClaimCarried;
            }
            ++npend;
        } else if (lane == 0) {
            rsrc[i] = kClaimNone;
        }
        uint32_t tk = (cw1 >> (nxt.node & 31)) & 1u;
        if (aa1) tk |= ((aw1 >> (nxt.azb & 31)) & 1u) | ((aa && nxt.azb == bw) ? 1u : 0u);
        am = __ballot(tk == 0u && nxt.node != w);
        fl = fl1;
    };
    uint32_t i = 0;
    for (; i + 2 < nb; i += 3) {
        step(i, sa, sb, sc);
        step(i + 1, sb, sc, sa);
        step(i + 2, sc, sa, sb);
    }
    if (i < nb) step(i, sa, sb, sc);
    if (i + 1 < nb) step(i + 1, sb, sc, sa);
    CLAIM_STAMP(2);
    int32_t my_node = -2;
    uint64_t my_key = 0;
    if ((uint32_t)lane < nb) {
        const uint32_t r = rsrc[lane];
        if (r < 64u) {
            my_key = lkey[(uint32_t)lane * 64 + r];
            my_node = (int32_t)key_node(my_key);
        } else {
            my_node = r == kClaimCarried ? -2 : -1;
        }
    }
    if ((uint32_t)lane < nb && my_node != -2) {
        const uint32_t s = my_s;
        if (my_node >= 0) {
            const PodT<F> p = pods[s];
            const uint32_t w = (uint32_t)my_node;
            RowT<F> r = load_row<F>(t, w);
            RowX x = load_rowx<F>(t, w);
            reserve(r, x, p, +1);
            store_dyn<F>(t, w, r);
            store_dynx<F>(t, w, x);
            if (t.apps) {
                const uint32_t app = pod_app(p.flags);
                atomicOr(&t.apps[(size_t)(app >> 5) * t.cap + w], 1u << (app & 31));
                atomicAdd(&t.zcount[app * kMaxZones + (uint32_t)t.zone[w]], 1);
            }
        }
        out_node[s] = my_node;
        if (out_key) out_key[s] = my_key;
    }
    const uint32_t take = min(B - npend, P - cursor);
    if ((uint32_t)lane < npend) bidx[lane] = pend[lane];
    else if ((uint32_t)lane < npend + take) bidx[lane] = cursor + (uint32_t)lane - npend;
    if (lane == 0) { ctrl[0] = npend + take; ctrl[1] = cursor + take; }
    CLAIM_STAMP(3);
#ifdef QS_CLAIM_DIAG
    if (lane == 0) {
        for (int q = 0; q < 4; ++q) atomicAdd((unsigned long long *)&g_claim_diag[q], (unsigned long long)cds[q]);
        const unsigned long long nbt = atomicAdd((unsigned long long *)&g_claim_diag[4], 1ull);
        if (npend + take == 0)
            printf("claim diag: batches %llu  stage %llu  setup %llu  walk %llu  apply %llu (clocks, totals)\n",
                   nbt + 1, (unsigned long long)g_claim_diag[0], (unsigned long long)g_claim_diag[1],
                   (unsigned long long)g_claim_diag[2], (unsigned long long)g_claim_diag[3]);
    }
#endif
}


#define QS_RET(x) do { hipError_t e_ = (x); if (e_ != hipSuccess) return e_; } while (0)

template <int NPT, int BS, uint32_t F>
static hipError_t persistent_t(const DevTable &t, const void *pods, const DPodX *podx, uint32_t P,
                               const DevCfg &c, int32_t *on, uint64_t *ok, uint64_t *st,
                               hipStream_t stream) {
    hipLaunchKernelGGL((k_persistent<NPT, BS, F>), dim3(1), dim3(BS), 0, stream, t,
                       (const PodT<F> *)pods, podx, P, c, on, ok, st);
    return hipGetLastError();
}

template <uint32_t F>
static constexpr uint32_t persistent_cap() {
    if (F & kFeatWide) return (F & kFeatNorm) ? 2048u : 5120u;
    return F == 0 ? 6144u : (F == kFeatExt ? 5120u : 2048u);
}

template <uint32_t F>
static hipError_t persistent_f(const DevTable &t, const void *pods, const DPodX *podx, uint32_t P,
                               const DevCfg &c, int32_t *on, uint64_t *ok, uint64_t *st,
                               hipStream_t stream) {
    const uint32_t n = t.n;
    if (n > persistent_cap<F>()) return hipErrorInvalidValue;
    if (n <= 64) return persistent_t<1, 64, F>(t, pods, podx, P, c, on, ok, st, stream);
    if (n <= 128) return persistent_t<1, 128, F>(t, pods, podx, P, c, on, ok, st, stream);
    if (n <= 256) return persistent_t<1, 256, F>(t, pods, podx, P, c, on, ok, st, stream);
    if (n <= 512) return persistent_t<1, 512, F>(t, pods, podx, P, c, on, ok, st, stream);
    if (n <= 1024) return persistent_t<1, 1024, F>(t, pods, podx, P, c, on, ok, st, stream);
    if (n <= 2048) return persistent_t<2, 1024, F>(t, pods, podx, P, c, on, ok, st, stream);
    if constexpr (persistent_cap<F>() > 2048) {
        if (n <= 3072) return persistent_t<3, 1024, F>(t, pods, podx, P, c, on, ok, st, stream);
        if (n <= 4096) return persistent_t<4, 1024, F>(t, pods, podx, P, c, on, ok, st, stream);
    }
    if constexpr (persistent_cap<F>() > 4096) {
        if (n <= 5120) return persistent_t<5, 1024, F>(t, pods, podx, P, c, on, ok, st, stream);
    }
    if constexpr (persistent_cap<F>() > 5120) {
        if (n <= 6144) return persistent_t<6, 1024, F>(t, pods, podx, P, c, on, ok, st, stream);
    }
    return hipErrorInvalidValue;
}

template <uint32_t F>
static hipError_t scan_pod_f(const DevTable &t, const void *pods_, const DPodX *podx, uint32_t s,
                             const DevCfg &c, void *scratch, int32_t *on, uint64_t *ok,
                             uint64_t *st, uint8_t *feas, int32_t *score, int32_t *total,
                             int part, hipStream_t stream) {
    const PodT<F> *pods = (const PodT<F> *)pods_;
    ScanScratch *sc = (ScanScratch *)scratch;
    constexpr bool kSoaOk = (F & (kFeatNorm | kFeatWide)) == 0;
    const bool soa = kSoaOk && t.soa.c[0];
    const uint32_t units = soa ? (t.n + 3) / 4 : t.n;
    uint32_t blocks = min(kScanBlocksMax, max(1u, (units + 255) / 256));
    if (part & 1) {
// ... 223 lines not shown
```

### custom-k8s-scheduler_amd/csrc/qs_launch.hpp

```cpp
#pragma once
#include <hip/hip_runtime.h>
#include <stddef.h>
#include <stdint.h>

namespace qs {

struct DevTable;
struct DevCfg;
struct DPodX;

struct HostRow {
    int32_t ac, am, rc, rm, zc, zm, np, mp;
    double yc, ym;
    int32_t ae0, re0, ae1, re1;
    uint64_t th, ts, lb0, lb1;
    int32_t zone, pad;
    double wam, wrm, wzm;
};

struct LaGeom {
    uint32_t K, L, G, E, chunk, epl, waves, k32;
    uint32_t W, v0, nv, eplr, lr;
    uint32_t e2 = 1;
};
struct LaShard {
    uint32_t W, v0, kw, pad;
    uint64_t RS;
};

hipError_t launch_persistent(const DevTable &t, const void *pods, const DPodX *podx, uint32_t P,
                             const DevCfg &c, int32_t *out_node, uint64_t *out_key,
                             uint64_t *stamps, hipStream_t stream);
uint32_t persistent_max_nodes(uint32_t feat);

hipError_t launch_scan_pod(const DevTable &t, const void *pods, const DPodX *podx, uint32_t s,
                           const DevCfg &c, void *scratch, int32_t *out_node, uint64_t *out_key,
                           uint64_t *stamps, uint8_t *feas, int32_t *score, int32_t *total,
                           int part, hipStream_t stream);
hipError_t launch_rows_to_soa(const DevTable &t, hipStream_t stream);
uint32_t score_pod1_max_nodes();
constexpr uint32_t kScoreInfeasible = 0xFFFFFFFFu;
size_t score_pod1_pack_bytes(uint32_t n);
hipError_t launch_score_pod1(const DevTable &t, const void *pod, const DPodX *podx, const DevCfg &c, uint8_t *hout,
                             uint64_t *gs, uint64_t seq, uint32_t pidx, const HostRow &prow, hipStream_t stream);
size_t scan_scratch_bytes();
struct ScanHead {
    unsigned long long best;
    uint32_t mt, ma, lo, hi;
};

LaGeom la_geometry(uint32_t n, uint32_t K, uint32_t W = 1, uint32_t L = 0);
struct NormInfo;
struct LaBufs {
    uint64_t *lists, *clists;
    uint4 *npart;
    NormInfo *norm;
    const uint32_t *dprev;
    uint32_t *dcur;
    unsigned long long *nfall;
    const uint32_t *pidx = nullptr, *pcount = nullptr;
    uint32_t *rec = nullptr;
    uint32_t *tickets = nullptr;
};
hipError_t launch_ready_set(uint64_t *ready, uint64_t value, hipStream_t stream);

LaGeom la_stream_res_plan(const LaGeom &geo, uint32_t feat, uint32_t n, uint32_t cus, uint32_t per_cu = 1);
size_t la_stream_res_ctl_bytes();
uint32_t la_stream_res_max_blocks(const LaGeom &geo, uint32_t feat, uint32_t n, uint32_t cus);
struct ResShard {
    uint32_t W, rank;
    uint64_t seq;
    char *const *peers;
    uint64_t hello, flags, lists;
    uint64_t nflags, norm;
};
hipError_t launch_la_stream_res(const DevTable &t, const void *pods, const DPodX *podx, const DevCfg &c, uint32_t P,
                                const LaGeom &geo, uint64_t *lists0, uint64_t *clists0, uint32_t lwords,
                                uint32_t cwords, uint4 *npart, NormInfo *norm, uint32_t *stat, unsigned long long *nfall, int32_t *on,
                                uint64_t *ok, uint64_t *st, void *ctl, uint32_t sel_blocks, uint64_t *rdiag,
                                const ResShard &rsh, hipStream_t stream);

hipError_t launch_la_window(const DevTable &t, const void *pods, const DPodX *podx, uint32_t s0,
                            uint32_t P, const DevCfg &c, const LaGeom &geo, const LaBufs &bufs,
                            int32_t *out_node, uint64_t *out_key, uint64_t *stamps, uint64_t *diag,
                            hipStream_t stream, int part);

hipError_t launch_batch_init(uint32_t *ctrl, uint32_t *bidx, uint32_t P, uint32_t B, hipStream_t stream);
size_t batch_claim_lds(uint32_t n);
hipError_t batch_claim_prepare();
hipError_t launch_batch_claim(const DevTable &t, const void *pods, const uint64_t *lists, uint32_t *ctrl,
                              uint32_t *bidx, uint32_t P, uint32_t B, int32_t *out_node,
                              uint64_t *out_key, hipStream_t stream);

__global__ void k_set_row(DevTable t, uint32_t i, HostRow v, uint32_t feat);

}
```

Baseline: 2.205 million pods/s.

## Make host mirror lazy via device snapshot tail kernel and reuse run resources

After each stream run, a small tail kernel writes the status words (handoff flag, rescan counters) and the dynamic node-table columns into a double-buffered pinned host snapshot. This replaces the blocking device-to-host memcpys and the per-run host loop that rebuilt the mirror from rows. The host mirror is now materialised lazily, only when a later API call needs it, and table restore becomes a pointer switch to the saved copy instead of a full copy. Timing events, a single zero-filled arena for resident-path memsets, and memoised LDS attribute and per-CU occupancy queries are reused across runs to cut per-call host overhead. The cost is extra state-tracking complexity, with a risk of the mirror going stale if the lazy bookkeeping is wrong.

```diff
diff --git a/custom-k8s-scheduler_amd/csrc/qs_ctx.hpp b/custom-k8s-scheduler_amd/csrc/qs_ctx.hpp
--- a/custom-k8s-scheduler_amd/csrc/qs_ctx.hpp
+++ b/custom-k8s-scheduler_amd/csrc/qs_ctx.hpp
@@ -9,6 +9,7 @@
 #include "../../include/qsched.h"
 #include "qs_device.hpp"
 #include "qs_launch.hpp"
+#include "qs_mirror_state.hpp"
 
 namespace qs_host {
 
@@ -55,26 +56,6 @@
     }
     template <class T>
     T *as() const { return (T *)p; }
-};
-
-struct Mirror {
-    uint32_t n = 0;
-    std::vector<int64_t> ac, am, mp, rc, rm, zc, zm, np;
-    std::vector<int64_t> ae, re;
-    std::vector<uint64_t> th, ts, lb;
-    std::vector<int32_t> zone;
-    std::vector<uint64_t> gen;
-    void resize(uint32_t nn) {
-        n = nn;
-        zone.assign(nn, 0);
-        for (auto *v : {&ac, &am, &mp, &rc, &rm, &zc, &zm, &np}) v->assign(nn, 0);
-        ae.assign((size_t)nn * QS_MAX_EXT, 0);
-        re.assign((size_t)nn * QS_MAX_EXT, 0);
-        th.assign(nn, 0);
-        ts.assign(nn, 0);
-        lb.assign((size_t)nn * 2, 0);
-        gen.assign(nn, 0);
-    }
 };
 
 inline int ctz64(int64_t v) { return v == 0 ? 64 : __builtin_ctzll((uint64_t)v); }
@@ -126,7 +107,10 @@
     bool saved = false;
     bool saved_wide = false;
     int saved_shift = 20;
-    bool mirror_stale = false;
+    qs_host::MirrorLazy lz;
+    hipEvent_t ev_run[2] = {nullptr, nullptr};
+    uint64_t tail_seq = 0;
+    qs_host::DevBuf res_arena;
     uint64_t device_faults = 0;
     qs_host::DevBuf diag;
     qs_host::DevBuf scratch, lists, clists, dio, npart, normi, nstat, nfall, nrec, bctrl, one_pod, one_podx;
@@ -138,7 +122,6 @@
     uint32_t pend = 0xFFFFFFFFu;
     qs_host::DevBuf hand;
     bool handoff_off = false;
-    qs_host::DevBuf resctl;
     int res_timeouts = 0;
     bool res_cooldown = false;
     uint32_t inject_used = 0;
diff --git a/custom-k8s-scheduler_amd/csrc/qs_host.cpp b/custom-k8s-scheduler_amd/csrc/qs_host.cpp
--- a/custom-k8s-scheduler_amd/csrc/qs_host.cpp
+++ b/custom-k8s-scheduler_amd/csrc/qs_host.cpp
@@ -260,7 +260,30 @@
     return d;
 }
 
+void materialise_mirror(qs_ctx *c) { mirror_materialise(c->lz, c->m, c->m_saved); }
+
+void ensure_snap(qs_ctx *c, uint32_t n) {
+    if (c->lz.snap[0] && c->lz.snap[1] && c->lz.snap_cap >= std::max<uint32_t>(n, 1)) return;
+    materialise_mirror(c);
+    c->lz.pending = false;
+    for (int b = 0; b < 2; ++b) {
+        if (c->lz.snap[b]) (void)hipHostFree(c->lz.snap[b]);
+        c->lz.snap[b] = nullptr;
+    }
+    c->lz.snap_cap = 0;
+    const uint32_t cap = std::max<uint32_t>(64, (n + 63) & ~63u);
+    for (int b = 0; b < 2; ++b) {
+        void *p = nullptr;
+        HIPCHK(hipHostMalloc(&p, snap_words(cap) * 8, hipHostMallocDefault));
+        std::memset(p, 0, snap_words(cap) * 8);
+        c->lz.snap[b] = static_cast<int64_t *>(p);
+    }
+    c->lz.snap_cap = cap;
+}
+
 void upload_table(qs_ctx *c) {
+    materialise_mirror(c);
+    ensure_snap(c, c->m.n);
     const uint32_t n = c->m.n;
     const uint32_t cap = std::max<uint32_t>(64, (n + 63) & ~63u);
     const bool wide = c->wide;
@@ -305,7 +328,6 @@
     HIPCHK(hipStreamSynchronize(c->stream));
     c->dev_valid = true;
     c->soa_valid = soa;
-    c->mirror_stale = false;
 }
 
 void ensure_soa(qs_ctx *c) {
@@ -327,42 +349,13 @@
     if (c->pend == 0xFFFFFFFFu) return;
     const uint32_t i = c->pend;
     c->pend = 0xFFFFFFFFu;
-    if (c->dev_valid && i < c->m.n) push_row(c, i, false);
-}
-
-void sync_mirror(qs_ctx *c) {
-    if (!c->mirror_stale || !c->dev_valid) return;
-    const uint32_t n = c->m.n;
-    Mirror &m = c->m;
-    if (c->wide) {
-        std::vector<DRowW> rows(n);
-        if (n) HIPCHK(hipMemcpyAsync(rows.data(), c->dt.wrows, n * sizeof(DRowW), hipMemcpyDeviceToHost, c->stream));
-        HIPCHK(hipStreamSynchronize(c->stream));
-        for (uint32_t i = 0; i < n; i++) {
-            m.rc[i] = rows[i].rc;
-            m.rm[i] = (int64_t)rows[i].rm;
-            m.zc[i] = rows[i].zc;
-            m.zm[i] = (int64_t)rows[i].zm;
-            m.np[i] = rows[i].np;
-            m.re[(size_t)i * QS_MAX_EXT] = rows[i].re0;
-            m.re[(size_t)i * QS_MAX_EXT + 1] = rows[i].re1;
-        }
-    } else {
-        std::vector<DRow> rows(n);
-        if (n) HIPCHK(hipMemcpyAsync(rows.data(), c->dt.rows, n * sizeof(DRow), hipMemcpyDeviceToHost, c->stream));
-        HIPCHK(hipStreamSynchronize(c->stream));
-        for (uint32_t i = 0; i < n; i++) {
-            m.rc[i] = rows[i].rc;
-            m.rm[i] = (int64_t)rows[i].rm << c->shift;
-            m.zc[i] = rows[i].zc;
-            m.zm[i] = (int64_t)rows[i].zm << c->shift;
-            m.np[i] = rows[i].np;
-            m.re[(size_t)i * QS_MAX_EXT] = rows[i].re0;
-            m.re[(size_t)i * QS_MAX_EXT + 1] = rows[i].re1;
-        }
-    }
-    c->mirror_stale = false;
-}
+    if (c->dev_valid && i < c->m.n) {
+        materialise_mirror(c);
+        push_row(c, i, false);
+    }
+}
+
+void sync_mirror(qs_ctx *c) { materialise_mirror(c); }
 
 int pod_min_shift(const qs_pod &p) { return std::min(ctz64(p.req_mem), ctz64(p.nz_mem)); }
 
@@ -540,10 +533,11 @@
 void flush_pending(qs_ctx *c);
 
 template <class F>
-qs_status guarded(qs_ctx *c, F &&f, bool keep_pending = false) {
+qs_status guarded(qs_ctx *c, F &&f, bool keep_pending = false, bool lazy_mirror = false) {
     if (!c) return QS_EINVAL;
     std::lock_guard<std::mutex> lk(c->mu);
     try {
+        if (!lazy_mirror) materialise_mirror(c);
         if (!keep_pending) flush_pending(c);
         f();
         c->err.clear();
@@ -551,8 +545,8 @@
     } catch (const QsError &e) {
         c->err = e.msg;
         if (e.st == QS_EDEVICE || e.st == QS_ETIMEOUT) {
+            mirror_run_discard(c->lz);
             c->dev_valid = false;
-            c->mirror_stale = false;
             c->saved = false;
             c->device_faults++;
         }
@@ -821,6 +815,10 @@
     hipStream_t s = c->stream, s2 = c->stream2;
     if (s2) (void)hipStreamSynchronize(s2);
     if (c->pin) (void)hipHostFree(c->pin);
+    for (int b = 0; b < 2; ++b) {
+        if (c->lz.snap[b]) (void)hipHostFree(c->lz.snap[b]);
+        if (c->ev_run[b]) (void)hipEventDestroy(c->ev_run[b]);
+    }
     delete c;
     if (s) (void)hipStreamDestroy(s);
     if (s2) (void)hipStreamDestroy(s2);
@@ -960,6 +958,7 @@
             m.lb[2 * (size_t)i] = nd->label_bits ? nd->label_bits[2 * (size_t)i] : 0;
             m.lb[2 * (size_t)i + 1] = nd->label_bits ? nd->label_bits[2 * (size_t)i + 1] : 0;
         }
+        mirror_statics_changed(c->lz);
         for (uint32_t i = 0; i < n; i++) check_row_values(m, i);
         c->shift = table_shift(m);
         c->zero_alloc = count_zero_alloc(m);
@@ -967,7 +966,6 @@
         for (uint32_t i = 0; i < n && !c->wide; i++) c->wide = !row_compact_ok(m, i, c->shift);
         c->dev_valid = false;
         c->saved = false;
-        c->mirror_stale = false;
         ++c->table_epoch;
         upload_table(c);
     });
@@ -1012,6 +1010,7 @@
         one.gen[0] = generation;
         check_row_values(one, 0);
         const bool was_zero = idx < m.n && zero_alloc_row(m, idx);
+        mirror_statics_changed(c->lz);
         if (idx == m.n) {
             Mirror old = m;
             m.resize(old.n + 1);
@@ -1209,6 +1208,12 @@
 }
 
 static const bool g_sdiag = getenv("QS_SCORE_DIAG") && getenv("QS_SCORE_DIAG")[0] == '1';
+static const bool g_rdiag = getenv("QS_RUN_DIAG") && getenv("QS_RUN_DIAG")[0] == '1';
+using RunClock = std::chrono::steady_clock;
+static inline RunClock::time_point run_stamp() { return g_rdiag ? RunClock::now() : RunClock::time_point{}; }
+static inline double run_us(RunClock::time_point a, RunClock::time_point b) {
+    return std::chrono::duration<double, std::micro>(b - a).count();
+}
 struct ScoreSplit { std::chrono::steady_clock::time_point ts, tl, t0, te; };
 static thread_local ScoreSplit g_split;
 static void score_diag_report(uint64_t seq, std::chrono::steady_clock::time_point tu) {
@@ -1361,6 +1366,8 @@
 
 qs_status qs_stream_run(qs_ctx *c, qs_stream *s, qs_mode mode, qs_stats *stats) {
     return guarded(c, [&] {
+        const auto d_in = run_stamp();
+        auto d_launch = d_in;
         if (!s) fail(QS_EINVAL, "null stream");
         if (mode != QS_MODE_EXACT && mode != QS_MODE_BATCHED) fail(QS_EINVAL, "unknown qs_mode");
         if (s->shift != c->shift || s->wide != c->wide) fail(QS_ESTATE, "node table re-laid out after prepare");
@@ -1376,11 +1383,13 @@
         uint64_t *ok = s->d_key.as<uint64_t>();
         uint64_t *st = c->cfg.record_timestamps ? s->d_stamp.as<uint64_t>() : nullptr;
         uint64_t batches = 0;
-        hipEvent_t e0, e1;
-        HIPCHK(hipEventCreate(&e0));
-        HIPCHK(hipEventCreate(&e1));
+        for (hipEvent_t &e : c->ev_run)
+            if (!e) HIPCHK(hipEventCreate(&e));
+        const hipEvent_t e0 = c->ev_run[0], e1 = c->ev_run[1];
+        const void *tail_werr = nullptr, *tail_nfall = nullptr;
         KernelTimer kt(c->cfg.profile_kernels != 0, c->stream, c->stream2);
         HIPCHK(hipEventRecord(e0, c->stream));
+        d_launch = run_stamp();
         if (P > 0 && n == 0) {
             HIPCHK(hipMemsetAsync(on, 0xFF, 4 * (size_t)P, c->stream));
             HIPCHK(hipMemsetAsync(ok, 0, 8 * (size_t)P, c->stream));
@@ -1632,19 +1641,24 @@
                 c->last_resident = resident;
                 if (!resident) c->res_cooldown = false;
                 if (resident) {
-                    c->resctl.ensure(la_stream_res_ctl_bytes());
+                    auto up256 = [](size_t b) { return (b + 255) & ~(size_t)255; };
+                    const size_t a_ctl = up256(8 * lwords * nbuf), a_werr = a_ctl + up256(la_stream_res_ctl_bytes());
+                    const size_t a_nfall = a_werr + 16, a_bytes = a_werr + 256;
+                    c->res_arena.ensure(a_bytes);
+                    char *arena = c->res_arena.as<char>();
+                    uint64_t *rlists = reinterpret_cast<uint64_t *>(arena);
+                    void *rctl = arena + a_ctl;
+                    unsigned long long *rnfall = reinterpret_cast<unsigned long long *>(arena + a_nfall);
                     c->dc.ready = nullptr;
                     c->dc.epoch = 0;
-                    c->dc.werr = reinterpret_cast<uint32_t *>(hw + 2);
+                    c->dc.werr = reinterpret_cast<uint32_t *>(arena + a_werr);
                     c->last_waits = true;
-                    HIPCHK(hipMemsetAsync(c->lists.p, 0, 8 * lwords * nbuf, c->stream));
-                    HIPCHK(hipMemsetAsync(c->dio.p, 0, 2 * kDioWords * 4, c->stream));
-                    HIPCHK(hipMemsetAsync(c->resctl.p, 0, la_stream_res_ctl_bytes(), c->stream));
-                    HIPCHK(hipMemsetAsync(hw + 2, 0, 8, c->stream));
+                    tail_werr = arena + a_werr;
+                    tail_nfall = rnfall;
+                    HIPCHK(hipMemsetAsync(arena, 0, a_bytes, c->stream));
                     c->npart.ensure(16 * 2 * (size_t)rgeo.K * rgeo.G);
                     c->normi.ensure(16 * 2 * 64);
                     c->nstat.ensure(4 * 2 * 128 * (size_t)rgeo.K);
-                    HIPCHK(hipMemsetAsync(c->nfall.p, 0, 16, c->stream));
                     const size_t rcw = std::max<size_t>(1, (size_t)rgeo.K * rgeo.G * rgeo.L);
                     c->clists.ensure(8 * rcw * 2);
                     ResShard rsh{1u, 0u, 0ull, nullptr, 0ull, 0ull, 0ull, 0ull, 0ull};
@@ -1671,11 +1685,12 @@
                         HIPCHK(hipMemsetAsync(rdiag, 0, 1024, c->stream));
                     }
                     kt.begin(3, c->stream);
-                    HIPCHK(launch_la_stream_res(c->dt, dp, dx, dcr, P, rgeo, L0, c->clists.as<uint64_t>(),
+                    d_launch = run_stamp();
+                    HIPCHK(launch_la_stream_res(c->dt, dp, dx, dcr, P, rgeo, rlists, c->clists.as<uint64_t>(),
                                                 (uint32_t)lwords, (uint32_t)rcw, c->npart.as<uint4>(),
                                                 c->normi.as<NormInfo>(), c->nstat.as<uint32_t>(),
-                                                c->nfall.as<unsigned long long>(), on, ok,
-                                                st, c->resctl.p, sel, rdiag, rsh, c->stream));
+                                                rnfall, on, ok,
+                                                st, rctl, sel, rdiag, rsh, c->stream));
                     kt.end(3, c->stream);
                     if (rdiag) {
                         uint64_t h[128] = {0};
@@ -1764,6 +1779,10 @@
                 } else {
                     enqueue();
                 }
+                if (!resident) {
+                    tail_werr = c->last_waits ? hw + 2 : nullptr;
+                    tail_nfall = c->nfall.p;
+                }
                 batches = nwin;
                 if (getenv("QS_HOSTTIME"))
                     fprintf(stderr, "QS_HOSTTIME enqueue %.3f ms for %u windows (overlap %d)\n",
@@ -1784,16 +1803,22 @@
                 }
             }
         }
+        ensure_snap(c, n);
+        const int sb = mirror_run_begin(c->lz);
+        const uint64_t tag = ++c->tail_seq;
+        HIPCHK(launch_run_tail(c->dt, n, c->shift, tail_werr, tail_nfall, tag, c->lz.snap[sb], c->stream));
         HIPCHK(hipEventRecord(e1, c->stream));
+        const auto d_enq = run_stamp();
         HIPCHK(hipEventSynchronize(e1));
+        const auto d_done = run_stamp();
+        std::atomic_thread_fence(std::memory_order_acquire);
+        const int64_t *head = c->lz.snap[sb];
+        if ((uint64_t)head[3] != tag) fail(QS_EDEVICE, "qs_stream_run: the run's snapshot did not reach the host");
         float ms = 0.f;
         HIPCHK(hipEventElapsedTime(&ms, e0, e1));
-        (void)hipEventDestroy(e0);
-        (void)hipEventDestroy(e1);
         uint64_t rescans = 0, resumed = 0;
         if (eng == QS_ENGINE_LOOKAHEAD && c->last_waits) {
-            uint64_t w = 0;
-            HIPCHK(hipMemcpy(&w, c->hand.as<uint64_t>() + 2, 8, hipMemcpyDeviceToHost));
+            uint64_t w = (uint64_t)head[0];
             if (inject_once(c, "handoff", kInjHandoff)) w = 1;
             if (w) {
                 if (c->last_resident) {
@@ -1813,19 +1838,19 @@
         }
         if (eng == QS_ENGINE_LOOKAHEAD && c->last_resident) c->res_timeouts = 0;
         if (eng == QS_ENGINE_LOOKAHEAD && c->nfall.p) {
-            uint64_t h[2] = {0, 0};
-            HIPCHK(hipMemcpy(h, c->nfall.p, 16, hipMemcpyDeviceToHost));
+            const uint64_t h[2] = {(uint64_t)head[1], (uint64_t)head[2]};
             rescans = h[0];
             resumed = h[1];
             if (getenv("QS_NORM_DIAG"))
                 fprintf(stderr, "QS_NORM_DIAG rescans %llu resumed windows %llu\n", (unsigned long long)h[0],
                         (unsigned long long)h[1]);
         }
-        c->mirror_stale = true;
+        const auto d_status = run_stamp();
         if (eng != QS_ENGINE_SCAN) c->soa_valid = false;
         kt.finish();
         maybe_inject_fault(c, "stream_run");
-        sync_mirror(c);
+        mirror_run_accept(c->lz);
+        const auto d_mirror = run_stamp();
         s->ran = true;
         s->mode_ran = (int)mode;
         s->epoch_after = ++c->table_epoch;
@@ -1847,7 +1872,12 @@
             stats->resident_path = stats->resident ? c->last_res_path : 0;
             stats->device_faults = c->device_faults;
         }
-    });
+        if (g_rdiag)
+            std::fprintf(stderr, "QS_RUN_DIAG run %u pods: pre-launch %.1f us, launch return %.1f us, completion seen %.1f us "
+                                 "(e0..e1 %.1f us), status words %.1f us, mirror %.1f us, return %.1f us\n",
+                         P, run_us(d_in, d_launch), run_us(d_launch, d_enq), run_us(d_enq, d_done), ms * 1e3,
+                         run_us(d_done, d_status), run_us(d_status, d_mirror), run_us(d_mirror, run_stamp()));
+    }, false, true);
 }
 
 qs_status qs_stream_results(qs_ctx *c, qs_stream *s, int32_t *placement, uint64_t *best_key) {
@@ -1867,7 +1897,7 @@
             if (placement) placement[j] = node[k];
             if (best_key) best_key[j] = key[k];
         }
-    });
+    }, false, true);
 }
 
 qs_status qs_stream_free(qs_ctx *c, qs_stream *s) {
@@ -1889,7 +1919,7 @@
         c->tbl_saved.ensure(c->tbl.bytes);
         HIPCHK(hipMemcpyAsync(c->tbl_saved.p, c->tbl.p, c->tbl.bytes, hipMemcpyDeviceToDevice, c->stream));
         HIPCHK(hipStreamSynchronize(c->stream));
-        c->m_saved = c->m;
+        mirror_save(c->lz, c->m, c->m_saved, c->zero_alloc);
         c->saved_wide = c->wide;
         c->saved_shift = c->shift;
         c->saved = true;
@@ -1902,13 +1932,16 @@
             c->saved_shift != c->shift)
             fail(QS_ESTATE, "no matching qs_table_save snapshot");
         HIPCHK(hipSetDevice(c->device));
+        const auto d_in = run_stamp();
         HIPCHK(hipMemcpyAsync(c->tbl.p, c->tbl_saved.p, c->tbl.bytes, hipMemcpyDeviceToDevice, c->stream));
-        c->m = c->m_saved;
-        c->zero_alloc = count_zero_alloc(c->m);
-        c->mirror_stale = false;
+        const auto d_enq = run_stamp();
+        mirror_restore(c->lz, c->m, c->m_saved, c->zero_alloc);
         ++c->table_epoch;
         c->soa_valid = false;
-    });
+        if (g_rdiag)
+            std::fprintf(stderr, "QS_RUN_DIAG restore: enqueue %.1f us, host work %.1f us\n", run_us(d_in, d_enq),
+                         run_us(d_enq, run_stamp()));
+    }, false, true);
 }
 
 qs_status qs_schedule_stream(qs_ctx *c, const qs_pod *pods, uint32_t p, qs_mode mode,
diff --git a/custom-k8s-scheduler_amd/csrc/qs_kernels.hip b/custom-k8s-scheduler_amd/csrc/qs_kernels.hip
--- a/custom-k8s-scheduler_amd/csrc/qs_kernels.hip
+++ b/custom-k8s-scheduler_amd/csrc/qs_kernels.hip
@@ -1,4 +1,8 @@
 #include "qs_kernels.hpp"
+
+#include <array>
+#include <map>
+#include <mutex>
 
 namespace qs {
 
@@ -187,15 +191,39 @@
 }
 size_t la_stream_res_ctl_bytes() { return kResCtlBytes; }
 
+static int la_stream_res_per_cu_query(const LaGeom &geo, uint32_t feat, uint32_t n) {
+    return (feat & kFeatStrat) ? ((feat & kFeatWide) ? strat_wide_la_stream_res_per_cu(geo, feat, n)
+                                                     : strat_compact_la_stream_res_per_cu(geo, feat, n))
+           : (feat & kFeatRes)   ? ((feat & kFeatWide) ? res_wide_la_stream_res_per_cu(geo, feat, n)
+                                                     : res_compact_la_stream_res_per_cu(geo, feat, n))
+           : (feat & kFeatWide)  ? wide_la_stream_res_per_cu(geo, feat, n)
+           : (feat & kFeatNorm)  ? la_stream_res_per_cu<kFeatExt | kFeatTaint | kFeatAffinity>(geo, n)
+           : (feat & kFeatExt) ? la_stream_res_per_cu<kFeatExt>(geo, n)
+                               : la_stream_res_per_cu<0>(geo, n);
+}
+
+static int la_stream_res_per_cu_memo(const LaGeom &geo, uint32_t feat, uint32_t n) {
+    const uint32_t cls = feat & (kFeatStrat | kFeatRes | kFeatWide | kFeatTaint | kFeatAffinity | kFeatExt);
+    const uint32_t words = (((n + 31) / 32) + 3) & ~3u;
+    int dev = 0;
+    (void)hipGetDevice(&dev);
+    const std::array<uint32_t, 6> key = {cls, geo.E, geo.e2, geo.k32 ? 1u : 0u, words, (uint32_t)dev};
+    static std::mutex mu;
+    static std::map<std::array<uint32_t, 6>, int> memo;
+    {
+        std::lock_guard<std::mutex> lk(mu);
+        const auto it = memo.find(key);
+        if (it != memo.end()) return it->second;
+    }
+    const int per = la_stream_res_per_cu_query(geo, feat, n);
+    std::lock_guard<std::mutex> lk(mu);
+    if (memo.size() >= 256) memo.clear();
+    if (per > 0) memo[key] = per;
+    return per;
+}
+
 uint32_t la_stream_res_max_blocks(const LaGeom &geo, uint32_t feat, uint32_t n, uint32_t cus) {
-    const int per = (feat & kFeatStrat) ? ((feat & kFeatWide) ? strat_wide_la_stream_res_per_cu(geo, feat, n)
-                                                              : strat_compact_la_stream_res_per_cu(geo, feat, n))
-                    : (feat & kFeatRes)   ? ((feat & kFeatWide) ? res_wide_la_stream_res_per_cu(geo, feat, n)
-                                                              : res_compact_la_stream_res_per_cu(geo, feat, n))
-                    : (feat & kFeatWide)  ? wide_la_stream_res_per_cu(geo, feat, n)
-                    : (feat & kFeatNorm)  ? la_stream_res_per_cu<kFeatExt | kFeatTaint | kFeatAffinity>(geo, n)
-                    : (feat & kFeatExt) ? la_stream_res_per_cu<kFeatExt>(geo, n)
-                                        : la_stream_res_per_cu<0>(geo, n);
+    const int per = la_stream_res_per_cu_memo(geo, feat, n);
     const int sgpr_waves = 800 / (((int)kResSgprMax + 15) / 16 * 16 + 16);
     const int safe = std::min(per, sgpr_waves / (kResBS / 64 / 4));
     return (uint32_t)std::max(0, safe) * cus;
diff --git a/custom-k8s-scheduler_amd/csrc/qs_kernels.hpp b/custom-k8s-scheduler_amd/csrc/qs_kernels.hpp
--- a/custom-k8s-scheduler_amd/csrc/qs_kernels.hpp
+++ b/custom-k8s-scheduler_amd/csrc/qs_kernels.hpp
@@ -1,6 +1,9 @@
 #pragma once
 #include <algorithm>
 #include <cstring>
+#include <map>
+#include <mutex>
+#include <utility>
 
 #include "qs_device.hpp"
 #include "qs_launch.hpp"
@@ -3312,7 +3315,23 @@
 
 static hipError_t res_lds_attr(const void *fn, size_t lds4) {
     if (lds4 <= 64 * 1024) return hipSuccess;
-    return hipFuncSetAttribute(fn, hipFuncAttributeMaxDynamicSharedMemorySize, (int)lds4);
+    static std::mutex mu;
+    static std::map<std::pair<const void *, int>, size_t> raised;
+    int dev = 0;
+    (void)hipGetDevice(&dev);
+    const std::pair<const void *, int> key{fn, dev};
+    {
+        std::lock_guard<std::mutex> lk(mu);
+        const auto it = raised.find(key);
+        if (it != raised.end() && it->second >= lds4) return hipSuccess;
+    }
+    const hipError_t e = hipFuncSetAttribute(fn, hipFuncAttributeMaxDynamicSharedMemorySize, (int)lds4);
+    if (e == hipSuccess) {
+        std::lock_guard<std::mutex> lk(mu);
+        size_t &v = raised[key];
+        v = std::max(v, lds4);
+    }
+    return e;
 }
 template <uint32_t F>
 static hipError_t la_stream_res_f(const DevTable &t, const void *pods, const DPodX *podx, const DevCfg &c, uint32_t P,
diff --git a/custom-k8s-scheduler_amd/csrc/qs_kernels_tail.hip b/custom-k8s-scheduler_amd/csrc/qs_kernels_tail.hip
--- /dev/null
+++ b/custom-k8s-scheduler_amd/csrc/qs_kernels_tail.hip
@@ -0,0 +1,50 @@
+#include "qs_device.hpp"
+#include "qs_launch.hpp"
+
+namespace qs {
+
+__global__ void __launch_bounds__(256) k_run_tail(DevTable t, uint32_t n, int shift, const unsigned long long *werr,
+                                                  const unsigned long long *nfall, unsigned long long tag,
+                                                  long long *out) {
+    const uint32_t i = blockIdx.x * 256u + threadIdx.x;
+    if (i == 0) {
+        out[0] = werr ? (long long)werr[0] : 0;
+        out[1] = nfall ? (long long)nfall[0] : 0;
+        out[2] = nfall ? (long long)nfall[1] : 0;
+        out[3] = (long long)tag;
+    }
+    if (i >= n) return;
+    long long rc, rm, zc, zm, np, re0, re1;
+    if (t.wrows) {
+        const DRowW r = t.wrows[i];
+        rc = r.rc; zc = r.zc; np = r.np; re0 = r.re0; re1 = r.re1;
+        rm = (long long)r.rm;
+        zm = (long long)r.zm;
+    } else {
+        const DRow r = t.rows[i];
+        rc = r.rc; zc = r.zc; np = r.np; re0 = r.re0; re1 = r.re1;
+        rm = (long long)r.rm << shift;
+        zm = (long long)r.zm << shift;
+    }
+    long long *col = out + 4;
+    const size_t N = n;
+    col[i] = rc;
+    col[N + i] = rm;
+    col[2 * N + i] = zc;
+    col[3 * N + i] = zm;
+    col[4 * N + i] = np;
+    col[5 * N + 2 * (size_t)i] = re0;
+    col[5 * N + 2 * (size_t)i + 1] = re1;
+}
+
+hipError_t launch_run_tail(const DevTable &t, uint32_t n, int shift, const void *werr, const void *nfall,
+                           uint64_t tag, int64_t *out, hipStream_t stream) {
+    if (!out || (n && !t.rows && !t.wrows) || shift < 0 || shift > 62) return hipErrorInvalidValue;
+    const uint32_t blocks = n ? (n + 255u) / 256u : 1u;
+    hipLaunchKernelGGL(k_run_tail, dim3(blocks), dim3(256), 0, stream, t, n, shift,
+                       (const unsigned long long *)werr, (const unsigned long long *)nfall,
+                       (unsigned long long)tag, (long long *)out);
+    return hipGetLastError();
+}
+
+}
diff --git a/custom-k8s-scheduler_amd/csrc/qs_launch.hpp b/custom-k8s-scheduler_amd/csrc/qs_launch.hpp
--- a/custom-k8s-scheduler_amd/csrc/qs_launch.hpp
+++ b/custom-k8s-scheduler_amd/csrc/qs_launch.hpp
@@ -94,4 +94,7 @@
 
 __global__ void k_set_row(DevTable t, uint32_t i, HostRow v, uint32_t feat);
 
+hipError_t launch_run_tail(const DevTable &t, uint32_t n, int shift, const void *werr, const void *nfall,
+                           uint64_t tag, int64_t *out, hipStream_t stream);
+
 }
diff --git a/custom-k8s-scheduler_amd/csrc/qs_mirror_state.hpp b/custom-k8s-scheduler_amd/csrc/qs_mirror_state.hpp
--- /dev/null
+++ b/custom-k8s-scheduler_amd/csrc/qs_mirror_state.hpp
@@ -0,0 +1,107 @@
+#pragma once
+#include <stddef.h>
+#include <stdint.h>
+
+#include <cstring>
+#include <vector>
+
+#include "../../include/qsched.h"
+
+namespace qs_host {
+
+struct Mirror {
+    uint32_t n = 0;
+    std::vector<int64_t> ac, am, mp, rc, rm, zc, zm, np;
+    std::vector<int64_t> ae, re;
+    std::vector<uint64_t> th, ts, lb;
+    std::vector<int32_t> zone;
+    std::vector<uint64_t> gen;
+    void resize(uint32_t nn) {
+        n = nn;
+        zone.assign(nn, 0);
+        for (auto *v : {&ac, &am, &mp, &rc, &rm, &zc, &zm, &np}) v->assign(nn, 0);
+        ae.assign((size_t)nn * QS_MAX_EXT, 0);
+        re.assign((size_t)nn * QS_MAX_EXT, 0);
+        th.assign(nn, 0);
+        ts.assign(nn, 0);
+        lb.assign((size_t)nn * 2, 0);
+        gen.assign(nn, 0);
+    }
+};
+
+constexpr size_t kSnapHead = 4;
+constexpr size_t kSnapCols = 5 + QS_MAX_EXT;
+inline size_t snap_words(uint32_t n) { return kSnapHead + kSnapCols * (size_t)n; }
+
+struct MirrorLazy {
+    enum Where : uint8_t { kHere, kSnapshot, kSaved };
+    Where dyn = kHere;
+    int64_t *snap[2] = {nullptr, nullptr};
+    uint32_t snap_cap = 0;
+    int accepted = 0;
+    bool pending = false;
+    uint64_t gen_counter = 0;
+    uint64_t static_gen = 0;
+    uint64_t saved_gen = 0;
+    uint32_t saved_zero_alloc = 0;
+};
+
+inline void mirror_statics_changed(MirrorLazy &l) { l.static_gen = ++l.gen_counter; }
+
+inline void mirror_materialise(MirrorLazy &l, Mirror &m, const Mirror &saved) {
+    if (l.dyn == MirrorLazy::kHere) return;
+    const size_t n = m.n;
+    if (l.dyn == MirrorLazy::kSnapshot) {
+        const int64_t *s = l.snap[l.accepted] + kSnapHead;
+        if (n) {
+            std::memcpy(m.rc.data(), s + 0 * n, 8 * n);
+            std::memcpy(m.rm.data(), s + 1 * n, 8 * n);
+            std::memcpy(m.zc.data(), s + 2 * n, 8 * n);
+            std::memcpy(m.zm.data(), s + 3 * n, 8 * n);
+            std::memcpy(m.np.data(), s + 4 * n, 8 * n);
+            std::memcpy(m.re.data(), s + 5 * n, 8 * n * QS_MAX_EXT);
+        }
+    } else {
+        m.rc = saved.rc;
+        m.rm = saved.rm;
+        m.zc = saved.zc;
+        m.zm = saved.zm;
+        m.np = saved.np;
+        m.re = saved.re;
+    }
+    l.dyn = MirrorLazy::kHere;
+}
+
+inline int mirror_run_begin(MirrorLazy &l) {
+    l.pending = true;
+    return l.accepted ^ 1;
+}
+inline void mirror_run_discard(MirrorLazy &l) { l.pending = false; }
+inline void mirror_run_accept(MirrorLazy &l) {
+    if (!l.pending) return;
+    l.pending = false;
+    l.accepted ^= 1;
+    l.dyn = MirrorLazy::kSnapshot;
+}
+
+inline void mirror_save(MirrorLazy &l, Mirror &m, Mirror &saved, uint32_t zero_alloc) {
+    mirror_materialise(l, m, saved);
+    saved = m;
+    l.saved_gen = l.static_gen;
+    l.saved_zero_alloc = zero_alloc;
+}
+
+inline bool mirror_restore(MirrorLazy &l, Mirror &m, const Mirror &saved, uint32_t &zero_alloc) {
+    l.pending = false;
+    zero_alloc = l.saved_zero_alloc;
+    if (l.static_gen == l.saved_gen && m.n == saved.n) {
+        l.dyn = MirrorLazy::kSaved;
+        return false;
+    }
+    m = saved;
+    l.static_gen = l.saved_gen;
+    l.dyn = MirrorLazy::kHere;
+    return true;
+}
+
+}
```

After: 2.201 million pods/s. Within noise of the previous version (-0.2%).
